# lh3/psmc

Measured on AMD Instinct MI355X. Metric: genome bins/sec through forward-backward (n=64), higher is better.
Workload: dtype f64; 1 GPU; configs[2]: whole-genome .psmcfa-like batch, 30000001 bins x 64 states in 90 segments per GPU, -p 4+25*2+4+6, one E-step (EM iteration) per step, parameters of a different EM round every step; mode=fast, bins_per_gpu=30000001, bins_total=30000001, n_states=64, segments=90, longest_segment=2490000, tiles=8127, speculative_overlap_bins=3072, structured_sweeps=True, tile_bins=3712

## Files before the change

psmc_amd/csrc/api.hip:

```cpp
#include "psmc_hip_ctx.h"

static void destroy_kids(psmc_hip_ctx *c);

static int make_streams(psmc_hip_ctx *c)
{
	hipStream_t *st[5] = {&c->stream, &c->stream2, &c->stream3, &c->stream4, &c->stream5};
	for (hipStream_t *s : st) if (*s) { (void)hipStreamSynchronize(*s); (void)hipStreamDestroy(*s); *s = nullptr; }
	if (c->cu_count <= 0) {
		for (hipStream_t *s : st) if (hipStreamCreateWithFlags(s, hipStreamNonBlocking) != hipSuccess) return PSMC_HIP_EDEVICE;
		return 0;
	}
	int cus = 0;
	if (hipDeviceGetAttribute(&cus, hipDeviceAttributeMultiprocessorCount, c->device) != hipSuccess || cus <= 0) return PSMC_HIP_EDEVICE;
	if (c->cu_first < 0 || c->cu_first + c->cu_count > cus) return PSMC_HIP_EINVAL;
	std::vector<uint32_t> mask((size_t)(cus + 31) / 32, 0u);
	for (int i = c->cu_first; i < c->cu_first + c->cu_count; ++i) mask[(size_t)i >> 5] |= 1u << (i & 31);
	for (hipStream_t *s : st) if (hipExtStreamCreateWithCUMask(s, (uint32_t)mask.size(), mask.data()) != hipSuccess) return PSMC_HIP_EDEVICE;
	return 0;
}

extern "C" int psmc_hip_device_cus(int device)
{
	int cus = 0;
	if (hipDeviceGetAttribute(&cus, hipDeviceAttributeMultiprocessorCount, device) != hipSuccess) { (void)hipGetLastError(); return 0; }
// ... 93 lines not shown
			}
		}
	}
	*out = c;
	return PSMC_HIP_OK;
}

static void destroy_kids(psmc_hip_ctx *c)
{
	if (c->x_twin) { psmc_hip_destroy(c->x_twin); c->x_twin = nullptr; }
	for (psmc_hip_ctx *k : c->kids) psmc_hip_destroy(k);
	c->kids.clear();
	c->share_T = 0;
}

extern "C" void psmc_hip_destroy(psmc_hip_ctx *c)
{
	if (!c) return;
	(void)hipSetDevice(c->device);
	destroy_kids(c);
	if (c->parent) {
		void *mine[] = {c->d_seg_off, c->d_seg_len, c->d_work, c->d_chunks, c->d_entry, c->d_bexit, c->d_Cpart, c->d_Epart, c->d_LLpart,
		                c->d_stage, c->d_stats, c->d_warm, c->d_bentry, c->d_dirty, c->d_cnt, c->d_gate, c->d_queue, c->d_touch, c->d_items, c->d_ftiles, c->d_Kcol,
		                c->d_segA, c->d_segE, c->d_segA0, c->d_chk};
		for (void *p : mine) if (p) (void)hipFree(p);
		if (c->h_cnt) (void)hipHostFree(c->h_cnt);
		if (c->h_ritems) (void)hipHostFree(c->h_ritems);
		if (c->h_mlen) (void)hipHostFree(c->h_mlen);
		if (c->h_chunks) (void)hipHostFree(c->h_chunks);
		if (c->h_mis) (void)hipHostFree(c->h_mis);
		if (c->d_prevx) (void)hipFree(c->d_prevx);
		if (c->d_finv) (void)hipFree(c->d_finv);
		delete c;
		return;
	}
	if (c->stream) (void)hipStreamSynchronize(c->stream);
	free_wide_fast(c);
	if (c->stream2) (void)hipStreamSynchronize(c->stream2);
	if (c->stream3) (void)hipStreamSynchronize(c->stream3);
	if (c->stream4) (void)hipStreamSynchronize(c->stream4);
	if (c->stream5) (void)hipStreamSynchronize(c->stream5);
	if (!c->obs_borrowed && c->d_obs) (void)hipFree(c->d_obs);
	void *ptrs[] = {c->d_seg_off, c->d_seg_len, c->d_work, c->d_par, c->d_f, c->d_b, c->d_s, c->d_segA, c->d_segE,
	                c->d_segA0, c->d_chk, c->d_chunks, c->d_entry, c->d_bexit, c->d_Cpart, c->d_Epart, c->d_LLpart,
	                c->d_stage, c->d_stats, c->d_warm, c->d_bentry, c->d_dirty, c->d_cnt, c->d_gate, c->d_queue, c->d_touch, c->d_sb, c->d_items, c->d_ftiles, c->d_Kcol,
	                c->d_bw_seg, c->d_bw_par, c->d_bw_tab, c->d_bpar, c->d_s_all, c->d_cu_mask, c->d_lkp, c->d_lkoff, c->d_b2};
	for (void *p : ptrs) if (p) (void)hipFree(p);
	if (c->h_par) (void)hipHostFree(c->h_par);
	if (c->h_cnt) (void)hipHostFree(c->h_cnt);
	if (c->h_ritems) (void)hipHostFree(c->h_ritems);
	if (c->h_mlen) (void)hipHostFree(c->h_mlen);
	if (c->h_chunks) (void)hipHostFree(c->h_chunks);
	if (c->h_mis) (void)hipHostFree(c->h_mis);
	if (c->d_prevx) (void)hipFree(c->d_prevx);
	if (c->d_finv) (void)hipFree(c->d_finv);
	for (int i = 0; i < 10; ++i) if (c->ev[i]) (void)hipEventDestroy(c->ev[i]);
	for (int i = 0; i < 14; ++i) if (c->evx[i]) (void)hipEventDestroy(c->evx[i]);
	if (c->stream4) (void)hipStreamDestroy(c->stream4);
	if (c->stream5) (void)hipStreamDestroy(c->stream5);
	if (c->stream2) (void)hipStreamDestroy(c->stream2);
	if (c->stream3) (void)hipStreamDestroy(c->stream3);
	if (c->stream) (void)hipStreamDestroy(c->stream);
	delete c;
}

extern "C" int psmc_hip_set_option(psmc_hip_ctx *c, const char *key, double v)
{
	if (!c || !key) return PSMC_HIP_EINVAL;
	std::string k(key);
	if (k == "batch_first") { if (v < 0 || v > 1e6) return PSMC_HIP_EINVAL; c->batch_first = (int)v; return PSMC_HIP_OK; }
	destroy_kids(c);
	if (k == "chunk") { if (v < 0) return PSMC_HIP_EINVAL; c->chunk = (int)v; c->plan_dirty = true; }
	else if (k == "warmup") { if (v < 0) return PSMC_HIP_EINVAL; c->warmup = (int)v; c->warmup_set = true; c->plan_dirty = true; }
	else if (k == "max_rounds") c->max_rounds = (int)v;
	else if (k == "structured") { c->struct_opt = v != 0 ? 1 : 0; }
	else if (k == "learn") { c->learn = v != 0 ? 1 : 0; }
	else if (k == "merge") { c->merge = v != 0 ? 1 : 0; c->plan_dirty = true; c->chunk_cap = 0; }
	else if (k == "adapt") { c->adapt = v != 0 ? 1 : 0; c->plan_dirty = true; c->chunk_cap = 0; }
	else if (k == "prev_start") { c->prev_start = v != 0 ? 1 : 0; c->prev_ok = false; c->plan_dirty = true; c->chunk_cap = 0; }
	else if (k == "warm_shift") { if (v < 0 || v > 4) return PSMC_HIP_EINVAL; c->warm_shift = (int)v; c->warm_shift_set = true; c->plan_dirty = true; }
	else if (k == "merge1") { if (v < -1 || v > 1) return PSMC_HIP_EINVAL; c->merge1 = (int)v; c->plan_dirty = true; }
	else if (k == "phase1") { if (v < -1 || v > 1) return PSMC_HIP_EINVAL; c->phase1 = (int)v; }
	else if (k == "phase1_waves") { if (v < 1 || v > 4) return PSMC_HIP_EINVAL; c->phase1_waves = (int)v; }
	else if (k == "lanes8") { if (v < -1 || v > 1) return PSMC_HIP_EINVAL; c->lanes8 = (int)v; }
	else if (k == "gap_tiles") { c->gap_tiles = v != 0 ? 1 : 0; c->plan_dirty = true; c->items_dirty = true; }
	else if (k == "coarse") { if (v < -1 || v > 16) return PSMC_HIP_EINVAL; c->coarse = (int)v; c->plan_dirty = true; c->items_dirty = true; }
	else if (k == "kc_sub") { if (v < 1 || v > 16) return PSMC_HIP_EINVAL; c->kc_sub = (int)v; c->kc_sub_set = true; c->plan_dirty = true; c->items_dirty = true; }
	else if (k == "two_phase") { if (v != -1 && v != 0 && v != 2) return PSMC_HIP_EINVAL; c->two_phase = (int)v; c->plan_dirty = true; c->items_dirty = true; }
	else if (k == "kc_min") { if (v < -1) return PSMC_HIP_EINVAL; c->kc_min = (int)v; c->items_dirty = true; }
	else if (k == "ckpt") { c->ckpt = v != 0 ? 1 : 0; }
	else if (k == "fuse") { c->fuse = v != 0 ? 1 : 0; c->plan_dirty = true; }
	else if (k == "fuse128") { if (v != 0 && v != 2) return PSMC_HIP_EINVAL; c->fuse128 = (int)v; c->plan_dirty = true; c->items_dirty = true; }
	else if (k == "group_cap") { if (v < 0) return PSMC_HIP_EINVAL; c->group_cap = (int)v; c->items_dirty = true; }
	else if (k == "share_learn") { c->share_learn = v != 0 ? 1 : 0; }
	else if (k == "exact_refwd") { if (v < -1 || v > 2) return PSMC_HIP_EINVAL; c->exact_refwd = (int)v; c->reserved_refwd = -1; c->reserved_cap = 0; if (c->d_b2) { (void)hipFree(c->d_b2); c->d_b2 = nullptr; c->b2_bins = c->b2_alloc = 0; } }
	else if (k == "batch_sort") { c->batch_sort = v != 0 ? 1 : 0; }
	else if (k == "batch_tailfill") c->batch_tailfill = v != 0;
	else if (k == "batch_major") c->batch_major = v != 0;
	else if (k == "batch_bins") { if (v < 0) return PSMC_HIP_EINVAL; c->batch_bins = (int64_t)v; }
	else if (k == "overlap") c->overlap = v != 0 ? 1 : 0;
	else if (k == "warm_tol") c->warm_tol = v;
	else if (k == "wide_fast") { if (v != 0 && v != 1) return PSMC_HIP_EINVAL; c->wide_fast = (int)v; }
	else if (k == "wide_decode") { if (v != 0 && v != 1) return PSMC_HIP_EINVAL; c->wide_decode = (int)v; }
	else if (k == "rep_impl") c->rep_impl = v < 0 ? -1 : (v != 0 ? 1 : 0);
	else return PSMC_HIP_EINVAL;
	return PSMC_HIP_OK;
}

int set_segments_common(psmc_hip_ctx *c, int n_seg, const int32_t *L)
{
	destroy_kids(c);
	c->reserved_refwd = -1; c->reserved_cap = 0;
	if (c->d_b2) { (void)hipFree(c->d_b2); c->d_b2 = nullptr; c->b2_bins = c->b2_alloc = 0; }
	c->n_seg = n_seg;
	c->L.assign(L, L + n_seg);
	int rc;
	if ((rc = dev_alloc(c, &c->d_seg_off, (size_t)n_seg))) return rc;
	if ((rc = dev_alloc(c, &c->d_seg_len, (size_t)n_seg))) return rc;
	HIPCHK(c, hipMemcpy(c->d_seg_off, c->off.data(), sizeof(int64_t) * n_seg, hipMemcpyHostToDevice));
	HIPCHK(c, hipMemcpy(c->d_seg_len, c->L.data(), sizeof(int32_t) * n_seg, hipMemcpyHostToDevice));
	std::vector<int32_t> all(n_seg);
	for (int i = 0; i < n_seg; ++i) all[i] = i;
	return psmc_hip_select(c, n_seg, all.data());
}

extern "C" int psmc_hip_load_segments(psmc_hip_ctx *c, int n_seg, const uint8_t *const *seq, const int32_t *L)
{
	if (!c || n_seg < 1 || !seq || !L) return fail(c, PSMC_HIP_EINVAL, "load_segments: bad argument");
	HIPCHK(c, hipSetDevice(c->device));
	c->off.resize(n_seg);
	int64_t tot = 0;
	for (int i = 0; i < n_seg; ++i) {
		if (L[i] < 1 || !seq[i]) return fail(c, PSMC_HIP_EINVAL, "load_segments: empty segment");
		c->off[i] = tot;
		tot += ((int64_t)L[i] + 63) & ~(int64_t)63;
	}
	c->total = tot;
	std::vector<uint8_t> host((size_t)tot + 256, 2);
	for (int i = 0; i < n_seg; ++i) {
		for (int32_t j = 0; j < L[i]; ++j)
			if (seq[i][j] > 2) return fail(c, PSMC_HIP_EINVAL, "load_segments: symbol outside {0,1,2}");
		memcpy(host.data() + c->off[i], seq[i], (size_t)L[i]);
	}
	if (!c->obs_borrowed && c->d_obs) { (void)hipFree(c->d_obs); }
	c->d_obs = nullptr; c->obs_borrowed = false;
	int rc;
	if ((rc = dev_alloc(c, &c->d_obs, host.size()))) return rc;
	HIPCHK(c, hipMemcpy(c->d_obs, host.data(), host.size(), hipMemcpyHostToDevice));
	return set_segments_common(c, n_seg, L);
}

extern "C" int psmc_hip_load_segments_device(psmc_hip_ctx *c, int n_seg, const void *d_obs, const int64_t *off,
                                             const int32_t *L)
{
	if (!c || n_seg < 1 || !d_obs || !off || !L) return fail(c, PSMC_HIP_EINVAL, "load_segments_device: bad argument");
	HIPCHK(c, hipSetDevice(c->device));
	int64_t end = 0;
	for (int i = 0; i < n_seg; ++i) {
		if (L[i] < 1 || (off[i] & 63) || off[i] < end) return fail(c, PSMC_HIP_EINVAL, "load_segments_device: bad layout");
		end = off[i] + (((int64_t)L[i] + 63) & ~(int64_t)63);
	}
	if (!c->obs_borrowed && c->d_obs) (void)hipFree(c->d_obs);
	c->d_obs = (uint8_t *)d_obs; c->obs_borrowed = true;
	c->off.assign(off, off + n_seg);
	c->total = end;
	return set_segments_common(c, n_seg, L);
// ... 374 lines not shown
```

psmc_amd/csrc/api_batch.hip:

```cpp
#include "psmc_hip_ctx.h"

namespace {
struct RepSel { std::vector<int32_t> work, sel2work; int64_t bins = 0; };
}

static int batch_selections(psmc_hip_ctx *c, int n_rep, const int32_t *sel_off, const int32_t *sel_idx, std::vector<RepSel> &reps)
{
	std::vector<int32_t> pos(c->n_seg);
	reps.assign(n_rep, RepSel());
	for (int r = 0; r < n_rep; ++r) {
		const int n_sel = sel_off[r + 1] - sel_off[r];
		if (n_sel < 1) return fail(c, PSMC_HIP_EINVAL, "estep_batch: empty selection");
		std::fill(pos.begin(), pos.end(), -1);
		RepSel &R = reps[r];
		R.sel2work.resize(n_sel);
		for (int i = 0; i < n_sel; ++i) {
			const int32_t sg = sel_idx[sel_off[r] + i];
			if (sg < 0 || sg >= c->n_seg) return fail(c, PSMC_HIP_EINVAL, "estep_batch: index out of range");
			if (pos[sg] < 0) { pos[sg] = (int32_t)R.work.size(); R.work.push_back(sg); R.bins += ((int64_t)c->L[sg] + 63) & ~(int64_t)63; }
			R.sel2work[i] = pos[sg];
		}
	}
	return 0;
}
// ... 299 lines not shown
				}
		}
	};
	std::vector<int32_t> finished;
	for (int g = 0; g < n_launches; ++g) {
		const double t_a = now();
		const int e0 = l_first[g], nw = l_first[g + 1] - e0;
		int64_t run = 0; int32_t longest = 0;
		for (int i = e0; i < e0 + nw; ++i) if (wseg[i] >= 0) { run = std::max(run, wtab[i] + padded_len(wseg[i])); longest = std::max(longest, c->L[wseg[i]]); }
		EstepLaunch p;
		fill_common(c, p, c->stream, c->d_bpar);
		p.d_work = c->d_bw_seg + e0; p.n_work = nw; p.d_work_par = c->d_bw_par + e0; p.d_work_tab = c->d_bw_tab + e0; p.par_stride = (int64_t)PL; p.work_align = align;
		p.exact_refwd = refwd ? (c->exact_refwd == 1 ? 1 : 2) : 0;
		p.d_cu_mask = c->d_cu_mask;
		if (fwd_all) { p.exact_only = 2; p.d_work_tab_s = c->d_bw_tab + n_all + e0; p.d_s = c->d_s_all; }
		p.d_segA = c->d_segA; p.d_segE = c->d_segE; p.d_segA0 = c->d_segA0; p.d_chk = c->d_chk;
		const double t_b = now();
		if (launch_exact(p) != 0) return fail(c, PSMC_HIP_EDEVICE, "launch_exact (batch)", hipGetLastError());
		if (dbg_t) (void)hipStreamSynchronize(c->stream);
		const double t_c = now();
		std::vector<int64_t> lkoff((size_t)nw);
		int64_t lk_tot = 0;
		for (int i = 0; i < nw; ++i) { lkoff[i] = lk_tot; lk_tot += wseg[e0 + i] >= 0 ? c->L[wseg[e0 + i]] / LKP_DIV + LKP_MIN : 1; }
		HIPCHK(c, hipMemcpyAsync(c->d_lkoff, lkoff.data(), sizeof(int64_t) * nw, hipMemcpyHostToDevice, c->stream));
		if (launch_lk_products(c->stream, p, fwd_all ? c->d_s_all : c->d_s, c->d_lkoff, c->d_lkp) != 0) return fail(c, PSMC_HIP_EDEVICE, "launch_lk_products", hipGetLastError());
		c->h_lkp.resize((size_t)lk_tot);
		HIPCHK(c, hipMemcpyAsync(c->h_segA.data() + (size_t)e0 * S * S, c->d_segA, sizeof(double) * nw * S * S, hipMemcpyDeviceToHost, c->stream));
		HIPCHK(c, hipMemcpyAsync(c->h_segE.data() + (size_t)e0 * 3 * S, c->d_segE, sizeof(double) * nw * 3 * S, hipMemcpyDeviceToHost, c->stream));
		HIPCHK(c, hipMemcpyAsync(c->h_lkp.data(), c->d_lkp, sizeof(double) * (size_t)lk_tot, hipMemcpyDeviceToHost, c->stream));
		HIPCHK(c, hipStreamSynchronize(c->stream));
		const double t_d = now();
		collect_timing(c);
		int n_over = 0;
		for (int i = 0; i < nw; ++i) {
			if (wseg[e0 + i] < 0) continue;
			const int32_t sg = wseg[e0 + i];
			const double *q = &c->h_lkp[(size_t)lkoff[i]];
			const int cnt = (int)q[0], cap_i = c->L[sg] / LKP_DIV + LKP_MIN;
			if (cnt >= 1 && cnt < cap_i) {
				double sum = 0.0;
				for (int j = 1; j <= cnt; ++j) sum += log(q[j]);
				lk_all[(size_t)e0 + i] = sum;
			} else {
				++n_over;
				c->h_s.resize((size_t)c->L[sg]);
				HIPCHK(c, hipMemcpyAsync(c->h_s.data(), (fwd_all ? c->d_s_all + wtab_s[e0 + i] : c->d_s + wtab[e0 + i]), sizeof(double) * (size_t)c->L[sg], hipMemcpyDeviceToHost, c->stream));
				HIPCHK(c, hipStreamSynchronize(c->stream));
				lk_all[(size_t)e0 + i] = host_lk(c->h_s.data(), c->L[sg]);
			}
		}
		if (dbg_t && n_over) fprintf(stderr, "[psmc_hip] batch launch %d: %d entries logged more products than their buffer holds (host hmm_lk)\n", g, n_over);
		if (dbg_t) fprintf(stderr, "[psmc_hip] batch launch %d: %d entries (longest %d bins), %.1f M table bins | prepare %.3f s, kernels %.3f (fwd %.0f bwd %.0f expect %.0f ms%s), read-back %.3f, hmm_lk %.3f\n",
		                   g, nw, (int)longest, run / 1e6, t_b - t_a, t_c - t_b, c->last_ms[1], c->last_ms[2], c->last_ms[3],
		                   fwd_all ? (g == 0 ? (std::string("; forward pass of all entries ") + std::to_string(fwd_all_s) + " s").c_str() : "; fwd: see launch 0") : "", t_d - t_c, now() - t_d);
		++c->last_batch_groups;
		const double t_f = now();
		finished.clear();
		for (int r = 0; r < n_rep; ++r) if (last_launch[r] == g) { finalize(r); finished.push_back(r); }
		t_sums += now() - t_f;
		if (done && !finished.empty()) done(user, (int)finished.size(), finished.data());
	}
	if (dbg_t) {
		std::string per;
		for (int g = 0; g < n_launches; ++g) per += (g ? " " : "") + std::to_string(std::count(last_launch.begin(), last_launch.end(), g));
		fprintf(stderr, "[psmc_hip] batch: %d replicates, %d entries in %d launches (replicates complete after launch 0..: %s), host sums %.3f s\n", n_rep, n_all, n_launches, per.c_str(), t_sums);
	}
	return PSMC_HIP_OK;
}

static psmc_hip_ctx *batch_child(psmc_hip_ctx *c, int r)
{
	while ((int)c->kids.size() <= r) {
		psmc_hip_ctx *k = new (std::nothrow) psmc_hip_ctx();
		if (!k) return nullptr;
		k->n = c->n; k->ns = c->ns; k->device = c->device; k->mode = c->mode; k->parent = c;
		k->chunk = c->chunk > 0 ? c->chunk : c->share_T;
		k->warmup = c->warmup; k->max_rounds = c->max_rounds; k->rep_impl = c->rep_impl;
		k->n_sub = c->n_sub; k->target_waves = c->target_waves; k->overlap = c->overlap; k->warm_tol = c->warm_tol; k->struct_opt = c->struct_opt;
		k->struct_tiles_set = c->struct_tiles_set; k->struct_tiles = c->struct_tiles;
		k->two_phase = c->two_phase; k->kc_div = c->kc_div; k->kc_min = c->kc_min; k->ckpt = c->ckpt; k->fuse = c->fuse;
		k->learn = c->learn; k->group_cap = c->group_cap; k->warm_shift = c->warm_shift; k->kc_sub = c->kc_sub; k->kcol_prio = c->kcol_prio;
		k->fuse128 = c->fuse128; k->coarse = c->coarse; k->gate = c->gate; k->lanes8 = c->lanes8; k->gap_tiles = c->gap_tiles; k->exact_refwd = c->exact_refwd;
		k->merge = c->merge; k->adapt = c->adapt; k->prev_start = c->prev_start;
		k->merge1 = c->merge1; k->merge_order = c->merge_order; k->runs_late = c->runs_late; k->warm_shift_set = c->warm_shift_set; k->kc_sub_set = c->kc_sub_set;
		k->stream = c->stream; k->stream2 = c->stream2; k->stream3 = c->stream3; k->stream4 = c->stream4; k->stream5 = c->stream5;
		for (int i = 0; i < 14; ++i) k->evx[i] = c->evx[i];
		for (int i = 0; i < 10; ++i) k->ev[i] = c->ev[i];
		k->h_par = c->h_par; k->d_par = c->d_par; k->par_len = c->par_len;
		k->d_obs = c->d_obs; k->obs_borrowed = true; k->off = c->off; k->total = c->total;
		if (set_segments_common(k, c->n_seg, c->L.data()) != 0) { c->err = k->err; psmc_hip_destroy(k); return nullptr; }
		c->kids.push_back(k);
	}
	return c->kids[r];
}

static int batch_exact_once(psmc_hip_ctx *c, int r, const int32_t *idx, int n_sel, const double *a, const double *e, const double *a0,
                            double *A, double *sums, double *E, double *LL, const char *why)
{
	const int n = c->n;
	fprintf(stderr, "[psmc_hip] replicate %d: fast E-step did not converge (%s); repeating this E-step with the exact kernels\n", c->batch_first + r, why);
	int rc = 0;
	if (!c->x_twin) {
		if ((rc = psmc_hip_create(&c->x_twin, n, c->device, PSMC_HIP_MODE_EXACT))) return fail(c, rc, "estep_batch: cannot create the exact twin context");
		if ((rc = psmc_hip_load_segments_device(c->x_twin, c->n_seg, c->d_obs, c->off.data(), c->L.data()))) {
			c->err = "exact twin: " + c->x_twin->err; psmc_hip_destroy(c->x_twin); c->x_twin = nullptr; return rc;
		}
	}
	std::vector<double> Af;
	double *Ao = A;
	if (!Ao) { Af.resize((size_t)n * n); Ao = Af.data(); }
	if ((rc = psmc_hip_select(c->x_twin, n_sel, idx)) || (rc = psmc_hip_estep(c->x_twin, a, e, a0, Ao, E, nullptr, LL, nullptr))) { c->err = "exact twin: " + c->x_twin->err; return rc; }
	if (sums) {
		memset(sums, 0, sizeof(double) * 5 * (size_t)n);
		for (int k = 0; k < n; ++k)
			for (int l = 0; l < n; ++l) {
				const double v = Ao[(size_t)k * n + l];
				if (l < k) { sums[k] += v; sums[3 * n + l] += v; } else if (l > k) { sums[n + k] += v; sums[4 * n + l] += v; } else sums[2 * n + k] = v;
			}
	}
	++c->n_exact_fallbacks;
	return PSMC_HIP_OK;
}

static int batch_fast(psmc_hip_ctx *c, int n_rep, const double *a, const double *e, const double *a0, const int32_t *sel_off,
                      const int32_t *sel_idx, double *A, double *sums, double *E, double *LL, psmc_hip_batch_done_fn done, void *user)
{
	const int n = c->n;
	if (c->share_T == 0 && c->share_learn) {
		int T = c->chunk;
		if (T <= 0) {
			std::vector<RepSel> reps;
			int rc0 = batch_selections(c, n_rep, sel_off, sel_idx, reps);
			if (rc0) return rc0;
			int64_t most = 0; size_t nw = 1;
			for (const RepSel &R : reps) {
				int64_t bins = 0;
				for (int32_t sg : R.work) bins += c->L[sg];
				if (bins > most) { most = bins; nw = R.work.size(); }
			}
			T = auto_tile_len(c, most, nw, true);
		}
		c->share_T = T;
		c->sh_glue_f.assign(c->n_seg, {}); c->sh_glue_b.assign(c->n_seg, {}); c->sh_wf.assign(c->n_seg, {}); c->sh_wb.assign(c->n_seg, {});
		for (int sg = 0; sg < c->n_seg; ++sg) {
			const size_t nt = ((size_t)c->L[sg] + T - 1) / T;
			c->sh_glue_f[sg].assign(nt, 0); c->sh_glue_b[sg].assign(nt, 0); c->sh_wf[sg].assign(nt, c->warmup); c->sh_wb[sg].assign(nt, c->warmup);
		}
	}
	static const bool dbg_t = getenv("PSMC_HIP_DEBUG_TIMES") != nullptr;
	const double t_call = dbg_now();
	double t_est = 0.0;
	for (int r = 0; r < n_rep; ++r) {
		const double t_k = dbg_now();
		psmc_hip_ctx *k = batch_child(c, c->batch_first + r);
		c->dbg_acc[0] += dbg_now() - t_k;
		if (!k) return fail(c, PSMC_HIP_ENOMEM, "estep_batch: cannot create the replicate context");
		const int n_sel = sel_off[r + 1] - sel_off[r];
		if (n_sel < 1) return fail(c, PSMC_HIP_EINVAL, "estep_batch: empty selection");
		const int32_t *idx = sel_idx + sel_off[r];
		int rc = 0;
		{
			const double t_s = dbg_now();
			if ((int)k->sel.size() != n_sel || memcmp(k->sel.data(), idx, sizeof(int32_t) * n_sel) != 0) rc = psmc_hip_select(k, n_sel, idx);
			c->dbg_acc[1] += dbg_now() - t_s;
		}
		const double t_e = dbg_now();
// ... 48 lines not shown
```

psmc_amd/csrc/api_fast.hip:

```cpp
#include "psmc_hip_ctx.h"

int ensure_fast_buffers(psmc_hip_ctx *c)
{
	if (c->d_stage && c->d_stats && c->d_warm && c->d_cnt && c->h_cnt && c->d_gate) return 0;
	int rc;
	const size_t sl = (size_t)c->ns * c->ns + 3 * (size_t)c->ns + 1;
	if ((rc = dev_alloc(c, &c->d_stage, (size_t)RED_ROWS * sl))) return rc;
	if ((rc = dev_alloc(c, &c->d_stats, sl))) return rc;
	if ((rc = dev_alloc(c, &c->d_warm, (size_t)2))) return rc;
	if ((rc = dev_alloc(c, &c->d_cnt, (size_t)4))) return rc;
	if ((rc = dev_alloc(c, &c->d_gate, (size_t)4))) return rc;
	if (!c->h_cnt && (hipHostMalloc((void **)&c->h_cnt, 4 * sizeof(int), hipHostMallocMapped) != hipSuccess ||
	                  hipHostGetDevicePointer((void **)&c->m_cnt, c->h_cnt, 0) != hipSuccess)) {
		c->h_cnt = nullptr;
		return fail(c, PSMC_HIP_ENOMEM, "hipHostMalloc (mapped)");
	}
	return 0;
}

int auto_tile_len(const psmc_hip_ctx *c, int64_t bins, size_t n_work, bool st)
{
	const int64_t ROUND1 = 4096;
	int64_t want = st ? c->struct_tiles : c->target_waves;
	if (st && !c->struct_tiles_set && bins < 2 * ROUND1 * (int64_t)std::max(c->warmup, 1))
		want = std::max<int64_t>(ROUND1 - (int64_t)n_work, ROUND1 / 2);
	const int T = (int)((bins + want - 1) / want);
	return std::max(256, (T + 63) & ~63);
}

static int plan_fast(psmc_hip_ctx *c)
{
	int64_t bins = 0;
	for (int32_t s : c->work) bins += c->L[s];
	int T = c->chunk;
	const bool st = c->use_struct;
	const int64_t ROUND1 = 4096;
	bool one_round = false;
	if (T <= 0) T = auto_tile_len(c, bins, c->work.size(), st);
	c->chunks.clear(); c->chunk_seg.clear(); c->chunk_idx.clear();
	for (size_t w = 0; w < c->work.size(); ++w) {
		const int32_t s = c->work[w];
		for (int32_t lo = 1; lo <= c->L[s]; lo += T) {
			c->chunk_seg.push_back(s); c->chunk_idx.push_back((lo - 1) / T);
			Chunk ch;
			ch.off = c->off[s]; ch.L = c->L[s]; ch.lo = lo; ch.hi = std::min(c->L[s], lo + T - 1); ch.mult = c->mult[w];
			ch.flags = 0; ch.wf = ch.wb = c->warmup;
			if (ch.lo - c->warmup <= 1) ch.flags |= CHUNK_ANCHOR_F;
			if ((int64_t)ch.hi + c->warmup + 1 >= ch.L) ch.flags |= CHUNK_ANCHOR_B;
			if (ch.hi == ch.L) ch.flags |= CHUNK_LAST;
			c->chunks.push_back(ch);
		}
	}
	const int nc = (int)c->chunks.size();
	c->chunk_used = T;
	c->planned_struct = st;
	one_round = st && nc <= ROUND1;
	c->two_phase_used = c->two_phase >= 0 ? c->two_phase : (one_round ? 0 : 2);
	c->merge1_used = c->merge1 >= 0 ? c->merge1 : (one_round ? 1 : 0);
	c->warm_shift_used = c->warm_shift_set ? c->warm_shift : (one_round ? 0 : 1);
	c->coarse_used = c->coarse >= 0 ? std::max(c->coarse, 1) : (one_round && nc > 2048 && T < c->warmup ? 2 : 1);
	c->kc_sub_used = c->kc_sub_set ? c->kc_sub : std::max(1, std::min(4, (int)((8 * (int64_t)T + T + c->warmup - 1) / std::max(T + c->warmup, 1))));
	c->n_sub_used = st ? (fused_counts(c) ? 1 : std::max(1, std::min(c->n_sub, (9216 + nc - 1) / std::max(nc, 1)))) : c->n_sub;
	c->glue_f.assign(nc, 0); c->glue_b.assign(nc, 0);
	if (c->parent && c->parent->share_T == T && st) {
		const psmc_hip_ctx *P = c->parent;
		for (int b = 0; b < nc; ++b) {
			const int sg = c->chunk_seg[b], ix = c->chunk_idx[b];
			if (sg >= (int)P->sh_glue_f.size() || ix >= (int)P->sh_glue_f[sg].size()) continue;
			c->glue_f[b] = P->sh_glue_f[sg][ix]; c->glue_b[b] = P->sh_glue_b[sg][ix];
			c->chunks[b].wf = std::max(c->chunks[b].wf, P->sh_wf[sg][ix]); c->chunks[b].wb = std::max(c->chunks[b].wb, P->sh_wb[sg][ix]);
		}
	}
	c->items_dirty = true;
	int rc;
	c->gap.assign(nc, 0);
	if (nc > c->chunk_cap) {
		if ((rc = dev_alloc(c, &c->d_chunks, (size_t)nc))) return rc;
		if ((rc = dev_alloc(c, &c->d_entry, (size_t)nc * c->ns))) return rc;
		if ((rc = dev_alloc(c, &c->d_bexit, (size_t)(nc + 1) * c->ns))) return rc;
		if ((rc = dev_alloc(c, &c->d_bentry, (size_t)nc * c->ns))) return rc;
		if ((rc = dev_alloc(c, &c->d_dirty, (size_t)2 * nc))) return rc;
		if ((rc = dev_alloc(c, &c->d_touch, (size_t)3 * nc))) return rc;
		if ((rc = dev_alloc(c, &c->d_finv, (size_t)nc))) return rc;
		if (c->h_mlen) { (void)hipHostFree(c->h_mlen); c->h_mlen = nullptr; c->m_mlen = nullptr; }
		if (c->h_mis) { (void)hipHostFree(c->h_mis); c->h_mis = nullptr; c->m_mis = nullptr; }
		if (c->prev_start && (rc = dev_alloc(c, &c->d_prevx, (size_t)nc * c->ns))) return rc;
		if ((c->merge || c->adapt) &&
		    (hipHostMalloc((void **)&c->h_mlen, (size_t)nc * sizeof(int), hipHostMallocMapped) != hipSuccess ||
		     hipHostGetDevicePointer((void **)&c->m_mlen, c->h_mlen, 0) != hipSuccess ||
		     hipHostMalloc((void **)&c->h_mis, (size_t)2 * nc * sizeof(double), hipHostMallocMapped) != hipSuccess ||
		     hipHostGetDevicePointer((void **)&c->m_mis, c->h_mis, 0) != hipSuccess))
			return fail(c, PSMC_HIP_ENOMEM, "hipHostMalloc (mapped)");
		if ((rc = dev_alloc(c, &c->d_LLpart, (size_t)nc))) return rc;
		if ((rc = dev_alloc(c, &c->d_items, (size_t)32 * nc + 64))) return rc;
		if ((rc = dev_alloc(c, &c->d_ftiles, (size_t)2 * (nc + 16)))) return rc;
		if (c->h_ritems) { (void)hipHostFree(c->h_ritems); c->h_ritems = nullptr; }
		if (hipHostMalloc((void **)&c->h_ritems, (size_t)4 * nc * sizeof(int), hipHostMallocMapped) != hipSuccess ||
		    hipHostGetDevicePointer((void **)&c->m_ritems, c->h_ritems, 0) != hipSuccess)
			return fail(c, PSMC_HIP_ENOMEM, "hipHostMalloc (mapped)");
		c->chunk_cap = nc;
	}
	if ((rc = dev_alloc(c, &c->d_Epart, (size_t)nc * c->n_sub_used * 3 * c->ns))) return rc;
	if ((rc = ensure_fast_buffers(c))) return rc;
	HIPCHK(c, hipMemcpy(c->d_chunks, c->chunks.data(), sizeof(Chunk) * nc, hipMemcpyHostToDevice));
	if (st && c->gap_tiles) {
		std::vector<int> fl(nc, 0);
		if (launch_tile_allmiss(c->stream, c->d_obs, c->d_chunks, nc, c->d_dirty) != 0) return fail(c, PSMC_HIP_EDEVICE, "k_tile_allmiss", hipGetLastError());
		HIPCHK(c, hipMemcpyAsync(fl.data(), c->d_dirty, sizeof(int) * nc, hipMemcpyDeviceToHost, c->stream));
		HIPCHK(c, hipMemsetAsync(c->d_dirty, 0, sizeof(int) * nc, c->stream));
		HIPCHK(c, hipStreamSynchronize(c->stream));
		for (int b = 0; b < nc; ++b) {
			const Chunk &ch = c->chunks[b];
			c->gap[b] = fl[b] && ch.lo > 1 && ch.hi < ch.L && ch.hi - ch.lo + 1 == T;
		}
		auto same = [&](int x, int y) { return x >= 0 && y < nc && c->chunks[x].off == c->chunks[y].off; };
		for (int b = 0; b < nc; ++b) {
			if (c->gap[b]) { if (same(b - 1, b)) c->glue_f[b] = 1; if (same(b, b + 1)) c->glue_b[b] = 1; }
			if (b > 0 && c->gap[b - 1] && same(b - 1, b)) c->glue_f[b] = 1;
			if (b + 1 < nc && c->gap[b + 1] && same(b, b + 1)) c->glue_b[b] = 1;
		}
	}
	c->plan_dirty = false; c->chunks_dirty = false; c->prev_ok = false;
	return 0;
}

static int build_items(psmc_hip_ctx *c, bool two_phase_bwd, int coarse)
{
	const int nc = (int)c->chunks.size(), W = c->warmup;
	const int cf = std::max(1, coarse), cb = two_phase_bwd ? 1 : cf;
	std::vector<int> odd(nc, 0), idx(nc, 0);
	for (int b = 1; b < nc; ++b) if (c->chunks[b].off == c->chunks[b - 1].off) { odd[b] = !odd[b - 1]; idx[b] = idx[b - 1] + 1; }
	std::vector<std::pair<long long, std::pair<int, int>>> kf, kb;
	auto key = [](int steps, bool run, bool phase_b) { return (run ? -(1ll << 40) : (phase_b ? (1ll << 40) : 0ll)) - steps; };
	std::vector<char> from_above(nc, 0), in_run(nc, 0), in_run_f(nc, 0), in_run_b(nc, 0);
	std::vector<std::pair<int, int>> gf, gb;
	auto same_seg = [&](int x, int y) { return c->chunks[x].off == c->chunks[y].off; };
	const bool gaps = c->gap_tiles && (int)c->gap.size() == nc;
	std::vector<int64_t> eff(nc + 1, 0);
	for (int b = 0; b < nc; ++b) eff[b + 1] = eff[b] + ((gaps && c->gap[b]) ? 0 : c->chunks[b].hi - c->chunks[b].lo + 1);
	auto span_ok = [&](int b, int e) { return eff[e + 1] - eff[b] <= (int64_t)c->group_cap; };
	for (int b = 0; b < nc;) {
		int e = b + 1;
		while (e < nc && c->glue_f[e] && same_seg(e, b) && span_ok(b, e)) ++e;
		if (e - b > 1) for (int t = b; t < e; ++t) in_run[t] = in_run_f[t] = 1;
		else
			while (e < nc && e - b < cf && same_seg(e, b) && idx[e] % cf != 0 && !c->glue_f[e] && !(e + 1 < nc && c->glue_f[e + 1] && same_seg(e + 1, e))) ++e;
		gf.push_back({b, e - b});
		b = e;
	}
	for (int b = 0; b < nc;) {
		int e = b + 1;
		while (e < nc && c->glue_b[e - 1] && same_seg(e, b) && span_ok(b, e) &&
		       c->chunks[e].lo < c->chunks[e].L)
			++e;
		if (e - b > 1) for (int t = b; t < e; ++t) in_run[t] = in_run_b[t] = 1;
		else
			while (e < nc && e - b < cb && same_seg(e, b) && idx[e] % cb != 0 && !c->glue_b[e - 1] && !(e + 1 < nc && c->glue_b[e] && same_seg(e + 1, e)) &&
			       c->chunks[e].lo < c->chunks[e].L)
				++e;
		gb.push_back({b, e - b});
		b = e;
	}
	int n_run = 0;
	for (int b = 0; b < nc; ++b) n_run += in_run[b];
	const int cap_b = (nc + 7) / 8 * 4;
	c->runs_in_b = two_phase_bwd && c->runs_late && n_run > 0 && n_run <= cap_b / 2;
	int above_budget = c->runs_in_b ? cap_b - n_run : nc;
	for (const auto &gr : gb) {
		const int b = gr.first, e = b + gr.second;
		const Chunk &lo = c->chunks[b], &top = c->chunks[e - 1];
		bool pb = two_phase_bwd && e - b == 1 && odd[b] && b + 1 < nc && c->chunks[b + 1].off == lo.off && c->chunks[b + 1].lo < c->chunks[b + 1].L;
		if (pb && c->runs_in_b && (in_run[b] || in_run[b + 1] || above_budget <= 0)) pb = false;
		if (pb) { from_above[b] = 1; --above_budget; }
		kb.push_back({key(std::min(top.hi + chunk_warm_b(top, W) + 1, top.L) - lo.lo, in_run_b[b] != 0, pb), {b, e - b}});
	}
	std::vector<int> la, lb;
	{
		std::vector<int> freet;
		for (int b = 0; b < nc; ++b) {
			if (from_above[b]) lb.push_back(b | (1 << 30));
			else if (b > 0 && from_above[b - 1]) la.push_back(b);
			else if (c->runs_in_b && in_run[b]) lb.push_back(b);
			else freet.push_back(b);
		}
		const bool single = lb.empty() && nc <= 4096;
		for (int b : freet) { if (single || la.size() <= lb.size()) la.push_back(b); else lb.push_back(b); }
	}
	for (const auto &gr : gf) {
		const int b = gr.first, e = b + gr.second;
		const Chunk &h = c->chunks[b], &l = c->chunks[e - 1];
		kf.push_back({key(l.hi - std::max(1, h.lo - chunk_warm_f(h, W)) + 1, in_run_f[b] != 0, false), {b, e - b}});
	}
	std::sort(kf.begin(), kf.end()); std::sort(kb.begin(), kb.end());
	std::vector<int> h((size_t)4 * nc, 0), mem((size_t)4 * nc, 0);
	c->n_mem_f = c->n_mem_b = 0;
	for (size_t i = 0; i < kf.size(); ++i) {
		h[2 * i] = kf[i].second.first; h[2 * i + 1] = kf[i].second.second;
		if (in_run_f[kf[i].second.first])
			for (int t = 0; t < kf[i].second.second; ++t) { mem[2 * (size_t)c->n_mem_f] = kf[i].second.first + t; mem[2 * (size_t)c->n_mem_f + 1] = 1; ++c->n_mem_f; }
	}
	for (size_t i = 0; i < kb.size(); ++i) {
		h[(size_t)2 * nc + 2 * i] = kb[i].second.first; h[(size_t)2 * nc + 2 * i + 1] = kb[i].second.second;
		if (in_run_b[kb[i].second.first])
			for (int t = 0; t < kb[i].second.second; ++t) {
				mem[(size_t)2 * nc + 2 * (size_t)c->n_mem_b] = kb[i].second.first + t; mem[(size_t)2 * nc + 2 * (size_t)c->n_mem_b + 1] = 1; ++c->n_mem_b;
			}
	}
	c->n_items_f = (int)kf.size(); c->n_items_b = (int)kb.size();
	c->order_f.clear();
	for (const auto &it : kf) if (!in_run_f[it.second.first]) c->order_f.push_back(it.second.first);
	c->n_long_f = c->n_long_b = 0;
	while (c->n_long_f < c->n_items_f && in_run_f[kf[c->n_long_f].second.first]) ++c->n_long_f;
	while (c->n_long_b < c->n_items_b && in_run_b[kb[c->n_long_b].second.first]) ++c->n_long_b;
	c->n_B_b = 0;
	for (int b = 0; b < nc; ++b) c->n_B_b += from_above[b];
	{
		c->n_list_a = (int)la.size(); c->n_list_b = (int)lb.size();
		c->count_group = c->ns == 128 && c->fuse128 == 2 ? 16 : 4;
		while (la.size() % c->count_group) la.push_back(-1);
		while (lb.size() % c->count_group) lb.push_back(-1);
		la.insert(la.end(), lb.begin(), lb.end());
		if (!la.empty()) HIPCHK(c, hipMemcpy(c->d_ftiles, la.data(), sizeof(int) * la.size(), hipMemcpyHostToDevice));
	}
	c->items_two_phase = two_phase_bwd ? 2 : 0; c->items_coarse = coarse;
	HIPCHK(c, hipMemcpy(c->d_items, h.data(), sizeof(int) * h.size(), hipMemcpyHostToDevice));
	{
		std::vector<int> sg;
		for (size_t i = (size_t)c->n_long_b; i < kb.size(); ++i)
			for (int t = kb[i].second.second - 1; t >= 0; --t) { sg.push_back(kb[i].second.first + t); sg.push_back(1); }
		c->n_singles_b = (int)sg.size() / 2;
		if (!sg.empty()) HIPCHK(c, hipMemcpy(c->d_items + (size_t)24 * nc, sg.data(), sizeof(int) * sg.size(), hipMemcpyHostToDevice));
	}
	HIPCHK(c, hipMemcpy(c->d_items + (size_t)8 * nc, mem.data(), sizeof(int) * mem.size(), hipMemcpyHostToDevice));
	{
		std::vector<int> fx;
		for (int b = 0; b < nc; ++b)
			if (!in_run_f[b] && !(b > 0 && in_run_f[b - 1] && same_seg(b - 1, b))) { fx.push_back(b); fx.push_back(1); }
		c->n_fix_f = (int)fx.size() / 2;
		if (!fx.empty()) HIPCHK(c, hipMemcpy(c->d_items + (size_t)30 * nc, fx.data(), sizeof(int) * fx.size(), hipMemcpyHostToDevice));
	}
	{
		const int n4f = c->n_items_f - c->n_long_f, n4b = c->n_items_b - c->n_long_b - c->n_B_b;
		std::vector<std::pair<long long, int>> qk;
		for (int k = 0; 4 * k < n4f; ++k) {
			long long st = 0;
			for (int i = c->n_long_f + 4 * k; i < std::min(c->n_long_f + 4 * k + 4, c->n_items_f); ++i) {
				const Chunk &h = c->chunks[kf[i].second.first], &l = c->chunks[kf[i].second.first + kf[i].second.second - 1];
				st = std::max(st, (long long)(l.hi - std::max(1, h.lo - chunk_warm_f(h, W)) + 1));
			}
			qk.push_back({-st * 504, 2 * k});
		}
		for (int k = 0; 4 * k < n4b; ++k) {
			long long st = 0;
			for (int i = c->n_long_b + 4 * k; i < std::min(c->n_long_b + 4 * k + 4, c->n_long_b + n4b); ++i) {
				const Chunk &lo = c->chunks[kb[i].second.first], &top = c->chunks[kb[i].second.first + kb[i].second.second - 1];
				const int q = std::min(top.hi + chunk_warm_b(top, W) + 1, top.L);
				st = std::max(st, (long long)(q - (coarse > 1 ? std::min(lo.hi, lo.L - 1) : std::min(top.hi, top.L - 1))));
			}
			qk.push_back({-st * 534, 2 * k + 1});
		}
		std::stable_sort(qk.begin(), qk.end(), [](const std::pair<long long, int> &x, const std::pair<long long, int> &y) { return x.first < y.first; });
		std::vector<int> qv(qk.size());
		for (size_t i = 0; i < qk.size(); ++i) qv[i] = qk[i].second;
		if (c->queue_cap < qv.size()) { int rc; if ((rc = dev_alloc(c, &c->d_queue, qv.size()))) return rc; c->queue_cap = qv.size(); }
		c->n_queue = (int)qv.size();
		if (!qv.empty()) HIPCHK(c, hipMemcpy(c->d_queue, qv.data(), sizeof(int) * qv.size(), hipMemcpyHostToDevice));
	}
	std::vector<int> wl((size_t)4 * nc, 0), kc, runs_f, runs_b, kslot, kuniq;
	int gap_slot[2] = {-1, -1};
	auto push_kc = [&](int t, int dir) {
		const int j = (int)kc.size() / 2;
		kc.push_back(t); kc.push_back(dir);
		if (gaps && c->gap[t] && c->chunk_used % 4 == 0) {
			if (gap_slot[dir] < 0) { gap_slot[dir] = (int)kuniq.size(); kuniq.push_back(j); }
			kslot.push_back(gap_slot[dir]);
		} else { kslot.push_back((int)kuniq.size()); kuniq.push_back(j); }
	};
	c->n_wl_f = c->n_wl_b = 0;
	const int kc_min = c->kc_min >= 0 ? c->kc_min : (c->ns == 128 ? (nc > 4096 ? 12 : 8) : (nc > 4096 ? 5 : 4));
	const bool chains = kc_min >= 2;
	const int head_count = c->ns == 64 ? 0 : 1;
	auto add_runs = [&](const std::vector<std::pair<long long, std::pair<int, int>>> &k, int n_long, bool bwd) {
		int &nw = bwd ? c->n_wl_b : c->n_wl_f;
		std::vector<int> &rv = bwd ? runs_b : runs_f;
		int *w = wl.data() + (bwd ? (size_t)2 * nc : 0);
		int budget = std::max(64, nc / c->kc_div);
		for (int i = 0; i < n_long; ++i) {
			int first = k[i].second.first, count = k[i].second.second;
			int cost = 0;
			for (int tt = first; tt < first + count; ++tt) cost += (gaps && c->gap[tt] && c->chunk_used % 4 == 0) ? 0 : 1;
			cost = std::max(cost - 1, 1);
			const bool chain = chains && count >= kc_min && cost <= budget;
			if (chain) budget -= cost;
			if (chain && !bwd && c->chunks[first].lo == 1) {
				w[2 * nw] = first; w[2 * nw + 1] = (head_count == 0 && count - 1 >= 2) ? -1 : 2; ++nw;
				first += 1; count -= 1;
				if (count >= 2) {
					rv.push_back(first); rv.push_back(count); rv.push_back((int)(kc.size() / 2)); rv.push_back(0);
					for (int t = first; t < first + count - 1; ++t) push_kc(t, 0);
				}
			} else if (chain) {
				w[2 * nw] = bwd ? first + count - 1 : first; w[2 * nw + 1] = head_count; ++nw;
				rv.push_back(first); rv.push_back(count); rv.push_back((int)(kc.size() / 2)); rv.push_back(0);
				if (!bwd) for (int t = first; t < first + count - 1; ++t) push_kc(t, 0);
				else for (int t = first + count - 1; t > first; --t) push_kc(t, 1);
// ... 83 lines not shown
	if (changed) {
		c->chunks_dirty = true;
		int64_t total = 0, waste = 0;
		for (size_t i = 0; i + 3 < c->order_f.size(); i += 4) {
			int64_t s4 = 0, mx = 0;
			for (int r = 0; r < 4; ++r) { const Chunk &ch = c->chunks[c->order_f[i + r]]; const int64_t st = (int64_t)ch.hi - std::max(1, ch.lo - ch.wf) + 1; s4 += st; mx = std::max(mx, st); }
			total += 4 * mx; waste += 4 * mx - s4;
		}
		if (total > 0 && waste * 100 > total * 3) c->items_dirty = true;
	}
}

int enqueue_fast(psmc_hip_ctx *c, const double *a, const double *e, const double *a0, double *d_out,
                        hipStream_t st)
{
	HIPCHK(c, hipSetDevice(c->device));
	if (c->n_seg < 1) return fail(c, PSMC_HIP_ESTATE, "estep: no segments loaded");
	int rc;
	c->dec_kind = DEC_NONE;
	const unsigned long long serial0 = dbg_root(c)->tab_serial;
	if ((rc = ensure_tables(c, false))) return rc;
	c->tables_batch = false;
	if ((rc = stage_params(c, a, e, a0, st))) return rc;
	if (!c->want_factored && !(c->use_struct && fused_counts(c)) && (rc = ensure_tables(c, true))) return rc;
	if (c->ns == 128 && !c->use_struct)
		return fail(c, PSMC_HIP_ENOTSUP, "fast mode beyond 64 states needs a transition matrix of the PSMC form (structured sweeps)");
	if (c->want_factored && !c->use_struct)
		return fail(c, PSMC_HIP_ENOTSUP, "factored statistics need a transition matrix of the PSMC form");
	{
		const double t0 = dbg_now();
		if ((c->plan_dirty || c->planned_struct != c->use_struct) && (rc = plan_fast(c))) return rc;
		dbg_root(c)->dbg_acc[2] += dbg_now() - t0;
	}
	EstepLaunch p;
	fill_common(c, p, st);
	p.d_chunks = c->d_chunks; p.n_chunks = (int)c->chunks.size(); p.warmup = c->warmup; p.n_sub = c->n_sub_used;
	const bool two_phase_bwd = c->two_phase_used >= 1 && p.fused == 1;
	p.merge1 = c->merge1_used; p.merge_order = c->merge_order >= 0 ? c->merge_order : (c->chunk_used < c->warmup ? 1 : 0);
	if (c->chunks_dirty) {
		psmc_hip_ctx *R = dbg_root(c);
		if (R->h_chunks_cap < c->chunks.size()) {
			if (R->h_chunks) { (void)hipHostFree(R->h_chunks); R->h_chunks = nullptr; }
			if (hipHostMalloc((void **)&R->h_chunks, sizeof(Chunk) * c->chunks.size(), hipHostMallocDefault) != hipSuccess) return fail(c, PSMC_HIP_ENOMEM, "hipHostMalloc");
			R->h_chunks_cap = c->chunks.size();
		}
		HIPCHK(c, hipStreamSynchronize(st));
		memcpy(R->h_chunks, c->chunks.data(), sizeof(Chunk) * c->chunks.size());
		HIPCHK(c, hipMemcpyAsync(c->d_chunks, R->h_chunks, sizeof(Chunk) * c->chunks.size(), hipMemcpyHostToDevice, st));
		c->chunks_dirty = false;
	}
	const int coarse = (c->use_struct && p.fused != 0) ? c->coarse_used : 1;
	{
		const double t0 = dbg_now();
		if (c->use_struct && (c->items_dirty || c->items_two_phase != (two_phase_bwd ? 2 : 0) || c->items_coarse != coarse) && (rc = build_items(c, two_phase_bwd, coarse))) return rc;
		dbg_root(c)->dbg_acc[3] += dbg_now() - t0;
	}
	p.lanes8 = (c->lanes8 >= 0 ? c->lanes8 != 0 && p.fused != 0 : p.fused == 2 && p.n_chunks > 4096) && c->ns == 64 ? 1 : 0;
	{
		const size_t nc_ = c->chunks.size(), S_ = (size_t)c->ns;
		const size_t need = p.fused == 2 ? nc_ * 7 * S_ + 64 : (p.fused == 1 ? (nc_ / 4 + 8) * S_ * S_ : nc_ * (size_t)c->n_sub_used * S_ * S_);
		if (c->cpart_cap < need) { if ((rc = dev_alloc(c, &c->d_Cpart, need))) return rc; c->cpart_cap = need; }
	}
	{
		c->merge_used = c->merge != 0 && c->h_mlen && c->use_struct && p.fused == 1 && c->ns == 64 && c->chunk_used % 16 == 0;
		p.merge = c->merge_used ? 1 : 0;
		p.d_fmerge = c->d_touch + 2 * (size_t)p.n_chunks; p.d_finv = c->d_finv; p.m_mlen = c->m_mlen; p.h_mlen = c->h_mlen; p.m_mis = c->m_mis;
		p.d_fix_f = c->d_items + 30 * (size_t)p.n_chunks; p.n_fix_f = c->n_fix_f;
		if (c->h_mlen) memset(c->h_mlen, 0, sizeof(int) * p.n_chunks);
		if (c->h_mis) for (int b = 0; b < p.n_chunks; ++b) c->h_mis[b] = -1.0;
		const bool prev = c->prev_start && c->d_prevx && c->prev_ok && c->use_struct && c->prev_serial == serial0 && c->prev_f == c->d_f && c->prev_ckpt == p.ckpt;
		p.d_prevx = prev ? c->d_prevx : nullptr;
		c->prev_ok = false;
	}
	p.d_gate = (c->gate >= 0 ? c->gate != 0 : coarse > 1) ? c->d_gate : nullptr;
	if (c->phase1 != 0 && c->use_struct && p.fused == 1 && c->ns == 64 && !p.lanes8 && !p.merge1 && c->overlap && c->n_queue > 0) {
		int cus = c->cu_count;
		if (cus <= 0 && (hipDeviceGetAttribute(&cus, hipDeviceAttributeMultiprocessorCount, c->device) != hipSuccess || cus <= 0)) return fail(c, PSMC_HIP_EDEVICE, "hipDeviceGetAttribute");
		p.d_queue = c->d_queue; p.n_queue = c->n_queue; p.d_qhead = c->d_gate + 2;
		p.q_grid = std::min(c->n_queue, 4 * cus * c->phase1_waves);
	}
	p.coarse = coarse; p.d_singles_b = c->d_items + 24 * (size_t)p.n_chunks; p.n_singles_b = c->n_singles_b;
	p.n_B_b = c->n_B_b; p.runs_in_b = c->runs_in_b ? 1 : 0; p.n_list_a = c->n_list_a; p.n_list_b = c->n_list_b; p.d_ftiles = c->d_ftiles; p.count_group = c->count_group;
	c->timing_two_launches = p.fused == 1 && p.n_list_b > 0;
	p.d_items_f = c->d_items; p.d_items_b = c->d_items + 2 * p.n_chunks;
	p.d_ritems_f = c->d_items + 4 * p.n_chunks; p.d_ritems_b = c->d_items + 6 * p.n_chunks;
	p.n_items_f = c->n_items_f; p.n_items_b = c->n_items_b; p.tile_len = c->chunk_used; p.h_ritems = c->h_ritems; p.m_ritems = c->m_ritems; p.m_cnt = c->m_cnt;
	c->flagged_f.clear(); c->flagged_b.clear();
	p.flagged_f = &c->flagged_f; p.flagged_b = &c->flagged_b;
	p.d_entry = c->d_entry; p.d_bentry = c->d_bentry; p.d_bexit = c->d_bexit; p.d_Cpart = c->d_Cpart; p.d_Epart = c->d_Epart;
	p.d_dirty = c->d_dirty; p.d_cnt = c->d_cnt; p.h_cnt = c->h_cnt; p.tol = c->warm_tol; p.max_rounds = c->max_rounds;
	p.d_touch_f = c->d_touch; p.d_touch_b = c->d_touch + p.n_chunks; p.d_dirty_b = c->d_dirty + p.n_chunks;
	p.stream2 = c->stream2; p.stream3 = c->stream3; p.stream4 = c->stream4; p.overlap = c->overlap;
	p.n_long_f = c->n_long_f; p.n_long_b = c->n_long_b; p.n_mem_f = c->n_mem_f; p.n_mem_b = c->n_mem_b;
	p.d_members_f = c->d_items + 8 * p.n_chunks; p.d_members_b = c->d_items + 10 * p.n_chunks;
	p.d_wl_f = c->d_items + 12 * (size_t)p.n_chunks; p.d_wl_b = c->d_items + 14 * (size_t)p.n_chunks; p.n_wl_f = c->n_wl_f; p.n_wl_b = c->n_wl_b;
	p.d_kc = c->d_items + 16 * (size_t)p.n_chunks; p.d_kruns = c->d_items + 20 * (size_t)p.n_chunks;
	p.n_kc = c->n_kc; p.n_chain_f = c->n_chain_f; p.n_chain_b = c->n_chain_b;
	p.d_kslot = c->d_items + 26 * (size_t)p.n_chunks; p.d_kuniq = c->d_items + 28 * (size_t)p.n_chunks; p.n_kuniq = c->n_kuniq;
	p.kcol_prio = c->kcol_prio;
	p.d_Kcol = c->d_Kcol; p.kc_sub = kcol2_on(c) ? c->kc_sub_used : 1;
	p.d_Kexp = c->d_Kcol ? c->d_Kcol + (size_t)c->n_kuniq * p.kc_sub * c->ns * c->ns : nullptr; p.stream5 = c->stream5;
	for (int i = 0; i < 14; ++i) p.evx[i] = c->evx[i];
	p.d_LLpart = c->d_LLpart; p.d_stage = c->d_stage; p.d_stats = d_out; p.d_warm = c->d_warm;
	p.tiny_total = (double)c->sel.size() * HMM_TINY_H;
	if (p.d_prevx) launch_gather_prev(p, st, c->n_long_f, c->n_items_f - c->n_long_f, c->d_prevx);
	{
		const double t0 = dbg_now();
		if (launch_fast(p, &c->report) != 0) return fail(c, PSMC_HIP_EDEVICE, "launch_fast", hipGetLastError());
		psmc_hip_ctx *R = dbg_root(c);
		R->dbg_acc[4] += dbg_now() - t0;
		R->dbg_acc[6] += c->report.fwd_rounds + c->report.bwd_rounds; R->dbg_acc[7] += c->report.fwd_tiles + c->report.bwd_tiles;
	}
	if (getenv("PSMC_HIP_DEBUG_FLAGGED")) {
		auto dump = [&](const char *dir, const std::vector<int> &fl, const std::vector<uint8_t> &glue, bool bwd) {
			std::vector<int> u(fl); std::sort(u.begin(), u.end()); u.erase(std::unique(u.begin(), u.end()), u.end());
			fprintf(stderr, "[psmc_hip] flagged %s: %zu tile repairs, %zu distinct tiles, rounds %d:", dir, fl.size(), u.size(), bwd ? c->report.bwd_rounds : c->report.fwd_rounds);
			for (size_t i = 0; i < u.size() && i < 400; ++i) {
				const int b = u[i]; const Chunk &ch = c->chunks[b];
				int seg = 0; while (seg + 1 < c->n_seg && c->off[seg + 1] <= ch.off) ++seg;
				fprintf(stderr, " [t%d seg%d %d..%d w%d g%d x%d m%.1e ml%d]", b, seg, ch.lo, ch.hi, bwd ? ch.wb : ch.wf, (int)glue[b], (int)std::count(fl.begin(), fl.end(), b),
				        c->h_mis ? c->h_mis[(bwd ? c->chunks.size() : 0) + b] : 0.0, (!bwd && c->h_mlen) ? c->h_mlen[b] : 0);
			}
			fprintf(stderr, "\n");
		};
		dump("fwd", c->flagged_f, c->glue_f, false); dump("bwd", c->flagged_b, c->glue_b, true);
	}
	if (!c->report.converged) return fail(c, PSMC_HIP_ECONVERGE, "fast mode: tile boundaries did not converge within max_rounds");
	if (c->merge_used && c->h_mlen)
		for (size_t b = 0; b < c->chunks.size(); ++b) {
			c->report.merged += c->h_mlen[b] > 0;
			if (c->h_mlen[b] < 0 || (c->h_mlen[b] > 0 && !c->adapt)) c->flagged_f.push_back((int)b);
		}
	if (c->use_struct && c->adapt && c->merge_used && c->h_mis) adapt_warmups(c);
	if (c->use_struct && c->learn) learn_groups(c);
	if (c->use_struct) { c->prev_ok = true; c->prev_serial = dbg_root(c)->tab_serial; c->prev_f = c->d_f; c->prev_ckpt = p.ckpt; }
	c->dec_kind = c->merge_used ? DEC_MERGED : (p.fused != 0 ? DEC_NO_BT : DEC_FAST);
	c->dec_serial = dbg_root(c)->tab_serial;
	return 0;
}

int read_warm(psmc_hip_ctx *c, hipStream_t st)
{
	unsigned long long w[2];
	HIPCHK(c, hipMemcpyAsync(w, c->d_warm, sizeof(w), hipMemcpyDeviceToHost, st));
	HIPCHK(c, hipStreamSynchronize(st));
	memcpy(&c->warm_err[0], &w[0], 8); memcpy(&c->warm_err[1], &w[1], 8);
	return 0;
}

extern "C" int psmc_hip_estep_device(psmc_hip_ctx *c, const double *a, const double *e, const double *a0,
                                     void *d_stats, void *stream)
{
	if (!c || !a || !e || !a0 || !d_stats) return fail(c, PSMC_HIP_EINVAL, "estep_device: bad argument");
	if (c->mode != PSMC_HIP_MODE_FAST) return fail(c, PSMC_HIP_ENOTSUP, "estep_device: fast mode only");
	c->timing_valid = false;
	return enqueue_fast(c, a, e, a0, (double *)d_stats, (hipStream_t)stream);
}

extern "C" int psmc_hip_fast_diag(psmc_hip_ctx *c, double *wf, double *wb, int *n_chunks, int *warmup_used)
{
	if (!c) return PSMC_HIP_EINVAL;
	if (c->mode != PSMC_HIP_MODE_FAST || !c->d_warm) return fail(c, PSMC_HIP_ESTATE, "fast_diag: no fast E-step yet");
	HIPCHK(c, hipSetDevice(c->device));
	unsigned long long w[2];
	HIPCHK(c, hipMemcpy(w, c->d_warm, sizeof(w), hipMemcpyDeviceToHost));
	memcpy(&c->warm_err[0], &w[0], 8); memcpy(&c->warm_err[1], &w[1], 8);
// ... 158 lines not shown
```

psmc_amd/csrc/estep_fast.hip:

```cpp
#include <hip/hip_runtime.h>
#include <cmath>
#include <algorithm>
#include "wave_prims.h"
#include "psmc_hip_internal.h"

namespace psmc {

typedef double d4_t __attribute__((ext_vector_type(4)));

__device__ __forceinline__ double pick_ef(int sym, double e0, double e1) {
	return sym == 0 ? e0 : (sym == 1 ? e1 : 1.0);
}

__device__ __forceinline__ double fast_rcp(double x) {
	double r = __builtin_amdgcn_rcp(x);
	double t = __builtin_fma(-x, r, 1.0);
	r = __builtin_fma(r, t, r);
	t = __builtin_fma(-x, r, 1.0);
	r = __builtin_fma(r, t, r);
	return r;
}

__device__ __forceinline__ double wave_max(double v) {
#pragma unroll
	for (int m = 32; m >= 1; m >>= 1) v = fmax(v, __shfl_xor(v, m, 64));
	return v;
}
__device__ __forceinline__ double wave_add(double v) {
#pragma unroll
	for (int m = 32; m >= 1; m >>= 1) v += __shfl_xor(v, m, 64);
	return v;
}
__device__ __forceinline__ double rel_mismatch(double x, double y) {
	const double num = wave_max(fabs(x - y)), den = wave_max(fabs(y));
	const bool bad = __any((x != x) || (y != y));
	return bad ? __builtin_inf() : num / den;
}

template <int REP, bool REPAIR>
__global__ __launch_bounds__(64) void k_fwd_fast(const double *__restrict__ a, const double *__restrict__ e,
                                                   const double *__restrict__ a0, const uint8_t *__restrict__ obs,
                                                   const Chunk *__restrict__ chunks, int W, double tol,
                                                   const int *__restrict__ dirty, double *__restrict__ f,
                                                   double *__restrict__ invd, double *__restrict__ entry,
                                                   int *__restrict__ touch_f)
{
	if (REPAIR && !dirty[blockIdx.x]) return;
	if (REPAIR) __builtin_amdgcn_s_setprio(3);
	const int lane = threadIdx.x;
	if (REPAIR && lane == 0) touch_f[blockIdx.x] = 1;
	const Chunk c = chunks[blockIdx.x];
	const uint8_t *o = obs + c.off;
	double *fo = f + c.off * 64, *io = invd + c.off;
	double A[64];
	load_nat_matrix(a, lane, A);
	const double e0 = e[lane], e1 = e[64 + lane];
	double x;
	int p;
	if (REPAIR) {
		x = fo[(int64_t)(c.lo - 2) * 64 + lane];
		p = c.lo;
	} else {
		const int ws = max(1, c.lo - W);
		if (ws == 1) {
			x = a0[lane] * pick_ef((int)o[0], e0, e1);
			if (c.lo == 1) fo[lane] = x;
			p = 2;
		} else {
			x = a0[lane];
			p = ws;
		}
	}
	int symn = o[(((p - 1) >> 6) << 6) + lane];
	bool done = false;
	while (p <= c.hi && !done) {
		const int blk = (p - 1) >> 6;
		const int symv = symn;
		symn = o[((blk + 1) << 6) + lane];
		const int pend = min(c.hi, (blk + 1) << 6);
		double oldv = 0.0;
		if (REPAIR) oldv = fo[(int64_t)(pend - 1) * 64 + lane];
		for (; p <= pend; ++p) {
			const int idx = p - 1;
			const int sym = __builtin_amdgcn_readlane(symv, idx & 63);
			if (p == c.lo) entry[(int64_t)blockIdx.x * 64 + lane] = x;
			double ev = pick_ef(sym, e0, e1);
			if ((p & (NORM_EVERY - 1)) == 0) {
				const double inv = fast_rcp(first_lane_f64(wave_sum_nat(x)));
				ev *= inv;
				if (p >= c.lo && lane == 0) io[idx] = inv;
			}
			x = matvec64_nat(x, A) * ev;
			if (p >= c.lo) fo[(int64_t)idx * 64 + lane] = x;
		}
		if (REPAIR && rel_mismatch(x, oldv) <= tol) done = true;
	}
}

template <int REP, bool REPAIR>
__global__ __launch_bounds__(64) void k_bwd_fast(const double *__restrict__ aT, const double *__restrict__ e,
                                                   const uint8_t *__restrict__ obs, const Chunk *__restrict__ chunks,
                                                   int W, double tol, const int *__restrict__ dirty,
                                                   double *__restrict__ bt, double *__restrict__ sb,
                                                   double *__restrict__ bentry, double *__restrict__ bexit,
                                                   int *__restrict__ touch_b)
{
	if (REPAIR && !dirty[blockIdx.x]) return;
	if (REPAIR) __builtin_amdgcn_s_setprio(3);
	const int lane = threadIdx.x;
	if (REPAIR && lane == 0) touch_b[blockIdx.x] = 1;
	const Chunk c = chunks[blockIdx.x];
	const int L = c.L, lo = c.lo, top = min(c.hi, L - 1);
	if (top < lo) return;
	const uint8_t *o = obs + c.off;
	double *bto = bt + c.off * 64, *sbo = sb + c.off;
	double A[64];
	load_nat_matrix(aT, lane, A);
	const double e0 = e[lane], e1 = e[64 + lane];
	double btn;
	int p;
	if (REPAIR) {
		btn = bexit[(int64_t)(blockIdx.x + 1) * 64 + lane];
		p = top;
	} else {
		const int q = min(c.hi + W + 1, L);
		btn = pick_ef((int)o[q - 1], e0, e1);
		p = q - 1;
	}
	int symn = o[(max((p - 1) >> 6, 0) << 6) + lane];
	bool done = false;
	while (p >= lo && !done) {
		const int blk = (p - 1) >> 6;
		const int symv = symn;
		symn = o[(max(blk - 1, 0) << 6) + lane];
		const int pbeg = max(lo, (blk << 6) + 1);
		const int pc = max(pbeg, lo + 1);
		double oldv = 0.0, chkv = 0.0;
		const bool can_check = REPAIR && pc <= min(p, top);
		if (can_check) oldv = bto[(int64_t)(pc - 1) * 64 + lane];
		for (; p >= pbeg; --p) {
			const int idx = p - 1;
			const int sym = __builtin_amdgcn_readlane(symv, idx & 63);
			double ev = pick_ef(sym, e0, e1);
			if ((p & (NORM_EVERY - 1)) == 0) {
				const double sc = fast_rcp(first_lane_f64(wave_sum_nat(btn)));
				ev *= sc;
				if (p <= top && lane == 0) sbo[idx] = sc;
			}
			if (p == top) {
				bto[(int64_t)top * 64 + lane] = btn;
				bentry[(int64_t)blockIdx.x * 64 + lane] = btn;
			}
			btn = matvec64_nat(btn, A) * ev;
			if (p <= top) {
				if (p > lo || lo == 1) bto[(int64_t)idx * 64 + lane] = btn;
				if (p == lo) bexit[(int64_t)blockIdx.x * 64 + lane] = btn;
				if (p == pc) chkv = btn;
			}
		}
		if (can_check && rel_mismatch(chkv, oldv) <= tol) done = true;
	}
}

template <int S> __device__ __forceinline__ double rel_mismatch_vec(const double *x, const double *y, int lane, bool with_scale = false) {
	double xv = x[lane], yv = y[lane], xw = 0.0, yw = 0.0;
	if (S == 128) { xw = x[64 + lane]; yw = y[64 + lane]; }
	const double sx = wave_add(xv + xw), sy = wave_add(yv + yw);
	const double ix = 1.0 / sx, iy = 1.0 / sy;
	double num = fabs(xv * ix - yv * iy), den = fabs(yv * iy);
	if (with_scale) num = fmax(num, fabs(sx - sy) * iy * den);
	bool bad = (xv != xv) || (yv != yv) || (ix != ix) || (iy != iy);
	if (S == 128) {
		num = fmax(num, fabs(xw * ix - yw * iy)); den = fmax(den, fabs(yw * iy));
		bad = bad || (xw != xw) || (yw != yw);
	}
	num = wave_max(num); den = wave_max(den);
	return __any(bad) ? __builtin_inf() : num / den;
}
template <bool BWD, int S>
__global__ __launch_bounds__(64) void k_verify(const Chunk *__restrict__ chunks, int n_chunks, double tol,
                                                 const double *__restrict__ f, const double *__restrict__ mine,
                                                 const double *__restrict__ bexit, int *__restrict__ dirty,
                                                 int *__restrict__ cnt, unsigned long long *__restrict__ warm, int with_scale,
                                                 double *__restrict__ mis)
{
	const int lane = threadIdx.x, b = blockIdx.x;
	const Chunk c = chunks[b];
	double m = 0.0;
	bool check;
	if (!BWD) {
		check = c.lo > 1 && !(c.flags & CHUNK_ANCHOR_F);
		if (check) m = rel_mismatch_vec<S>(mine + (int64_t)b * S, f + (c.off + c.lo - 2) * S, lane);
	} else {
		check = !(c.flags & (CHUNK_ANCHOR_B | CHUNK_LAST)) && min(c.hi, c.L - 1) >= c.lo && b + 1 < n_chunks;
		if (check) m = rel_mismatch_vec<S>(mine + (int64_t)b * S, bexit + (int64_t)(b + 1) * S, lane, with_scale != 0);
	}
	if (lane == 0) {
		const int bad = check && !(m <= tol);
		dirty[b] = bad;
		if (bad) atomicAdd(cnt, 1);
		if (mis) mis[b] = check ? m : -1.0;
		if (check) atomicMax(&warm[BWD ? 1 : 0], (unsigned long long)__double_as_longlong(m));
	}
}

__device__ __forceinline__ bool tile_touched(const Chunk *__restrict__ chunks, int b, const int *__restrict__ touch_f,
                                             const int *__restrict__ touch_b)
{
	bool t = touch_f[b] || touch_b[b];
	if (b > 0 && chunks[b - 1].off == chunks[b].off) t = t || touch_b[b - 1];
	return t;
}
template <int S>
__global__ __launch_bounds__(64, 2) void k_expect_mfma(const Chunk *__restrict__ chunks, int n_sub,
                                                         const uint8_t *__restrict__ obs, const double *__restrict__ f,
                                                         const double *__restrict__ bt, const double *__restrict__ sb,
                                                         const double *__restrict__ re, double *__restrict__ Cpart,
                                                         double *__restrict__ Spart, const int *__restrict__ touch_f,
                                                         const int *__restrict__ touch_b, int redo)
{
	constexpr int Q = S / 64, NB = S / 16;
	const int lane = threadIdx.x, t = lane >> 4, i = lane & 15;
	const int part = blockIdx.x / (Q * Q), quad = blockIdx.x % (Q * Q), qm = quad / Q, qn = quad % Q;
	const Chunk c = chunks[part / n_sub];
	if (redo && !tile_touched(chunks, part / n_sub, touch_f, touch_b)) return;
	const int sub = part % n_sub;
	const int top = min(c.hi, c.L - 1), n = top - c.lo + 1;
	const int per = n > 0 ? ((((n + n_sub - 1) / n_sub) + 3) & ~3) : 0;
	const int p0 = c.lo + sub * per, p1 = min(top, p0 + per - 1);
	const double *fo = f + c.off * S + i, *bo = bt + c.off * S + i, *sbo = sb + c.off;
	const uint8_t *o = obs + c.off;
	double re0[NB], re1[NB];
#pragma unroll
	for (int m = 0; m < NB; ++m) { re0[m] = re[16 * m + i]; re1[m] = re[S + 16 * m + i]; }
	d4_t acc[4][4];
	double Sacc[3][4];
#pragma unroll
	for (int m = 0; m < 4; ++m) {
#pragma unroll
		for (int nn = 0; nn < 4; ++nn) acc[m][nn] = (d4_t){0.0, 0.0, 0.0, 0.0};
		Sacc[0][m] = Sacc[1][m] = Sacc[2][m] = 0.0;
	}
	auto load = [&](int p, double (&FA)[NB], double (&BM)[4], double (&BP)[NB], double &sc, int &sym, bool &ok) {
		const int pp = p + t;
		ok = pp <= p1;
		const int64_t idx = (int64_t)(ok ? pp : p1) - 1;
		const double *fr = fo + idx * S, *br = bo + idx * S;
#pragma unroll
		for (int m = 0; m < NB; ++m) { FA[m] = fr[16 * m]; BP[m] = br[16 * m]; }
#pragma unroll
		for (int m = 0; m < 4; ++m) BM[m] = br[S + 64 * qn + 16 * m];
		sc = 1.0;
		if (((int)(idx + 1) & (NORM_EVERY - 1)) == 0) sc = sbo[idx];
		sym = o[idx];
	};
	if (p0 <= p1) {
		double FA[NB], BM[4], BP[NB], sc; int sym; bool ok;
		load(p0, FA, BM, BP, sc, sym, ok);
		for (int p = p0; p <= p1; p += 4) {
			double FN[NB], BN[4] = {0, 0, 0, 0}, BQ[NB], scn = 1.0; int symn = 2; bool okn = false;
#pragma unroll
			for (int m = 0; m < NB; ++m) { FN[m] = 0.0; BQ[m] = 0.0; }
			if (S == 64 && p + 4 <= p1) load(p + 4, FN, BN, BQ, scn, symn, okn);
			double g[NB], G = 0.0;
#pragma unroll
			for (int m = 0; m < NB; ++m) {
				const double r = sym == 0 ? re0[m] : (sym == 1 ? re1[m] : 1.0);
				g[m] = FA[m] * BP[m] * r;
				G += g[m];
			}
			G = G + dpp_mov<0xB1>(G);
			G = G + dpp_mov<0x4E>(G);
			G = G + dpp_mov<0x124>(G);
			G = G + dpp_mov<0x128>(G);
			const double iG = ok ? 1.0 / G : 0.0;
			const double w0 = sym == 0 ? iG : 0.0, w1 = sym == 1 ? iG : 0.0, w2 = sym == 2 ? iG : 0.0, wa = sc * iG;
			double FM[4];
#pragma unroll
			for (int m = 0; m < 4; ++m) {
				const double gm = g[4 * qm + m];
				Sacc[0][m] = __builtin_fma(gm, w0, Sacc[0][m]);
				Sacc[1][m] = __builtin_fma(gm, w1, Sacc[1][m]);
				Sacc[2][m] = __builtin_fma(gm, w2, Sacc[2][m]);
				FM[m] = FA[4 * qm + m] * wa;
			}
#pragma unroll
			for (int m = 0; m < 4; ++m)
#pragma unroll
				for (int nn = 0; nn < 4; ++nn)
					acc[m][nn] = __builtin_amdgcn_mfma_f64_16x16x4f64(FM[m], BM[nn], acc[m][nn], 0, 0, 0);
			if (S != 64 && p + 4 <= p1) load(p + 4, FA, BM, BP, sc, sym, ok);
			else if (S != 64) ok = false;
			if (S == 64) {
#pragma unroll
				for (int m = 0; m < NB; ++m) { FA[m] = FN[m]; BP[m] = BQ[m]; }
#pragma unroll
				for (int m = 0; m < 4; ++m) BM[m] = BN[m];
				sc = scn; sym = symn; ok = okn;
			}
		}
	}
	const double mult = (double)c.mult;
	double *out = Cpart + (int64_t)part * (S * S) + (int64_t)(64 * qm) * S + 64 * qn;
#pragma unroll
	for (int m = 0; m < 4; ++m)
#pragma unroll
		for (int nn = 0; nn < 4; ++nn)
#pragma unroll
			for (int r = 0; r < 4; ++r) out[(16 * m + t + 4 * r) * S + 16 * nn + i] = acc[m][nn][r] * mult;
	if (qn == 0) {
		double *os = Spart + (int64_t)part * (3 * S) + 64 * qm;
#pragma unroll
		for (int b = 0; b < 3; ++b)
#pragma unroll
			for (int m = 0; m < 4; ++m) {
				double v = Sacc[b][m];
				v += __shfl_xor(v, 16, 64);
				v += __shfl_xor(v, 32, 64);
				if (t == 0) os[b * S + 16 * m + i] = v * mult;
			}
	}
}

template <int S>
__global__ __launch_bounds__(64) void k_ll(const Chunk *__restrict__ chunks, const double *__restrict__ f,
                                             const double *__restrict__ invd, const double *__restrict__ entry,
                                             double *__restrict__ LLpart, const int *__restrict__ fmerge, const double *__restrict__ finv)
{
	const int lane = threadIdx.x;
	const Chunk c = chunks[blockIdx.x];
	const double *io = invd + c.off;
	double prod = 1.0, ll = 0.0;
	const int first = (max(c.lo, 2) + NORM_EVERY - 1) & ~(NORM_EVERY - 1);
	for (int p = first + NORM_EVERY * lane; p <= c.hi; p += NORM_EVERY * 64) {
		prod *= io[p - 1];
		if (prod > 1e280 || prod < 1e-280) { ll -= log(prod); prod = 1.0; }
	}
	ll -= log(prod);
	ll = wave_add(ll);
	if (c.lo > 1) {
		double u = f[(c.off + c.lo - 2) * S + lane], v = entry[(int64_t)blockIdx.x * S + lane];
		if (S == 128) { u += f[(c.off + c.lo - 2) * S + 64 + lane]; v += entry[(int64_t)blockIdx.x * S + 64 + lane]; }
		ll += log(wave_add(u)) - log(wave_add(v));
	}
	if (c.hi == c.L) {
		double v = f[(c.off + c.L - 1) * S + lane];
		if (S == 128) v += f[(c.off + c.L - 1) * S + 64 + lane];
		ll += log(wave_add(v));
	}
	if (fmerge && fmerge[blockIdx.x] > 0) ll -= log(finv[blockIdx.x]);
	if (lane == 0) LLpart[blockIdx.x] = ll * (double)c.mult;
}

template <int S>
__global__ __launch_bounds__(256) void k_reduce1(const double *__restrict__ Cpart, const double *__restrict__ Spart,
                                                   int nC, int nS, const double *__restrict__ LLpart, int nchunks,
                                                   double *__restrict__ stage)
{
	constexpr int SL = S * S + 3 * S + 1;
	const int y = blockIdx.y, tid = threadIdx.x;
	double *st = stage + (int64_t)y * SL;
	if ((int)blockIdx.x < S * S / 256) {
		const int i = blockIdx.x * 256 + tid;
		double s = 0.0;
		for (int j = y; j < nC; j += RED_ROWS) s += Cpart[(int64_t)j * (S * S) + i];
		st[i] = s;
	} else {
		for (int i = tid; i < 3 * S; i += 256) {
			double s = 0.0;
			for (int j = y; j < nS; j += RED_ROWS) s += Spart[(int64_t)j * (3 * S) + i];
			st[S * S + i] = s;
		}
		if (tid == 255) {
			double s = 0.0;
			for (int j = y; j < nchunks; j += RED_ROWS) s += LLpart[j];
			st[S * S + 3 * S] = s;
		}
	}
}
template <int S>
__global__ __launch_bounds__(256) void k_reduce2(const double *__restrict__ stage, const double *__restrict__ a,
                                                   const double *__restrict__ e, double tiny_total, int n,
                                                   double *__restrict__ out)
{
	constexpr int SL = S * S + 3 * S + 1;
	const int i = blockIdx.x * 256 + threadIdx.x;
	if (i >= SL) return;
	double s = 0.0;
	for (int y = 0; y < RED_ROWS; ++y) s += stage[(int64_t)y * SL + i];
	if (i < S * S) {
		const int k = i / S, l = i % S;
		if (k < n && l < n) out[k * n + l] = a[i] * s + tiny_total;
	} else if (i < S * S + 3 * S) {
		const int b = (i - S * S) / S, k = (i - S * S) % S;
		if (b < 2 && k < n) out[n * n + b * n + k] = s + tiny_total;
	} else {
		out[n * n + 2 * n] = s;
	}
}

template <bool REPAIR>
static void launch_fwd(const EstepLaunch &p, hipStream_t st)
{
	const dim3 g(p.n_chunks), b(64);
	if (p.rep_impl == 0)
		hipLaunchKernelGGL((k_fwd_fast<0, REPAIR>), g, b, 0, st, p.d_a, p.d_e, p.d_a0, p.d_obs, p.d_chunks, p.warmup,
		                   p.tol, p.d_dirty, p.d_f, p.d_s, p.d_entry, p.d_touch_f);
	else
		hipLaunchKernelGGL((k_fwd_fast<1, REPAIR>), g, b, 0, st, p.d_a, p.d_e, p.d_a0, p.d_obs, p.d_chunks, p.warmup,
		                   p.tol, p.d_dirty, p.d_f, p.d_s, p.d_entry, p.d_touch_f);
}
template <bool REPAIR>
static void launch_bwd(const EstepLaunch &p, hipStream_t st)
{
	const dim3 g(p.n_chunks), b(64);
	const double *aT = p.d_aeT + 2 * 4096;
	if (p.rep_impl == 0)
		hipLaunchKernelGGL((k_bwd_fast<0, REPAIR>), g, b, 0, st, aT, p.d_e, p.d_obs, p.d_chunks, p.warmup, p.tol,
		                   p.d_dirty_b, p.d_b, p.d_sb, p.d_bentry, p.d_bexit, p.d_touch_b);
	else
		hipLaunchKernelGGL((k_bwd_fast<1, REPAIR>), g, b, 0, st, aT, p.d_e, p.d_obs, p.d_chunks, p.warmup, p.tol,
		                   p.d_dirty_b, p.d_b, p.d_sb, p.d_bentry, p.d_bexit, p.d_touch_b);
}
static void launch_expect(const EstepLaunch &p, hipStream_t st, int redo)
{
	const int nC = p.n_chunks * p.n_sub;
	{
		if (p.ns == 128)
			hipLaunchKernelGGL(k_expect_mfma<128>, dim3(nC * 4), dim3(64), 0, st, p.d_chunks, p.n_sub, p.d_obs, p.d_f, p.d_b, p.d_sb,
			                   p.d_re, p.d_Cpart, p.d_Epart, p.d_touch_f, p.d_touch_b, redo);
		else
			hipLaunchKernelGGL(k_expect_mfma<64>, dim3(nC), dim3(64), 0, st, p.d_chunks, p.n_sub, p.d_obs, p.d_f, p.d_b, p.d_sb,
			                   p.d_re, p.d_Cpart, p.d_Epart, p.d_touch_f, p.d_touch_b, redo);
	}
}

int launch_fast(const EstepLaunch &p, FastReport *rep)
{
	if (p.n_chunks <= 0) return 0;
	(void)hipGetLastError();
	const dim3 g(p.n_chunks), b(64);
	const bool ov = p.overlap != 0;
	hipStream_t sm = p.stream, sa = ov ? p.stream2 : p.stream, sx = ov ? p.stream3 : p.stream;
	rep->fwd_rounds = rep->bwd_rounds = rep->fwd_tiles = rep->bwd_tiles = rep->merged = rep->recounted = 0;
	rep->converged = 1;
	(void)hipMemsetAsync(p.d_warm, 0, 2 * sizeof(unsigned long long), sm);
	(void)hipMemsetAsync(p.d_touch_f, 0, 3 * sizeof(int) * (size_t)p.n_chunks, sm);
	if (p.d_gate) (void)hipMemsetAsync(p.d_gate, 0, 2 * sizeof(int), sm);
	if (p.q_grid > 0) (void)hipMemsetAsync(p.d_qhead, 0, sizeof(int), sm);
	if (p.ev[0]) (void)hipEventRecord(p.ev[0], sm);
	(void)hipEventRecord(p.evx[0], sm);
	if (ov) (void)hipStreamWaitEvent(sa, p.evx[0], 0);
	const bool lw = p.structured && (p.n_long_f > 0 || p.n_long_b > 0) && (ov || p.fused);
	const bool lf = lw && p.n_long_f > 0, lb = lw && p.n_long_b > 0;
	const int ff0 = lf ? p.n_long_f : 0, fb0 = lb ? p.n_long_b : 0;
	const bool mg = p.merge1 && p.structured && p.fused && ov;
	hipStream_t sw = ov ? (mg ? sa : p.stream4) : sm, sk = ov ? p.stream5 : sm;
	if (lw) {
		if (ov && sw != sa) (void)hipStreamWaitEvent(sw, p.evx[0], 0);
		launch_walks(p, sw);
	}
	const bool gated = lw && ov && p.d_gate != nullptr && sw != sm;
	const int rw = p.lanes8 && p.ns == 64 && p.fused ? 8 : 4;
	if (gated) launch_gate(sm, p.d_gate, walk_blocks(p));
	if (mg) {
		launch_sweeps(p, sm, ff0, p.n_items_f - ff0, fb0, p.n_items_b - fb0 - p.n_B_b, true);
		if (p.merge) launch_fwd_struct(p, sm, 6, 0, p.n_fix_f);
		(void)hipEventRecord(p.evx[1], sm);
	}
	if (lw) {
		if (p.n_kc > 0) {
			if (ov) (void)hipStreamWaitEvent(sk, p.evx[0], 0);
			if (gated && sk != sm) launch_gate(sk, p.d_gate + 1, std::min(2048, mg ? (p.n_items_f - ff0 + rw - 1) / rw + (p.n_items_b - fb0 - p.n_B_b + rw - 1) / rw : (p.q_grid > 0 ? p.q_grid : (p.structured ? (p.n_items_f - ff0 + rw - 1) / rw : 0))));
			launch_kchain(p, sk, sw, p.evx[8]);
		}
		(void)hipEventRecord(p.evx[6], sw);
		if (lf) launch_fwd_struct(p, sw, 3, 0, p.n_mem_f);
		(void)hipEventRecord(p.evx[7], sw);
		if (ov) (void)hipStreamWaitEvent(sk, p.fused ? p.evx[7] : p.evx[6], 0);
		if (lb && !p.fused) launch_bwd_struct(p, sk, 3, 0, p.n_mem_b);
		if (p.fused != 2) (void)hipEventRecord(p.evx[9], sk);
	}
	const bool one = p.structured && !p.fused;
	if (mg) {
	} else if (one) {
		if (p.ev[7]) (void)hipEventRecord(p.ev[7], sm);
		launch_sweeps(p, sm, ff0, p.n_items_f - ff0, fb0, p.n_items_b - fb0, false);
		if (p.ev[6]) (void)hipEventRecord(p.ev[6], sm);
	} else if (p.q_grid > 0) launch_phase1_queue(p, sm, ff0, p.n_items_f - ff0, fb0, p.n_items_b - fb0 - p.n_B_b);
	else if (p.structured) launch_fwd_struct(p, sm, 0, ff0, p.n_items_f - ff0);
	else launch_fwd<false>(p, sm);
	if (!mg && p.merge) launch_fwd_struct(p, sm, 6, 0, p.n_fix_f);
	if (!mg) (void)hipEventRecord(p.evx[1], sm);
	if (p.merge && lf) {
		if (ov && sw != sm) (void)hipStreamWaitEvent(sw, p.evx[1], 0);
		launch_fwd_struct(p, sw, 7, 0, p.n_mem_f);
		(void)hipEventRecord(p.evx[7], sw);
	}
	if (p.ev[5]) (void)hipEventRecord(p.ev[5], sm);
	if (one && ov) (void)hipStreamWaitEvent(sa, p.evx[1], 0);
	if (!one && p.ev[7]) (void)hipEventRecord(p.ev[7], sa);
	if (p.fused) {
		if (!mg && p.q_grid <= 0) launch_bwd_struct(p, sa, 4, fb0, p.n_items_b - fb0 - p.n_B_b);
		if (p.fused == 2 && lw) {
			if (lb) { if (ov) (void)hipStreamWaitEvent(sk, p.evx[1], 0); launch_bwd_acc(p, sk, 3, 0, p.n_mem_b); }
			(void)hipEventRecord(p.evx[9], sk);
		}
		(void)hipStreamWaitEvent(sa, p.evx[1], 0);
		const bool late = p.fused == 1 && p.runs_in_b && p.n_list_b > 0;
		if (lw && ov && sw != sa && !late) (void)hipStreamWaitEvent(sa, p.evx[7], 0);
		if (p.ev[8]) (void)hipEventRecord(p.ev[8], sa);
		if (p.fused == 2) { if (p.coarse > 1) launch_bwd_acc(p, sa, 6, 0, p.n_singles_b); else launch_bwd_acc(p, sa, 0, fb0, p.n_items_b - fb0); }
		else {
			launch_bwd_count(p, sa, 0, false);
			if (p.n_list_b > 0) {
				if (lw && ov && sw != sa && late) (void)hipStreamWaitEvent(sa, p.evx[7], 0);
				(void)hipEventRecord(p.evx[11], sa);
				(void)hipEventRecord(p.evx[12], sa);
				launch_bwd_count(p, sa, 1, false);
			}
		}
		if (p.ev[9]) (void)hipEventRecord(p.ev[9], sa);
		if (p.ev[6]) (void)hipEventRecord(p.ev[6], sa);
	} else {
		if (!one) {
			if (p.structured) launch_bwd_struct(p, sa, 0, fb0, p.n_items_b - fb0);
			else launch_bwd<false>(p, sa);
			if (p.ev[6]) (void)hipEventRecord(p.ev[6], sa);
		}
		if (ov) {
			(void)hipEventRecord(p.evx[2], sa);
			(void)hipStreamWaitEvent(sx, p.evx[1], 0); (void)hipStreamWaitEvent(sx, p.evx[2], 0);
			if (lw) { (void)hipStreamWaitEvent(sx, p.evx[7], 0); (void)hipStreamWaitEvent(sx, p.evx[9], 0); }
			if (p.ev[8]) (void)hipEventRecord(p.ev[8], sx);
			launch_expect(p, sx, 0);
			if (p.ev[9]) (void)hipEventRecord(p.ev[9], sx);
			(void)hipEventRecord(p.evx[3], sx);
		}
	}
	struct Chain { hipStream_t st; hipEvent_t rb; int slot; bool bwd, done, pending; int round; };
	Chain ch[2] = {{sm, p.evx[4], 0, false, false, false, 0}, {sa, p.evx[5], 1, true, false, false, 0}};
	auto post_verify = [&](Chain &c) -> int {
		(void)hipMemsetAsync(p.d_cnt + c.slot, 0, sizeof(int), c.st);
		(void)hipMemsetAsync(p.d_warm + c.slot, 0, sizeof(unsigned long long), c.st);
#define PSMC_LV(BW, S, MINE, DIRTY, CNT) hipLaunchKernelGGL((k_verify<BW, S>), g, b, 0, c.st, p.d_chunks, p.n_chunks, p.tol, p.d_f, \
			MINE, p.d_bexit, DIRTY, CNT, p.d_warm, (BW && !p.fused) ? 1 : 0, \
			(p.m_mis && c.round == 0 && (BW || !p.merge)) ? p.m_mis + (BW ? p.n_chunks : 0) : nullptr)
		if (!c.bwd) { if (p.ns == 128) PSMC_LV(false, 128, p.d_entry, p.d_dirty, p.d_cnt); else PSMC_LV(false, 64, p.d_entry, p.d_dirty, p.d_cnt); }
		else { if (p.ns == 128) PSMC_LV(true, 128, p.d_bentry, p.d_dirty_b, p.d_cnt + 1); else PSMC_LV(true, 64, p.d_bentry, p.d_dirty_b, p.d_cnt + 1); }
#undef PSMC_LV
		launch_compact(p, c.st, c.bwd);
		if (hipEventRecord(c.rb, c.st) != hipSuccess) return -1;
		c.pending = true;
		return 0;
	};
	if (lw && ov) { if (sw != sm) (void)hipStreamWaitEvent(sm, p.evx[7], 0); (void)hipStreamWaitEvent(sa, p.evx[9], 0); }
	auto launch_ll = [&](hipStream_t st) {
		const int *fm = p.merge ? p.d_fmerge : nullptr;
		if (p.ns == 128) hipLaunchKernelGGL(k_ll<128>, g, b, 0, st, p.d_chunks, p.d_f, p.d_s, p.d_entry, p.d_LLpart, fm, p.d_finv);
		else hipLaunchKernelGGL(k_ll<64>, g, b, 0, st, p.d_chunks, p.d_f, p.d_s, p.d_entry, p.d_LLpart, fm, p.d_finv);
		PSMC_DBG("k_ll", p.n_chunks, 0, 0);
	};
	auto launch_reduce = [&](hipStream_t sm) {
		const int nS = p.n_chunks * p.n_sub, nC = p.fused == 1 ? (p.n_list_a + p.count_group - 1) / p.count_group + (p.n_list_b + p.count_group - 1) / p.count_group : nS;
		if (p.fused == 2) {
			launch_reduce_factored(p, sm);
		} else if (p.ns == 128) {
			hipLaunchKernelGGL(k_reduce1<128>, dim3(128 * 128 / 256 + 1, RED_ROWS), dim3(256), 0, sm, p.d_Cpart, p.d_Epart, nC, nS, p.d_LLpart,
			                   p.n_chunks, p.d_stage);
			hipLaunchKernelGGL(k_reduce2<128>, dim3((128 * 128 + 3 * 128 + 1 + 255) / 256), dim3(256), 0, sm, p.d_stage, p.d_a, p.d_e,
			                   p.tiny_total, p.n_states, p.d_stats);
		} else {
			hipLaunchKernelGGL(k_reduce1<64>, dim3(17, RED_ROWS), dim3(256), 0, sm, p.d_Cpart, p.d_Epart, nC, nS, p.d_LLpart,
			                   p.n_chunks, p.d_stage);
			hipLaunchKernelGGL(k_reduce2<64>, dim3((STATS_LEN + 255) / 256), dim3(256), 0, sm, p.d_stage, p.d_a, p.d_e,
			                   p.tiny_total, p.n_states, p.d_stats);
		}
		if (p.ev[4]) (void)hipEventRecord(p.ev[4], sm);
	};
	if (post_verify(ch[0]) || post_verify(ch[1])) return -1;
	static const bool recheck = getenv("PSMC_HIP_DEBUG_RECHECK") != nullptr;
	const bool optimistic = p.fused != 0 && ov && !recheck;
	if (optimistic) {
		(void)hipStreamWaitEvent(sx, p.evx[4], 0);
		launch_ll(sx);
		(void)hipEventRecord(p.evx[2], sa); (void)hipStreamWaitEvent(sx, p.evx[2], 0);
		if (p.ev[1]) (void)hipEventRecord(p.ev[1], sx);
		if (p.ev[2]) (void)hipEventRecord(p.ev[2], sx);
		if (p.ev[3]) (void)hipEventRecord(p.ev[3], sx);
		launch_reduce(sx);
		(void)hipEventRecord(p.evx[10], sx);
	}
	bool ll_stale = !optimistic;
	while (!(ch[0].done && ch[1].done)) {
		bool progressed = false;
		for (int d = 0; d < 2; ++d) {
			Chain &c = ch[d];
			if (c.done || !c.pending) continue;
			const hipError_t q = ov ? hipEventQuery(c.rb) : hipEventSynchronize(c.rb);
			if (q == hipErrorNotReady) continue;
			if (q != hipSuccess) return -1;
			c.pending = false; progressed = true;
			const int nd = p.h_cnt[c.slot];
			if (nd == 0) { c.done = true; continue; }
			if (c.round >= p.max_rounds) { rep->converged = 0; c.done = true; continue; }
			++c.round;
			if (p.structured) {
				std::vector<int> *fl = c.bwd ? p.flagged_b : p.flagged_f;
				if (fl) for (int i = 0; i < nd; ++i) fl->push_back(p.h_ritems[(size_t)c.slot * 2 * p.n_chunks + 2 * i]);
			}
			if (!c.bwd) {
				rep->fwd_rounds++; rep->fwd_tiles += nd; ll_stale = true;
				if (p.structured) launch_fwd_struct(p, c.st, 1, 0, nd); else launch_fwd<true>(p, c.st);
			} else {
				rep->bwd_rounds++; rep->bwd_tiles += nd;
				if (p.fused == 2) launch_bwd_acc(p, c.st, 1, 0, nd);
				else if (p.fused) launch_bwd_struct(p, c.st, 5, 0, nd);
				else if (p.structured) launch_bwd_struct(p, c.st, 1, 0, nd);
				else launch_bwd<true>(p, c.st);
			}
			if (post_verify(c)) return -1;
		}
		if (!progressed) __builtin_ia32_pause();
	}
	const bool repaired = rep->fwd_rounds + rep->bwd_rounds > 0;
	if (optimistic) (void)hipStreamWaitEvent(sm, p.evx[10], 0);
	if (optimistic && !repaired) return (int)hipGetLastError();
	if (hipStreamSynchronize(sm) != hipSuccess) return -1;
	if (p.ev[1]) (void)hipEventRecord(p.ev[1], sm);
	if (ll_stale) launch_ll(sm);
	if (p.fused) {
		if (ov) { (void)hipEventRecord(p.evx[2], sa); (void)hipStreamWaitEvent(sm, p.evx[2], 0); }
		if (p.ev[2]) (void)hipEventRecord(p.ev[2], sm);
		const bool recount = repaired;
		rep->recounted = recount ? 1 : 0;
		if (recount) {
			if (p.fused == 2) launch_bwd_acc(p, sm, 2, 0, p.n_chunks); else { launch_bwd_count(p, sm, 0, true); launch_bwd_count(p, sm, 1, true); }
		}
	} else if (ov) {
		(void)hipEventRecord(p.evx[2], sa); (void)hipStreamWaitEvent(sm, p.evx[2], 0);
		(void)hipStreamWaitEvent(sm, p.evx[3], 0);
		if (p.ev[2]) (void)hipEventRecord(p.ev[2], sm);
		if (repaired) launch_expect(p, sm, 1);
	} else {
		if (p.ev[2]) (void)hipEventRecord(p.ev[2], sm);
		if (p.ev[8]) (void)hipEventRecord(p.ev[8], sm);
		launch_expect(p, sm, 0);
		if (p.ev[9]) (void)hipEventRecord(p.ev[9], sm);
	}
	if (p.fused == 1 && recheck) {
		const int ga = (p.n_list_a + 3) / 4, gb = (p.n_list_b + 3) / 4, ng = ga + gb;
		const size_t gs = (size_t)p.ns * p.ns;
		std::vector<double> c0(gs * ng), c1(gs * ng);
		std::vector<int> tl(4 * (size_t)ng), tf(p.n_chunks), tb(p.n_chunks);
		std::vector<Chunk> ch(p.n_chunks);
		(void)hipDeviceSynchronize();
		(void)hipMemcpy(c0.data(), p.d_Cpart, sizeof(double) * c0.size(), hipMemcpyDeviceToHost);
		launch_bwd_count(p, sm, 0, false, true); launch_bwd_count(p, sm, 1, false, true);
		(void)hipDeviceSynchronize();
		(void)hipMemcpy(c1.data(), p.d_Cpart, sizeof(double) * c1.size(), hipMemcpyDeviceToHost);
		(void)hipMemcpy(tl.data(), p.d_ftiles, sizeof(int) * tl.size(), hipMemcpyDeviceToHost);
		(void)hipMemcpy(tf.data(), p.d_touch_f, sizeof(int) * tf.size(), hipMemcpyDeviceToHost);
		(void)hipMemcpy(tb.data(), p.d_touch_b, sizeof(int) * tb.size(), hipMemcpyDeviceToHost);
		(void)hipMemcpy(ch.data(), p.d_chunks, sizeof(Chunk) * ch.size(), hipMemcpyDeviceToHost);
		for (int g2 = 0; g2 < ng; ++g2) {
			double worst = 0.0, big = 0.0;
			for (size_t i = 0; i < gs; ++i) { big = std::max(big, std::fabs(c1[g2 * gs + i])); worst = std::max(worst, std::fabs(c0[g2 * gs + i] - c1[g2 * gs + i])); }
			if (worst > 1e-9 * big) {
				fprintf(stderr, "[psmc_hip] RECHECK group %d (list %c) differs by %.2e of %.2e; rounds %d/%d; tiles:", g2, g2 < ga ? 'A' : 'B', worst, big, rep->fwd_rounds, rep->bwd_rounds);
				for (int r = 0; r < 4; ++r) {
					const int en = tl[4 * (size_t)g2 + r];
					if (en < 0) { fprintf(stderr, " -"); continue; }
					const int t = en & ~(1 << 30);
// ... 14 lines not shown
```

psmc_amd/csrc/estep_fused.hip:

```cpp
#include <hip/hip_runtime.h>
#include "wave_prims.h"
#include "struct_prims.h"
#include <type_traits>
#include "psmc_hip_internal.h"

namespace psmc {

#ifdef PSMC_NO_SB
#define PSMC_SB
#else
#define PSMC_SB __builtin_amdgcn_sched_barrier(0);
#endif

typedef double d4f_t __attribute__((ext_vector_type(4)));
constexpr int NPLF = 4, SF = 64;

__device__ __forceinline__ int64_t readlane_i64f(int64_t v, int lane) {
	const unsigned lo = (unsigned)__builtin_amdgcn_readlane((int)(unsigned)v, lane);
	const unsigned hi = (unsigned)__builtin_amdgcn_readlane((int)(unsigned)((unsigned long long)v >> 32), lane);
	return (int64_t)(((unsigned long long)hi << 32) | lo);
}

template <bool NORM, bool MASKED>
__device__ __forceinline__ void count4f_step(const StructParN<NPLF> &sc, const double *lds_e, const double *lds_m, int k0, int sym,
                                             const double (&X)[NPLF], double (&x)[NPLF], bool active, double inv, double &rho,
                                             double (&FA)[NPLF], double (&FB)[NPLF], double (&S)[2][NPLF])
{
	double ev[NPLF], y[NPLF];
	ev_load<NPLF>(lds_e + sym * SF, k0, ev);
	const d2v_t mk = *reinterpret_cast<const d2v_t *>(lds_m + 2 * sym);
	double rho_next = rho;
	if (NORM) {
		const double tot = row_sum16((x[0] + x[1]) + (x[2] + x[3]));
		const double sb = rcp_newton(tot);
#pragma unroll
		for (int i = 0; i < NPLF; ++i) ev[i] *= sb;
		rho_next = rho * (inv * tot);
		if (MASKED) rho_next = active ? rho_next : rho;
	}
#pragma unroll
	for (int i = 0; i < NPLF; ++i) y[i] = x[i];
	struct_step<NPLF>(sc, y);
#pragma unroll
	for (int i = 0; i < NPLF; ++i) {
		FA[i] = rho * X[i];
		if (MASKED) FA[i] = active ? FA[i] : 0.0;
		const double gk = MASKED ? (active ? FA[i] * y[i] : 0.0) : FA[i] * y[i];
		S[0][i] = __builtin_fma(gk, mk.x, S[0][i]);
		S[1][i] = __builtin_fma(gk, mk.y, S[1][i]);
		FB[i] = MASKED ? (active ? x[i] : 0.0) : x[i];
		const double nb = y[i] * ev[i];
		x[i] = MASKED ? (active ? nb : x[i]) : nb;
	}
	rho = rho_next;
}
__device__ __forceinline__ void count4f_mfma(const double (&FA)[NPLF], const double (&FB)[NPLF], d4f_t (&acc)[4][4])
{
#pragma unroll
	for (int j = 0; j < 4; ++j)
#pragma unroll
		for (int j2 = 0; j2 < 4; ++j2) acc[j][j2] = __builtin_amdgcn_mfma_f64_16x16x4f64(FA[j], FB[j2], acc[j][j2], 0, 0, 0);
}
#ifdef PSMC_TRACE_SWEEP
__device__ unsigned long long g_trace_c[4 * 8192];
#endif
__global__ __launch_bounds__(64, 1) void k_bwd_count4f_struct(const double *__restrict__ sp, const double *__restrict__ e,
                                                                const double *__restrict__ invd, const uint8_t *__restrict__ obs,
                                                                const Chunk *__restrict__ chunks, const int *__restrict__ tiles,
                                                                int group0, int mode, const double *__restrict__ f,
                                                                double *__restrict__ bentry, double *__restrict__ bexit,
                                                                double *__restrict__ Cpart,
                                                                double *__restrict__ Epart, const int *__restrict__ touch_f,
                                                                const int *__restrict__ touch_b, const int *__restrict__ fmerge, const double *__restrict__ finv)
{
	__shared__ double lds_e[4 * SF], lds_m[8];
	const int lane = threadIdx.x, row = lane >> 4, m = lane & 15, k0 = NPLF * m;
	{ const int q = ev_slot<NPLF>(lane); lds_e[q] = e[lane]; lds_e[SF + q] = e[SF + lane]; lds_e[2 * SF + q] = 1.0; lds_e[3 * SF + q] = 1.0; }
	if (lane < 8) lds_m[lane] = (lane == 0 || lane == 3) ? 1.0 : 0.0;
	__syncthreads();
	const int group = group0 + blockIdx.x;
#ifdef PSMC_TRACE_SWEEP
	struct TraceC { int g; unsigned long long w0, c0; __device__ ~TraceC() { if (threadIdx.x == 0 && g < 8192) { g_trace_c[4 * g] = w0; g_trace_c[4 * g + 1] = __builtin_readcyclecounter() - c0; g_trace_c[4 * g + 2] = wall_clock64(); } } }
		trace_c{group, (unsigned long long)wall_clock64(), (unsigned long long)__builtin_readcyclecounter()};
#endif
	const int entry = tiles[4 * blockIdx.x + row];
	const bool valid = entry >= 0, from_above = valid && mode == 0 && (entry & (1 << 30)) != 0;
	const int tile = valid ? (entry & ~(1 << 30)) : 0;
	if (mode == 2 && !__any(valid && (touch_f[tile] | touch_b[tile]) != 0)) return;
	const Chunk c = chunks[tile];
	const int L = c.L, lo = c.lo, top = min(c.hi, L - 1);
	const bool work = valid && top >= lo;
	const double *fo = f + c.off * SF + k0;
	const double *io = invd + c.off;
	StructParN<NPLF> sc;
	loadN<NPLF>(sp + 3 * SF + k0, sc.mS); loadN<NPLF>(sp + SF + k0, sc.wS);
	loadN<NPLF>(sp + 2 * SF + k0, sc.mP); loadN<NPLF>(sp + k0, sc.wP); loadN<NPLF>(sp + 4 * SF + k0, sc.dd);
	double x[NPLF];
	loadN<NPLF>((from_above ? bexit + (int64_t)(tile + 1) * SF : bentry + (int64_t)tile * SF) + k0, x);
	if (from_above) storeN<NPLF>(bentry + (int64_t)tile * SF + k0, x);
	const int p_min = lo, p_max = max(top, lo);
	const int g_hi = work ? (top - 1) >> 2 : -1, g_lo = work ? (lo - 1) >> 2 : 0;
	const int ng = g_hi - g_lo + 1;
	const int64_t off0 = readlane_i64f(c.off, 0), off1 = readlane_i64f(c.off, 16), off2 = readlane_i64f(c.off, 32), off3 = readlane_i64f(c.off, 48);
	const int gh0 = __builtin_amdgcn_readlane(g_hi, 0), gh1 = __builtin_amdgcn_readlane(g_hi, 16), gh2 = __builtin_amdgcn_readlane(g_hi, 32), gh3 = __builtin_amdgcn_readlane(g_hi, 48);
	const int n0 = __builtin_amdgcn_readlane(ng, 0), n1 = __builtin_amdgcn_readlane(ng, 16), n2 = __builtin_amdgcn_readlane(ng, 32), n3 = __builtin_amdgcn_readlane(ng, 48);
	const int ng_max = max(max(n0, n1), max(n2, n3));
	int g_merge = -1;
	double rho_fix = 1.0;
	if (fmerge != nullptr && work) {
		const int bm = fmerge[tile];
		if (bm > 0 && lo + 16 * bm - 1 < p_max) { g_merge = (lo + 16 * bm - 2) >> 2; rho_fix = finv[tile]; }
	}
	double rho;
	{
		double y[NPLF], Xt[NPLF];
		loadN<NPLF>(fo + (int64_t)(p_max - 1) * SF, Xt);
#pragma unroll
		for (int i = 0; i < NPLF; ++i) y[i] = x[i];
		struct_step<NPLF>(sc, y);
		const double I = row_sum16((Xt[0] * y[0] + Xt[1] * y[1]) + (Xt[2] * y[2] + Xt[3] * y[3]));
		rho = work ? (double)c.mult * rcp_newton(I) : 0.0;
	}
	d4f_t acc[4][4];
	double S[2][NPLF];
#pragma unroll
	for (int j = 0; j < 4; ++j) {
#pragma unroll
		for (int j2 = 0; j2 < 4; ++j2) acc[j][j2] = (d4f_t){0.0, 0.0, 0.0, 0.0};
		S[0][j] = S[1][j] = 0.0;
	}
	auto load_row = [&](int g, int j, double (&Xq)[NPLF]) {
		const int p = min(max(4 * g + j + 1, p_min), p_max);
		loadN<NPLF>(fo + (int64_t)(p - 1) * SF, Xq);
	};
	auto load_inv = [&](int g) {
		return io[min(max(4 * g + 4, p_min), p_max) - 1];
	};
	double Xg[4][NPLF];
#pragma unroll
	for (int j = 0; j < 4; ++j) load_row(max(g_hi, 0), j, Xg[j]);
	double inv_cur = load_inv(max(g_hi, 0));
	int gi = 0;
	struct Words { unsigned w0, w1, w2, w3; };
	auto load_words = [&](int gi_) {
		Words q;
		const uint8_t *p0 = obs + off0 + 4 * (int64_t)max(gh0 - min(gi_, max(n0 - 1, 0)), 0);
		const uint8_t *p1 = obs + off1 + 4 * (int64_t)max(gh1 - min(gi_, max(n1 - 1, 0)), 0);
		const uint8_t *p2 = obs + off2 + 4 * (int64_t)max(gh2 - min(gi_, max(n2 - 1, 0)), 0);
		const uint8_t *p3 = obs + off3 + 4 * (int64_t)max(gh3 - min(gi_, max(n3 - 1, 0)), 0);
		asm volatile("s_load_dword %0, %4, 0x0\n\ts_load_dword %1, %5, 0x0\n\ts_load_dword %2, %6, 0x0\n\ts_load_dword %3, %7, 0x0"
		             : "=&s"(q.w0), "=&s"(q.w1), "=&s"(q.w2), "=&s"(q.w3) : "s"(p0), "s"(p1), "s"(p2), "s"(p3) : "memory");
		return q;
	};
	auto select_word = [&](Words q) {
		asm volatile("s_waitcnt lgkmcnt(0)" : "+s"(q.w0), "+s"(q.w1), "+s"(q.w2), "+s"(q.w3));
		return row == 0 ? q.w0 : (row == 1 ? q.w1 : (row == 2 ? q.w2 : q.w3));
	};
	unsigned w_cur = select_word(load_words(0));
	auto all_full = [&](int gi_) {
		const int g = max(g_hi - gi_, g_lo);
		return __all(gi_ < ng && 4 * g + 1 >= lo && 4 * g + 4 <= top) != 0;
	};
	auto do_group = [&](auto masked_tag) {
		constexpr bool MASKED = decltype(masked_tag)::value;
		const unsigned w = w_cur;
		const Words wn = load_words(gi + 1);
		__builtin_amdgcn_sched_barrier(0);
		const int g = max(g_hi - gi, g_lo);
		const bool in_tile = gi < ng;
		const int s3 = (int)((w >> 24) & 3u), s2 = (int)((w >> 16) & 3u), s1 = (int)((w >> 8) & 3u), s0 = (int)(w & 3u);
		const int pb = 4 * g + 1;
		const double inv = inv_cur;
		rho = (in_tile && g == g_merge) ? rho * rho_fix : rho;
		double FAn[NPLF], FBn[NPLF];
#define PSMC_C4F(NORM, J, SYM)                                                                                                   \
		count4f_step<NORM, MASKED>(sc, lds_e, lds_m, k0, SYM, Xg[J], x, in_tile && pb + J <= top && pb + J >= lo, inv, rho, FAn, FBn, S); \
		count4f_mfma(FAn, FBn, acc);                                                                                        \
		load_row(g - 1, J, Xg[J]);                                                                                          \
		if (J == 3) inv_cur = load_inv(g - 1);                                                                              \
		__builtin_amdgcn_sched_barrier(0);
		PSMC_C4F(true, 3, s3) PSMC_C4F(false, 2, s2) PSMC_C4F(false, 1, s1) PSMC_C4F(false, 0, s0)
#undef PSMC_C4F
		if (in_tile && g == g_lo) storeN<NPLF>(bexit + (int64_t)tile * SF + k0, x);
		w_cur = select_word(wn);
	};
	for (; gi < ng_max && !all_full(gi); ++gi) do_group(std::true_type{});
	for (; gi < ng_max && all_full(gi); ++gi) do_group(std::false_type{});
	for (; gi < ng_max; ++gi) do_group(std::true_type{});
	asm volatile("s_nop 15\n\ts_nop 15\n\ts_nop 15"
	             : "+a"(acc[0][0]), "+a"(acc[0][1]), "+a"(acc[0][2]), "+a"(acc[0][3]), "+a"(acc[1][0]), "+a"(acc[1][1]), "+a"(acc[1][2]),
	               "+a"(acc[1][3]), "+a"(acc[2][0]), "+a"(acc[2][1]), "+a"(acc[2][2]), "+a"(acc[2][3]), "+a"(acc[3][0]), "+a"(acc[3][1]),
	               "+a"(acc[3][2]), "+a"(acc[3][3]));
	double *out = Cpart + (int64_t)group * (SF * SF);
#pragma unroll
	for (int j = 0; j < 4; ++j)
#pragma unroll
		for (int r = 0; r < 4; ++r) {
			const double v[NPLF] = {acc[j][0][r], acc[j][1][r], acc[j][2][r], acc[j][3][r]};
			storeN<NPLF>(out + (4 * (row + 4 * r) + j) * SF + k0, v);
		}
	if (valid) {
		double *os = Epart + (int64_t)tile * (3 * SF) + k0;
		const double zero[NPLF] = {0.0, 0.0, 0.0, 0.0};
		storeN<NPLF>(os, S[0]); storeN<NPLF>(os + SF, S[1]); storeN<NPLF>(os + 2 * SF, zero);
	}
}

constexpr int NPL8 = 8, S8 = 128;
constexpr int G8X = 16;
__device__ __forceinline__ void load8p(const d2v_t *v, int m, double (&out)[NPL8]) {
#pragma unroll
	for (int p = 0; p < 4; ++p) { const d2v_t t = v[16 * p + m]; out[2 * p] = t.x; out[2 * p + 1] = t.y; }
}
__device__ __forceinline__ void fill8p(d2v_t *v, int k, double val) { reinterpret_cast<double *>(v + 16 * ((k & 7) >> 1) + (k >> 3))[k & 1] = val; }
__device__ __forceinline__ void struct_step8_lds(const d2v_t *lds_sc, int m, double (&x)[NPL8])
{
	double cS[NPL8], cP[NPL8], su[NPL8], pv[NPL8];
	load8p(lds_sc, m, cS); load8p(lds_sc + 2 * 64, m, cP);
	su[NPL8 - 1] = x[NPL8 - 1] * cS[NPL8 - 1];
#pragma unroll
	for (int i = NPL8 - 2; i >= 0; --i) su[i] = __builtin_fma(x[i], cS[i], su[i + 1]);
	pv[0] = x[0] * cP[0];
#pragma unroll
	for (int i = 1; i < NPL8; ++i) pv[i] = __builtin_fma(x[i], cP[i], pv[i - 1]);
	const double ES = row_excl_suffix(su[0]), EP = row_excl_prefix(pv[NPL8 - 1]);
	double wS[NPL8], wP[NPL8], dd[NPL8];
	load8p(lds_sc + 64, m, wS); load8p(lds_sc + 3 * 64, m, wP); load8p(lds_sc + 4 * 64, m, dd);
#pragma unroll
	for (int i = 0; i < NPL8; ++i) {
		const double t = __builtin_fma(wS[i], su[i], __builtin_fma(wP[i], pv[i], dd[i] * x[i]));
		x[i] = __builtin_fma(wS[i], ES, __builtin_fma(wP[i], EP, t));
	}
}
template <bool NORM, bool MASKED>
__device__ __forceinline__ void count8x_step(const d2v_t *lds_sc, const d2v_t *lds_e, const double *lds_m, int m, int sym,
                                             const double (&X)[NPL8], double (&x)[NPL8], bool active, double inv, double &rho,
                                             double (&FA)[NPL8], double (&FB)[NPL8], double (&S)[2][NPL8])
{
	double ev[NPL8], y[NPL8];
	load8p(lds_e + sym * 64, m, ev);
	const d2v_t mk = *reinterpret_cast<const d2v_t *>(lds_m + 2 * sym);
	double rho_next = rho;
	if (NORM) {
		double t = 0.0;
#pragma unroll
		for (int i = 0; i < NPL8; ++i) t += x[i];
		const double tot = row_sum16(t);
		const double sb = rcp_newton(tot);
#pragma unroll
		for (int i = 0; i < NPL8; ++i) ev[i] *= sb;
		rho_next = rho * (inv * tot);
		if (MASKED) rho_next = active ? rho_next : rho;
	}
#pragma unroll
	for (int i = 0; i < NPL8; ++i) y[i] = x[i];
	struct_step8_lds(lds_sc, m, y);
#pragma unroll
	for (int i = 0; i < NPL8; ++i) {
		FA[i] = rho * X[i];
		if (MASKED) FA[i] = active ? FA[i] : 0.0;
		const double gk = MASKED ? (active ? FA[i] * y[i] : 0.0) : FA[i] * y[i];
		S[0][i] = __builtin_fma(gk, mk.x, S[0][i]);
		S[1][i] = __builtin_fma(gk, mk.y, S[1][i]);
		FB[i] = MASKED ? (active ? x[i] : 0.0) : x[i];
		const double nb = y[i] * ev[i];
		x[i] = MASKED ? (active ? nb : x[i]) : nb;
	}
	rho = rho_next;
}

__global__ __launch_bounds__(256, 1) void k_bwd_count8x_struct(const double *__restrict__ sp, const double *__restrict__ e,
                                                                 const double *__restrict__ invd, const uint8_t *__restrict__ obs,
                                                                 const Chunk *__restrict__ chunks, const int *__restrict__ tiles,
                                                                 int group0, int mode, const double *__restrict__ f,
                                                                 double *__restrict__ bentry, double *__restrict__ bexit,
                                                                 double *__restrict__ Cpart,
                                                                 double *__restrict__ Epart, const int *__restrict__ touch_f,
                                                                 const int *__restrict__ touch_b)
{
	__shared__ d2v_t lds_e[4 * 64];
	__shared__ double lds_m[8];
	__shared__ d2v_t xa[2][4][4][64], xb[2][4][4][64];
	__shared__ int lds_ng[4];
	__shared__ d2v_t lds_sc[5 * 64];
	const int tid = threadIdx.x, lane = tid & 63, row = lane >> 4, m = lane & 15, k0 = NPL8 * m;
	const int w = __builtin_amdgcn_readfirstlane(tid >> 6);
	if (tid < S8) {
		fill8p(lds_e, tid, e[tid]); fill8p(lds_e + 64, tid, e[S8 + tid]); fill8p(lds_e + 2 * 64, tid, 1.0); fill8p(lds_e + 3 * 64, tid, 1.0);
		fill8p(lds_sc, tid, sp[3 * S8 + tid]); fill8p(lds_sc + 64, tid, sp[S8 + tid]); fill8p(lds_sc + 2 * 64, tid, sp[2 * S8 + tid]);
		fill8p(lds_sc + 3 * 64, tid, sp[tid]); fill8p(lds_sc + 4 * 64, tid, sp[4 * S8 + tid]);
	}
	if (tid < 8) lds_m[tid] = (tid == 0 || tid == 3) ? 1.0 : 0.0;
	__syncthreads();
	const int group = group0 + blockIdx.x;
	const int entry = tiles[G8X * blockIdx.x + 4 * w + row];
	const bool valid = entry >= 0, from_above = valid && mode == 0 && (entry & (1 << 30)) != 0;
	const int tile = valid ? (entry & ~(1 << 30)) : 0;
	if (mode == 2 && !__syncthreads_or(valid && (touch_f[tile] | touch_b[tile]) != 0)) return;
	const Chunk c = chunks[tile];
	const int L = c.L, lo = c.lo, top = min(c.hi, L - 1);
	const bool work = valid && top >= lo;
	const double *fo = f + c.off * S8 + k0;
	const double *io = invd + c.off;
	double x[NPL8];
	loadN<NPL8>((from_above ? bexit + (int64_t)(tile + 1) * S8 : bentry + (int64_t)tile * S8) + k0, x);
	if (from_above) storeN<NPL8>(bentry + (int64_t)tile * S8 + k0, x);
	const int p_min = lo, p_max = max(top, lo);
	double rho;
	{
		double y[NPL8], Xt[NPL8];
		loadN<NPL8>(fo + (int64_t)(p_max - 1) * S8, Xt);
#pragma unroll
		for (int i = 0; i < NPL8; ++i) y[i] = x[i];
		struct_step8_lds(lds_sc, m, y);
		double t = 0.0;
#pragma unroll
		for (int i = 0; i < NPL8; ++i) t = __builtin_fma(Xt[i], y[i], t);
		rho = work ? (double)c.mult * rcp_newton(row_sum16(t)) : 0.0;
	}
	d4f_t acc[2][NPL8];
	double S[2][NPL8];
#pragma unroll
	for (int j2 = 0; j2 < NPL8; ++j2) {
		acc[0][j2] = (d4f_t){0.0, 0.0, 0.0, 0.0}; acc[1][j2] = (d4f_t){0.0, 0.0, 0.0, 0.0};
		S[0][j2] = S[1][j2] = 0.0;
	}
	const int g_hi = work ? (top - 1) >> 2 : -1, g_lo = work ? (lo - 1) >> 2 : 0;
	const int ng = g_hi - g_lo + 1;
	const int64_t off0 = readlane_i64f(c.off, 0), off1 = readlane_i64f(c.off, 16), off2 = readlane_i64f(c.off, 32), off3 = readlane_i64f(c.off, 48);
	const int gh0 = __builtin_amdgcn_readlane(g_hi, 0), gh1 = __builtin_amdgcn_readlane(g_hi, 16), gh2 = __builtin_amdgcn_readlane(g_hi, 32), gh3 = __builtin_amdgcn_readlane(g_hi, 48);
	const int n0 = __builtin_amdgcn_readlane(ng, 0), n1 = __builtin_amdgcn_readlane(ng, 16), n2 = __builtin_amdgcn_readlane(ng, 32), n3 = __builtin_amdgcn_readlane(ng, 48);
	if (lane == 0) lds_ng[w] = max(max(n0, n1), max(n2, n3));
	__syncthreads();
	const int ng_max = max(max(lds_ng[0], lds_ng[1]), max(lds_ng[2], lds_ng[3]));
	auto row_pos = [&](int g, int j) { return min(max(4 * g + j + 1, p_min), p_max); };
	auto load_inv = [&](int g) { return io[min(max(4 * g + 4, p_min), p_max) - 1]; };
	double Xa[NPL8], Xb[NPL8];
	loadN<NPL8>(fo + (int64_t)(row_pos(max(g_hi, 0), 3) - 1) * S8, Xa);
	double inv_cur = load_inv(max(g_hi, 0));
	auto all_full = [&](int gi_) {
		const int g = max(g_hi - gi_, g_lo);
		return __all(gi_ < ng && 4 * g + 1 >= lo && 4 * g + 4 <= top) != 0;
	};
	int gi = 0, par = 0;
	auto exchange = [&](const double (&FA)[NPL8], const double (&FB)[NPL8]) {
#pragma unroll
		for (int p = 0; p < 4; ++p) {
			d2v_t u, v; u.x = FA[2 * p]; u.y = FA[2 * p + 1]; v.x = FB[2 * p]; v.y = FB[2 * p + 1];
			xa[par][w][p][lane] = u; xb[par][w][p][lane] = v;
		}
		__syncthreads();
		d2v_t oa[2], ob[2][4];
		oa[0] = xa[par][0][w][lane];
#pragma unroll
		for (int p = 0; p < 4; ++p) ob[0][p] = xb[par][0][p][lane];
#pragma unroll
		for (int g = 0; g < 4; ++g) {
			if (g < 3) {
				oa[(g + 1) & 1] = xa[par][g + 1][w][lane];
#pragma unroll
				for (int p = 0; p < 4; ++p) ob[(g + 1) & 1][p] = xb[par][g + 1][p][lane];
			}
			__builtin_amdgcn_sched_barrier(0);
			const d2v_t a = oa[g & 1];
			const double B[NPL8] = {ob[g & 1][0].x, ob[g & 1][0].y, ob[g & 1][1].x, ob[g & 1][1].y, ob[g & 1][2].x, ob[g & 1][2].y, ob[g & 1][3].x, ob[g & 1][3].y};
#pragma unroll
			for (int j2 = 0; j2 < NPL8; ++j2) {
				acc[0][j2] = __builtin_amdgcn_mfma_f64_16x16x4f64(a.x, B[j2], acc[0][j2], 0, 0, 0);
				acc[1][j2] = __builtin_amdgcn_mfma_f64_16x16x4f64(a.y, B[j2], acc[1][j2], 0, 0, 0);
			}
			__builtin_amdgcn_sched_barrier(0);
		}
		par ^= 1;
	};
	auto do_group = [&](auto masked_tag) {
		constexpr bool MASKED = decltype(masked_tag)::value;
		const unsigned w0 = *reinterpret_cast<const unsigned *>(obs + off0 + 4 * (int64_t)max(gh0 - min(gi, max(n0 - 1, 0)), 0));
		const unsigned w1 = *reinterpret_cast<const unsigned *>(obs + off1 + 4 * (int64_t)max(gh1 - min(gi, max(n1 - 1, 0)), 0));
		const unsigned w2 = *reinterpret_cast<const unsigned *>(obs + off2 + 4 * (int64_t)max(gh2 - min(gi, max(n2 - 1, 0)), 0));
		const unsigned w3 = *reinterpret_cast<const unsigned *>(obs + off3 + 4 * (int64_t)max(gh3 - min(gi, max(n3 - 1, 0)), 0));
		const unsigned ww = row == 0 ? w0 : (row == 1 ? w1 : (row == 2 ? w2 : w3));
		const int g = max(g_hi - gi, g_lo);
		const bool in_tile = gi < ng;
		const int s3 = (int)((ww >> 24) & 3u), s2 = (int)((ww >> 16) & 3u), s1 = (int)((ww >> 8) & 3u), s0 = (int)(ww & 3u);
		const int pb = 4 * g + 1;
		const double inv = inv_cur;
		double FA[NPL8], FB[NPL8];
#define PSMC_C8X(NORM, J, SYM, XC, XN, GN, JN)                                                                                   \
		loadN<NPL8>(fo + (int64_t)(row_pos(GN, JN) - 1) * S8, XN);                                                          \
		count8x_step<NORM, MASKED>(lds_sc, lds_e, lds_m, m, SYM, XC, x, in_tile && pb + J <= top && pb + J >= lo, inv, rho, FA, FB, S); \
		if (J == 3) inv_cur = load_inv(g - 1);                                                                               \
		exchange(FA, FB);
		PSMC_C8X(true, 3, s3, Xa, Xb, g, 2) PSMC_C8X(false, 2, s2, Xb, Xa, g, 1) PSMC_C8X(false, 1, s1, Xa, Xb, g, 0) PSMC_C8X(false, 0, s0, Xb, Xa, g - 1, 3)
#undef PSMC_C8X
		if (in_tile && g == g_lo) storeN<NPL8>(bexit + (int64_t)tile * S8 + k0, x);
	};
	for (; gi < ng_max && !all_full(gi); ++gi) do_group(std::true_type{});
	for (; gi < ng_max && all_full(gi); ++gi) do_group(std::false_type{});
	for (; gi < ng_max; ++gi) do_group(std::true_type{});
	asm volatile("s_nop 15\n\ts_nop 15\n\ts_nop 15"
	             : "+a"(acc[0][0]), "+a"(acc[0][1]), "+a"(acc[0][2]), "+a"(acc[0][3]), "+a"(acc[0][4]), "+a"(acc[0][5]), "+a"(acc[0][6]),
	               "+a"(acc[0][7]), "+a"(acc[1][0]), "+a"(acc[1][1]), "+a"(acc[1][2]), "+a"(acc[1][3]), "+a"(acc[1][4]), "+a"(acc[1][5]),
	               "+a"(acc[1][6]), "+a"(acc[1][7]));
	double *out = Cpart + (int64_t)group * (S8 * S8);
#pragma unroll
	for (int jj = 0; jj < 2; ++jj)
#pragma unroll
		for (int r = 0; r < 4; ++r) {
			double v[NPL8];
#pragma unroll
			for (int j2 = 0; j2 < NPL8; ++j2) v[j2] = acc[jj][j2][r];
			storeN<NPL8>(out + (int64_t)(8 * (row + 4 * r) + 2 * w + jj) * S8 + k0, v);
		}
	if (valid) {
		double *os = Epart + (int64_t)tile * (3 * S8) + k0;
		const double zero[NPL8] = {0.0, 0.0, 0.0, 0.0, 0.0, 0.0, 0.0, 0.0};
		storeN<NPL8>(os, S[0]); storeN<NPL8>(os + S8, S[1]); storeN<NPL8>(os + 2 * S8, zero);
	}
}

void launch_bwd_count(const EstepLaunch &p, hipStream_t st, int list, bool redo, bool all_from_bentry)
{
	const int G = p.count_group;
	const int ga = (p.n_list_a + G - 1) / G, gb = (p.n_list_b + G - 1) / G;
	const int n_groups = list == 0 ? ga : gb;
	if (n_groups <= 0) return;
	const int *tl = p.d_ftiles + (list == 0 ? 0 : G * ga);
	const int g0 = list == 0 ? 0 : ga, md = all_from_bentry ? 3 : (redo ? 2 : 0);
	if (p.ns == 128) {
		hipLaunchKernelGGL(k_bwd_count8x_struct, dim3(n_groups), dim3(256), 0, st, p.d_sp, p.d_e, p.d_s, p.d_obs, p.d_chunks, tl, g0, md,
		                   p.d_f, p.d_bentry, p.d_bexit, p.d_Cpart, p.d_Epart, p.d_touch_f, p.d_touch_b);
		PSMC_DBG("launch_bwd_count (128 states)", list, redo, n_groups);
		return;
	}
	hipLaunchKernelGGL(k_bwd_count4f_struct, dim3(n_groups), dim3(64), 0, st, p.d_sp, p.d_e, p.d_s, p.d_obs, p.d_chunks, tl, g0, md,
	                   p.d_f, p.d_bentry, p.d_bexit, p.d_Cpart, p.d_Epart, p.d_touch_f, p.d_touch_b, p.merge ? p.d_fmerge : nullptr, p.d_finv);
	PSMC_DBG("launch_bwd_count", list, redo, n_groups);
}

}

#ifdef PSMC_TRACE_SWEEP
extern "C" int psmc_hip_debug_trace_counts(unsigned long long *out, int n)
{
	if (n > 8192) n = 8192;
	return (int)hipMemcpyFromSymbol(out, HIP_SYMBOL(psmc::g_trace_c), sizeof(unsigned long long) * 4 * n);
}
#endif
```

psmc_amd/csrc/estep_struct.hip:

```cpp
#include <hip/hip_runtime.h>
#include "wave_prims.h"
#include "struct_prims.h"
#include "psmc_hip_internal.h"

namespace psmc {

#ifdef PSMC_TRACE_SWEEP
__device__ unsigned long long g_trace_f[4 * 16384], g_trace_b[4 * 16384], g_trace_w[4 * 16384];
__device__ __forceinline__ void trace_put(unsigned long long *t, int block, int slot, unsigned long long v) {
	if ((threadIdx.x & 63) == 0 && block < 16384) t[4 * block + slot] = v;
}
__device__ __forceinline__ unsigned long long trace_hw() {
	const unsigned hw = __builtin_amdgcn_s_getreg((31 << 11) | (0 << 6) | 4), xcc = __builtin_amdgcn_s_getreg((31 << 11) | (0 << 6) | 20);
	return (unsigned long long)hw | ((unsigned long long)(xcc & 0xf) << 32);
}
#define PSMC_TRACE(t, block, slot, v) trace_put(t, block, slot, v)
#else
#define PSMC_TRACE(t, block, slot, v) ((void)0)
#endif

template <int J> __device__ __forceinline__ int sym_of(unsigned w) { return (int)((w >> (8 * J)) & 3u); }
__device__ __forceinline__ unsigned sym_word(const uint4 sv, int g) { return g == 0 ? sv.x : (g == 1 ? sv.y : (g == 2 ? sv.z : sv.w)); }
__device__ __forceinline__ int64_t readlane_i64(int64_t v, int lane) {
	const unsigned lo = (unsigned)__builtin_amdgcn_readlane((int)(unsigned)v, lane);
// ... 767 lines not shown
#pragma unroll
			for (int h = 0; h < PER; ++h) y[h] = __builtin_fma(v, m[i][h], y[h]);
		}
		double (*pp)[S] = part[j & 1];
#pragma unroll
		for (int h = 0; h < PER; ++h) pp[w][lane + 64 * h] = y[h];
		__syncthreads();
#pragma unroll
		for (int h = 0; h < PER; ++h) {
			double tsum = pp[0][lane + 64 * h];
#pragma unroll
			for (int v = 1; v < NW; ++v) tsum += pp[v][lane + 64 * h];
			y[h] = tsum;
		}
		double tot = y[0];
		if constexpr (PER == 2) tot += y[1];
		const double inv = rcp_newton(first_lane_f64(wave_sum_nat(tot)));
#pragma unroll
		for (int h = 0; h < PER; ++h) x[h] = y[h] * inv;
	};
	auto tile_done = [&]() {
		double y[PER];
#pragma unroll
		for (int h = 0; h < PER; ++h) y[h] = x[h];
		if (!fwd) {
			const Chunk c = chunks[t];
			const int top = min(c.hi, c.L - 1), ps = min((c.lo + 3) & ~3, top);
			const uint8_t *o = obs + c.off;
			for (int pq = ps; pq >= c.lo; --pq) {
				const int sym = (int)o[pq - 1] & 3;
				double ev[PER];
#pragma unroll
				for (int h = 0; h < PER; ++h) ev[h] = walk_ev(sym, e0[h], e1[h]);
				if ((pq & 3) == 0) {
					double tot = y[0];
					if constexpr (PER == 2) tot += y[1];
					const double inv = rcp_newton(first_lane_f64(wave_sum_nat(tot)));
#pragma unroll
					for (int h = 0; h < PER; ++h) ev[h] *= inv;
				}
				struct_step1n<PER>(s1, y, wm);
#pragma unroll
				for (int h = 0; h < PER; ++h) y[h] *= ev[h];
			}
		}
		t += fwd ? 1 : -1;
#pragma unroll
		for (int h = 0; h < PER; ++h) { if (w == 0) vec[(int64_t)t * S + lane + 64 * h] = y[h]; x[h] = y[h]; }
	};
	if (n_mats > 0) load(0, ma, ea);
	for (int j = 0; j < n_mats; j += 2) {
		if (j + 1 < n_mats) load(j + 1, mb, eb);
		product(j, ma, ea);
		if (j % sub == sub - 1) tile_done();
		if (j + 1 >= n_mats) break;
		if (j + 2 < n_mats) load(j + 2, ma, ea);
		product(j + 1, mb, eb);
		if ((j + 1) % sub == sub - 1) tile_done();
	}
}

template <int NPL, bool CK, int LPT = 16>
__global__ __launch_bounds__(64) void k_sweep_struct(const double *__restrict__ sp, const double *__restrict__ e,
                                                       const double *__restrict__ a0, const uint8_t *__restrict__ obs,
                                                       const Chunk *__restrict__ chunks, const SweepItem *__restrict__ items_f,
                                                       int n_f, const SweepItem *__restrict__ items_b, int n_b, int W, int T,
                                                       int flags_f, int flags_b, double *__restrict__ f, double *__restrict__ invd,
                                                       double *__restrict__ entry, double *__restrict__ bt,
                                                       double *__restrict__ sb, double *__restrict__ bentry,
                                                       double *__restrict__ bexit, int *__restrict__ started, const double *__restrict__ prevx)
{
	announce_start(started);
	constexpr int R = 64 / LPT;
	const int nbf = (n_f + R - 1) / R, nbb = (n_b + R - 1) / R, both = 2 * min(nbf, nbb), b = blockIdx.x;
	bool fwd; int blk;
	if (!(flags_b & SWEEP_ALTERNATE)) { fwd = b < nbf; blk = fwd ? b : b - nbf; }
	else if (b < both) { fwd = (b & 1) == 0; blk = b >> 1; }
	else { fwd = nbf > nbb; blk = b - both + min(nbf, nbb); }
	if (fwd) fwd_struct_body<false, NPL, CK, LPT>(blk, sp, e, a0, obs, chunks, items_f, n_f, W, T, flags_f, f, invd, entry, nullptr, FwdCtl{prevx, 0.0, nullptr, nullptr, nullptr, nullptr});
	else bwd_struct_body<false, NPL, LPT>(blk, sp, e, obs, chunks, items_b, n_b, W, T, flags_b, bt, sb, bentry, bexit, nullptr);
}

__global__ __launch_bounds__(64) void k_compact(const int *__restrict__ dirty, int n, SweepItem *__restrict__ out,
                                                  SweepItem *__restrict__ host_out, int *__restrict__ host_cnt)
{
	const int lane = threadIdx.x;
	int base = 0;
	for (int i0 = 0; i0 < n; i0 += 64) {
		const int i = i0 + lane;
		const bool d = i < n && dirty[i] != 0;
		const unsigned long long mask = __ballot(d);
		if (d) {
			SweepItem s; s.first = i; s.count = 1;
			const int at = base + __popcll(mask & ((1ull << lane) - 1ull));
			out[at] = s;
			if (host_out) host_out[at] = s;
		}
		base += __popcll(mask);
	}
	if (lane == 0) *host_cnt = base;
	__threadfence_system();
}

void launch_fwd_struct(const EstepLaunch &p, hipStream_t st, int which, int first, int n_items)
{
	if (n_items <= 0) return;
	const bool l8 = p.lanes8 && p.ns == 64 && which == 0;
	const dim3 g(l8 ? (n_items + 7) / 8 : (n_items + 3) / 4), b(64);
	const SweepItem *items = (const SweepItem *)(which == 1 ? p.d_ritems_f : (which == 3 || which == 7 ? p.d_members_f : (which == 6 ? p.d_fix_f : p.d_items_f))) + first;
	const bool fixp = which == 6 || which == 7;
	const int flags = (which == 3 ? (SWEEP_FROM_ENTRY | SWEEP_NO_TOUCH) : 0)
	                  | (p.ckpt ? SWEEP_CKPT : 0) | (which == 0 && p.coarse > 1 ? SWEEP_COARSE : 0) | (fixp ? SWEEP_MERGE : 0);
	const FwdCtl ctl = {which == 0 ? p.d_prevx : nullptr, p.tol, fixp ? p.m_mis : nullptr, fixp ? p.m_mlen : nullptr, p.d_fmerge, p.d_finv};
#define PSMC_LF(REP, NPL, CK) hipLaunchKernelGGL((k_fwd_struct<REP, NPL, CK>), g, b, 0, st, p.d_sp, p.d_e, p.d_a0, p.d_obs, p.d_chunks, \
		items, n_items, p.warmup, p.tile_len, flags, p.d_f, p.d_s, p.d_entry, p.d_touch_f, which == 0 && p.d_gate ? p.d_gate + 1 : nullptr, ctl)
	const bool rep = which != 0;
	if (l8) {
#define PSMC_LF8(CK) hipLaunchKernelGGL((k_fwd_struct<false, 8, CK, 8>), g, b, 0, st, p.d_sp, p.d_e, p.d_a0, p.d_obs, p.d_chunks, \
		items, n_items, p.warmup, p.tile_len, flags, p.d_f, p.d_s, p.d_entry, p.d_touch_f, p.d_gate ? p.d_gate + 1 : nullptr, ctl)
		if (p.ckpt) PSMC_LF8(true); else PSMC_LF8(false);
#undef PSMC_LF8
	} else if (p.ns == 128) { if (rep) PSMC_LF(true, 8, false); else PSMC_LF(false, 8, false); }
	else if (p.ckpt) { if (rep) PSMC_LF(true, 4, true); else PSMC_LF(false, 4, true); }
	else { if (rep) PSMC_LF(true, 4, false); else PSMC_LF(false, 4, false); }
	PSMC_DBG("launch_fwd_struct", which, first, n_items);
#undef PSMC_LF
}
void launch_bwd_struct(const EstepLaunch &p, hipStream_t st, int which, int first, int n_items)
{
	if (n_items <= 0) return;
	const bool l8 = p.lanes8 && p.ns == 64 && which == 4;
	const dim3 g(l8 ? (n_items + 7) / 8 : (n_items + 3) / 4), b(64);
	const SweepItem *items = (const SweepItem *)(which == 1 || which == 5 ? p.d_ritems_b : (which == 3 ? p.d_members_b : p.d_items_b)) + first;
	const int flags = which == 5 ? SWEEP_WALK : (which == 3 ? (SWEEP_FROM_ENTRY | SWEEP_NO_TOUCH) : (which == 4 ? (p.coarse > 1 ? (SWEEP_WALK | SWEEP_COARSE) : SWEEP_TOP_ONLY) : 0));
#define PSMC_LB(REP, NPL) hipLaunchKernelGGL((k_bwd_struct<REP, NPL>), g, b, 0, st, p.d_sp, p.d_e, p.d_obs, p.d_chunks, items, \
		n_items, p.warmup, p.tile_len, flags, p.d_b, p.d_sb, p.d_bentry, p.d_bexit, p.d_touch_b)
	const bool rep = !(which == 0 || which == 4);
	if (l8)
		hipLaunchKernelGGL((k_bwd_struct<false, 8, 8>), g, b, 0, st, p.d_sp, p.d_e, p.d_obs, p.d_chunks, items, n_items, p.warmup, p.tile_len, flags,
		                   p.d_b, p.d_sb, p.d_bentry, p.d_bexit, p.d_touch_b);
	else if (p.ns == 128) { if (rep) PSMC_LB(true, 8); else PSMC_LB(false, 8); }
	else { if (rep) PSMC_LB(true, 4); else PSMC_LB(false, 4); }
	PSMC_DBG("launch_bwd_struct", which, first, n_items);
#undef PSMC_LB
}
void launch_phase1_queue(const EstepLaunch &p, hipStream_t st, int ff, int nf, int fb, int nb)
{
	if (p.n_queue <= 0 || p.q_grid <= 0) return;
	const int flags_f = (p.ckpt ? SWEEP_CKPT : 0) | (p.coarse > 1 ? SWEEP_COARSE : 0);
	const int flags_b = p.coarse > 1 ? (SWEEP_WALK | SWEEP_COARSE) : SWEEP_TOP_ONLY;
	const FwdCtl ctl = {p.d_prevx, p.tol, nullptr, nullptr, p.d_fmerge, p.d_finv};
#define PSMC_LQ(CK) hipLaunchKernelGGL(k_phase1_queue<CK>, dim3(p.q_grid), dim3(64), 0, st, p.d_sp, p.d_e, p.d_a0, p.d_obs, p.d_chunks, \
		(const SweepItem *)p.d_items_f + ff, nf, (const SweepItem *)p.d_items_b + fb, nb, p.warmup, p.tile_len, flags_f, flags_b, p.d_f, p.d_s, \
		p.d_entry, p.d_b, p.d_sb, p.d_bentry, p.d_bexit, p.d_touch_f, p.d_touch_b, p.d_queue, p.n_queue, p.d_qhead, p.d_gate ? p.d_gate + 1 : nullptr, ctl)
	if (p.ckpt) PSMC_LQ(true); else PSMC_LQ(false);
#undef PSMC_LQ
	PSMC_DBG("launch_phase1_queue", nf, nb, p.q_grid);
}
void launch_compact(const EstepLaunch &p, hipStream_t st, bool bwd)
{
	hipLaunchKernelGGL(k_compact, dim3(1), dim3(64), 0, st, bwd ? p.d_dirty_b : p.d_dirty, p.n_chunks,
	                   (SweepItem *)(bwd ? p.d_ritems_b : p.d_ritems_f),
	                   (SweepItem *)(p.m_ritems ? p.m_ritems + (size_t)(bwd ? 1 : 0) * 2 * p.n_chunks : nullptr), p.m_cnt + (bwd ? 1 : 0));
	PSMC_DBG("verify + launch_compact", bwd, p.n_chunks, 0);
}
void launch_sweeps(const EstepLaunch &p, hipStream_t st, int ff, int nf, int fb, int nb, bool top_only)
{
	const bool l8 = p.lanes8 && p.ns == 64 && top_only;
	const int nblk = l8 ? (nf + 7) / 8 + (nb + 7) / 8 : (nf + 3) / 4 + (nb + 3) / 4;
	if (nblk <= 0) return;
	const int co = top_only && p.coarse > 1 ? SWEEP_COARSE : 0;
	const int flags_f = (p.ckpt ? SWEEP_CKPT : 0) | co,
	          flags_b = (top_only ? (co ? SWEEP_WALK | co : SWEEP_TOP_ONLY) : 0) | (top_only && p.merge_order ? SWEEP_MERGED : SWEEP_ALTERNATE);
#define PSMC_LS(NPL, CK) hipLaunchKernelGGL((k_sweep_struct<NPL, CK>), dim3(nblk), dim3(64), 0, st, p.d_sp, p.d_e, p.d_a0, p.d_obs, p.d_chunks, \
		(const SweepItem *)p.d_items_f + ff, nf, (const SweepItem *)p.d_items_b + fb, nb, p.warmup, p.tile_len, flags_f, flags_b, \
		p.d_f, p.d_s, p.d_entry, p.d_b, p.d_sb, p.d_bentry, p.d_bexit, p.d_gate ? p.d_gate + 1 : nullptr, p.d_prevx)
#define PSMC_LS8(CK) hipLaunchKernelGGL((k_sweep_struct<8, CK, 8>), dim3(nblk), dim3(64), 0, st, p.d_sp, p.d_e, p.d_a0, p.d_obs, p.d_chunks, \
		(const SweepItem *)p.d_items_f + ff, nf, (const SweepItem *)p.d_items_b + fb, nb, p.warmup, p.tile_len, flags_f, flags_b, \
		p.d_f, p.d_s, p.d_entry, p.d_b, p.d_sb, p.d_bentry, p.d_bexit, p.d_gate ? p.d_gate + 1 : nullptr, p.d_prevx)
	if (l8) { if (p.ckpt) PSMC_LS8(true); else PSMC_LS8(false); }
	else if (p.ns == 128) PSMC_LS(8, false); else if (p.ckpt) PSMC_LS(4, true); else PSMC_LS(4, false);
#undef PSMC_LS8
	PSMC_DBG("launch_sweeps", nf, nb, top_only);
#undef PSMC_LS
}
__global__ __launch_bounds__(64) void k_gather_prev(const Chunk *__restrict__ chunks, const SweepItem *__restrict__ items, int S, const double *__restrict__ f,
                                                      const double *__restrict__ a0, double *__restrict__ prevx, int ck)
{
	const SweepItem it = items[blockIdx.x];
	const Chunk c = chunks[it.first];
	const int ws = max(1, c.lo - c.wf);
	const bool have = ws > 1 && !(ck && ((ws - 1) & 7));
	for (int k = threadIdx.x; k < S; k += 64) {
		double v = a0[k];
		if (have) { const double t = f[(c.off + ws - 2) * S + k]; v = (t > 0.0 && t < 1e300) ? t : v; }
		prevx[(int64_t)it.first * S + k] = v;
	}
}
void launch_gather_prev(const EstepLaunch &p, hipStream_t st, int first, int n_items, double *prevx)
{
	if (n_items <= 0) return;
	hipLaunchKernelGGL(k_gather_prev, dim3(n_items), dim3(64), 0, st, p.d_chunks, (const SweepItem *)p.d_items_f + first, p.ns, p.d_f, p.d_a0, prevx, p.ckpt);
}

__global__ __launch_bounds__(64) void k_tile_allmiss(const uint8_t *__restrict__ obs, const Chunk *__restrict__ chunks, int *__restrict__ flags)
{
	const Chunk c = chunks[blockIdx.x];
	const uint8_t *o = obs + c.off;
	int bad = 0;
	for (int p = c.lo + (int)threadIdx.x; p <= c.hi; p += 64) bad |= ((int)o[p - 1] & 3) != 2;
	const int any_bad = __any(bad);
	if (threadIdx.x == 0) flags[blockIdx.x] = any_bad ? 0 : 1;
}
int launch_tile_allmiss(hipStream_t st, const uint8_t *d_obs, const Chunk *d_chunks, int n_chunks, int *d_flags)
{
	if (n_chunks <= 0) return 0;
	hipLaunchKernelGGL(k_tile_allmiss, dim3(n_chunks), dim3(64), 0, st, d_obs, d_chunks, d_flags);
	return (int)hipGetLastError();
}

void launch_kchain(const EstepLaunch &p, hipStream_t st_cols, hipStream_t st_chain, hipEvent_t ev_cols)
{
	if (p.n_kc <= 0) return;
	if (p.ns == 128)
		hipLaunchKernelGGL(k_kcol_struct<8>, dim3(p.n_kuniq * 32), dim3(64), 0, st_cols, p.d_sp, p.d_e, p.d_obs, p.d_chunks,
		                   (const KcTile *)p.d_kc, p.d_kuniq, p.d_Kcol, p.d_Kexp);
	else
		hipLaunchKernelGGL(k_kcol2_struct<2>, dim3(p.n_kuniq * p.kc_sub), dim3(128), 0, st_cols, p.d_kcc, p.d_obs, p.d_chunks, (const KcTile *)p.d_kc, p.d_kuniq,
		                   p.d_Kcol, p.d_Kexp, p.kc_sub, p.kcol_prio);
	if (st_cols != st_chain) { (void)hipEventRecord(ev_cols, st_cols); (void)hipStreamWaitEvent(st_chain, ev_cols, 0); }
	if (p.ns == 128)
		hipLaunchKernelGGL(k_kchain_struct<2>, dim3(p.n_chain_f + p.n_chain_b), dim3(512), 0, st_chain, (const KcRun *)p.d_kruns, p.n_chain_f, p.d_kslot,
		                   p.d_Kcol, p.d_Kexp, p.d_sp, p.d_e, p.d_obs, p.d_chunks, p.d_entry, p.d_bentry, p.kc_sub);
	else
		hipLaunchKernelGGL(k_kchain_struct<1>, dim3(p.n_chain_f + p.n_chain_b), dim3(128), 0, st_chain, (const KcRun *)p.d_kruns, p.n_chain_f, p.d_kslot,
		                   p.d_Kcol, p.d_Kexp, p.d_sp, p.d_e, p.d_obs, p.d_chunks, p.d_entry, p.d_bentry, p.kc_sub);
	PSMC_DBG("launch_kchain", p.n_kc, p.n_chain_f, p.n_chain_b);
}
int walk_blocks(const EstepLaunch &p) { return p.ns == 64 ? p.n_wl_f + p.n_wl_b : (p.n_wl_f + 3) / 4 + (p.n_wl_b + 3) / 4; }
void launch_walks(const EstepLaunch &p, hipStream_t st)
{
	if (p.n_wl_f + p.n_wl_b <= 0) return;
	if (p.ns == 64) {
		hipLaunchKernelGGL(k_walk1_struct, dim3(p.n_wl_f + p.n_wl_b), dim3(64), 0, st, p.d_sp, p.d_e, p.d_a0, p.d_obs, p.d_chunks,
		                   (const SweepItem *)p.d_wl_f, p.n_wl_f, (const SweepItem *)p.d_wl_b, p.n_wl_b, p.warmup,
		                   p.tile_len, p.d_entry, p.d_bentry, p.d_bexit, p.d_gate);
// ... 21 lines not shown
```

psmc_amd/csrc/psmc_hip_ctx.h:

```cpp
#pragma once
#include <hip/hip_runtime.h>
#include <math.h>
#include <stdio.h>
#include <stdlib.h>
#include <string.h>
#include <algorithm>
#include <atomic>
#include <chrono>
#include <string>
#include <thread>
#include <vector>
#include "psmc_hip.h"
#include "psmc_hip_internal.h"

using namespace psmc;

#define HMM_TINY_H 1e-25

constexpr int DEC_NONE = 0;
constexpr int DEC_FAST = 1;
constexpr int DEC_EXACT = 2;
constexpr int DEC_NO_BT = 3;
constexpr int DEC_MERGED = 4;
constexpr int DEC_WIDE = 5;
// ... 29 lines not shown
	size_t queue_cap = 0; int n_queue = 0;
	int coarse = -1;
	int coarse_used = 1, items_coarse = -1;
	bool warm_shift_set = false, kc_sub_set = false;
	int warm_shift_used = 1, kc_sub_used = 4;
	int kc_div = 16;
	int kc_min = -1;
	int n_wl_f = 0, n_wl_b = 0, n_kc = 0, n_chain_f = 0, n_chain_b = 0, n_singles_b = 0;
	double *d_Kcol = nullptr; size_t kcol_cap = 0;
	hipStream_t stream5 = nullptr;
	int ckpt = 1;
	int fuse = 1;
	int fuse128 = 2;
	int count_group = 4;
	int merge = 0;
	int adapt = 0;
	int prev_start = 0;
	int *h_mlen = nullptr, *m_mlen = nullptr;
	double *h_mis = nullptr, *m_mis = nullptr;
	double *d_prevx = nullptr, *d_finv = nullptr;
	std::vector<int> order_f;
	int n_fix_f = 0;
	bool merge_used = false;
	Chunk *h_chunks = nullptr; size_t h_chunks_cap = 0;
	bool prev_ok = false;
	unsigned long long prev_serial = 0, tab_serial = 0;
	const double *prev_f = nullptr; int prev_ckpt = 0;
	int learn = 1;
	int warm_shift = 1;
	bool chunks_dirty = false;
	int group_cap = 131072;
	int *d_items = nullptr;
	int *h_ritems = nullptr;
	int *m_ritems = nullptr, *m_cnt = nullptr;
	std::vector<uint8_t> glue_f, glue_b;
	std::vector<uint8_t> gap;
	int gap_tiles = 1;
	int n_kuniq = 0;
	std::vector<int> flagged_f, flagged_b;
	bool items_dirty = true;
	int n_items_f = 0, n_items_b = 0;
	int n_sub_used = 6;
	int n_seg = 0;
	std::vector<int32_t> L;
	std::vector<int64_t> off;
	int64_t total = 0;
	bool obs_borrowed = false;
	uint8_t *d_obs = nullptr;
	int64_t *d_seg_off = nullptr;
	int32_t *d_seg_len = nullptr;
	std::vector<int32_t> sel;
	std::vector<int32_t> work;
	std::vector<int32_t> sel2work;
	std::vector<int32_t> mult;
	int32_t *d_work = nullptr;
	bool plan_dirty = true;
	double *h_par = nullptr, *d_par = nullptr;
	size_t par_len = 0;
	static constexpr size_t PAR_LEN = 2 * 16384 + 3 * 128 + 128 + 3 * 128 + 5 * 128 + 2 * 11 * 128;
	static constexpr size_t RE128_OFF = 2 * 16384 + 3 * 128 + 128, SP128_OFF = RE128_OFF + 3 * 128, KCC128_OFF = SP128_OFF + 5 * 128;
	static constexpr size_t SP_OFF = 4 * 4096 + 192 + 64 + 192;
	static constexpr size_t KCC_OFF = SP_OFF + 5 * 64;
	double *d_f = nullptr, *d_b = nullptr, *d_s = nullptr, *d_sb = nullptr;
	int64_t tab_bins = 0; bool have_b = false;
	double *d_segA = nullptr, *d_segE = nullptr, *d_segA0 = nullptr, *d_chk = nullptr;
	int seg_cap = 0;
	std::vector<double> h_segA, h_segE, h_segA0, h_chk, h_s;
	std::vector<Chunk> chunks;
	Chunk *d_chunks = nullptr;
	int chunk_cap = 0, chunk_used = 0;
	double *d_entry = nullptr, *d_bentry = nullptr, *d_bexit = nullptr, *d_Cpart = nullptr, *d_Epart = nullptr,
	       *d_LLpart = nullptr;
	size_t cpart_cap = 0;
	int *d_dirty = nullptr, *d_cnt = nullptr, *h_cnt = nullptr, *d_touch = nullptr;
	hipStream_t stream2 = nullptr, stream3 = nullptr, stream4 = nullptr;
	hipEvent_t evx[14] = {nullptr, nullptr, nullptr, nullptr, nullptr, nullptr, nullptr, nullptr, nullptr, nullptr, nullptr, nullptr, nullptr, nullptr};
	bool timing_two_launches = false;
	int n_long_f = 0, n_long_b = 0, n_mem_f = 0, n_mem_b = 0;
	int n_B_b = 0, n_list_a = 0, n_list_b = 0;
	int items_two_phase = -1;
	int runs_late = 1;
	bool runs_in_b = false;
	int *d_ftiles = nullptr;
	FastReport report = {0, 0, 0, 0, 1, 0, 0};
	double *d_stage = nullptr, *d_stats = nullptr;
	unsigned long long *d_warm = nullptr;
	double warm_err[2] = {0, 0};
	hipStream_t stream = nullptr;
	hipEvent_t ev[10] = {nullptr, nullptr, nullptr, nullptr, nullptr, nullptr, nullptr, nullptr, nullptr, nullptr};
	double last_ms[7] = {0, 0, 0, 0, 0, 0, 0};
	bool timing_valid = false;
	int64_t batch_bins = 0;
	int exact_refwd = -1;
	int32_t *d_bw_seg = nullptr, *d_bw_par = nullptr; int64_t *d_bw_tab = nullptr; size_t bw_cap = 0;
	double *d_bpar = nullptr; size_t bpar_cap = 0;
	int *d_cu_mask = nullptr;
	double *d_lkp = nullptr; size_t lkp_cap = 0; std::vector<double> h_lkp;
	int64_t *d_lkoff = nullptr; size_t lkoff_cap = 0;
	double *d_s_all = nullptr; size_t s_all_cap = 0;
	int batch_sort = 1;
	int batch_tailfill = 1;
	int batch_major = 1;
	int batch_first = 0;
	double *d_b2 = nullptr; int64_t b2_bins = 0, b2_alloc = 0;
	int64_t reserved_cap = 0;
	int reserved_refwd = -1;
	int cu_first = 0, cu_count = 0;
	int last_batch_groups = 0;
	bool tables_batch = false;
	psmc_hip_ctx *x_twin = nullptr;
	int n_exact_fallbacks = 0;
	psmc_hip_ctx *parent = nullptr;
	std::vector<psmc_hip_ctx *> kids;
	int share_learn = 1;
	int share_T = 0;
	std::vector<std::vector<uint8_t>> sh_glue_f, sh_glue_b;
	std::vector<std::vector<int32_t>> sh_wf, sh_wb;
	std::vector<int32_t> chunk_seg, chunk_idx;
	double dbg_acc[8] = {0, 0, 0, 0, 0, 0, 0, 0};
	int wide_fast = 0;
	bool wf_ran = false;
	std::vector<Chunk> wf_chunks;
	Chunk *d_wf_chunks = nullptr;
	int wf_cap = 0, wf_T = 0, wf_W = 0;
	bool warmup_set = false;
	double *d_wf_X = nullptr, *d_wf_inv = nullptr; int64_t wf_bins = 0;
	double *d_wf_par = nullptr, *h_wf_par = nullptr;
	double *d_wf_entry = nullptr, *d_wf_bentry = nullptr, *d_wf_bexit = nullptr, *d_wf_part = nullptr, *d_wf_ll = nullptr;
	int *d_wf_dirty = nullptr, *d_wf_list = nullptr;
	int wide_decode = 0;
	int wd_kind = 0; unsigned long long wd_serial = 0, wd_sel = 0, sel_serial = 0;
};
inline double dbg_now() { return std::chrono::duration<double>(std::chrono::steady_clock::now().time_since_epoch()).count(); }
inline psmc_hip_ctx *dbg_root(psmc_hip_ctx *c) { return c->parent ? c->parent : c; }

inline int fail(psmc_hip_ctx *c, int code, const char *what, hipError_t e = hipSuccess)
{
	if (c) {
		c->err = what;
		if (e != hipSuccess) { c->err += ": "; c->err += hipGetErrorString(e); }
	}
	return code;
}
#define HIPCHK(c, call)                                                     \
	do {                                                                    \
		hipError_t e__ = (call);                                            \
		if (e__ != hipSuccess) return fail((c), PSMC_HIP_EDEVICE, #call, e__); \
	} while (0)

template <class T> inline int dev_alloc(psmc_hip_ctx *c, T **p, size_t n)
{
	if (*p) { (void)hipFree(*p); *p = nullptr; }
	if (n == 0) n = 1;
	hipError_t e = hipMalloc((void **)p, n * sizeof(T));
	if (e != hipSuccess) { *p = nullptr; return fail(c, PSMC_HIP_ENOMEM, "hipMalloc", e); }
	static const char *poison = getenv("PSMC_HIP_POISON");
	static int poison_count = 0;
	if (poison) {
		(void)hipMemset(*p, strcmp(poison, "vary") == 0 ? 0x3B + (poison_count++ % 8) : 0xFF, n * sizeof(T));
		(void)hipDeviceSynchronize();
	}
	return 0;
}

int  set_segments_common(psmc_hip_ctx *c, int n_seg, const int32_t *L);
bool fill_params(const psmc_hip_ctx *c, const double *a, const double *e, const double *a0, double *dst);
// ... 20 lines not shown
```

psmc_amd/csrc/psmc_hip_internal.h:

```cpp
#pragma once
#include <cstdio>
#include <cstdlib>
#include <hip/hip_runtime.h>
#include <stdint.h>
#include <vector>

namespace psmc {

constexpr int NS = 64;
constexpr int NORM_EVERY = 4;
constexpr int STATS_LEN = NS * NS + 3 * NS + 1;

struct Chunk {
	int64_t off;
	int32_t L;
	int32_t lo;
	int32_t hi;
	int32_t mult;
	int32_t flags;
	int32_t wf, wb;
};
__host__ __device__ inline int chunk_warm_f(const Chunk &c, int) { return c.wf; }
__host__ __device__ inline int chunk_warm_b(const Chunk &c, int) { return c.wb; }
constexpr int CHUNK_ANCHOR_F = 1;
constexpr int CHUNK_ANCHOR_B = 2;
constexpr int CHUNK_LAST = 4;

struct ExWork {
	const int32_t *seg;
	const int32_t *par;
	const int64_t *tab;
	const int64_t *tab_s;
	int n;
	int64_t par_stride;
};

struct FastReport { int fwd_rounds, bwd_rounds, fwd_tiles, bwd_tiles, converged, merged, recounted; };

struct EstepLaunch {
	hipStream_t stream, stream2, stream3;
	hipEvent_t evx[14];
	int overlap;
	int rep_impl, n_states;
	const int64_t *d_work_tab_s;
	int *d_cu_mask = nullptr;
	int exact_only;
	int exact_refwd;
	int ns;
	const double *d_a;
	const double *d_aeT;
	const double *d_e;
	const double *d_a0;
	const double *d_re;
	const double *d_sp;
	int structured;
	const double *d_kcc;
	int kc_sub;
	int kcol_prio;
	int fused;
	int ckpt;
	int merge_order;
	int merge1;
	const int *d_items_f, *d_items_b;
	int n_items_f, n_items_b, tile_len;
	int n_long_f, n_long_b;
	const int *d_members_f, *d_members_b;
	int n_mem_f, n_mem_b;
	int lanes8;
	int *d_gate;
	const int *d_queue; int n_queue;
	int q_grid; int *d_qhead;
	int coarse;
	const int *d_singles_b; int n_singles_b;
	int n_B_b;
	const int *d_ftiles; int n_list_a, n_list_b;
	int count_group;
	int runs_in_b;
	hipStream_t stream4, stream5;
	const int *d_wl_f, *d_wl_b; int n_wl_f, n_wl_b;
	const int *d_kc, *d_kruns; int n_kc, n_chain_f, n_chain_b;
	const int *d_kslot, *d_kuniq; int n_kuniq;
	double *d_Kcol, *d_Kexp;
	int *d_ritems_f, *d_ritems_b;
	int *h_ritems;
	int *m_ritems, *m_cnt;
	std::vector<int> *flagged_f, *flagged_b;
	const uint8_t *d_obs;
	const int64_t *d_seg_off;
	const int32_t *d_seg_len;
	const int32_t *d_work;
	int n_work;
	const int32_t *d_work_par; const int64_t *d_work_tab; int64_t par_stride; int work_align;
	double *d_f, *d_b, *d_s;
	double *d_segA, *d_segE, *d_segA0, *d_chk;
	const Chunk *d_chunks;
	int n_chunks, warmup, n_sub;
	double *d_entry, *d_bentry, *d_bexit;
	int *d_dirty, *d_dirty_b, *d_cnt, *h_cnt;
	int *d_touch_f, *d_touch_b;
	int merge;
	const int *d_fix_f; int n_fix_f;
	int *d_fmerge;
	double *d_finv;
	int *m_mlen, *h_mlen;
	double *m_mis;
	const double *d_prevx;
	double *d_sb;
	double tol; int max_rounds;
	double *d_Cpart;
	double *d_Epart;
	double *d_LLpart;
	double *d_stage;
	double *d_stats;
	unsigned long long *d_warm;
	double tiny_total;
	hipEvent_t ev[10];
};

inline bool dbg_sync_on() { static const bool on = getenv("PSMC_HIP_DEBUG_SYNC") != nullptr; return on; }
#define PSMC_DBG(NAME, A, B, C) do { if (psmc::dbg_sync_on()) { hipError_t e_ = hipDeviceSynchronize(); \
	fprintf(stderr, "[psmc_hip] %s(%d, %d, %d): %s\n", NAME, (int)(A), (int)(B), (int)(C), hipGetErrorString(e_)); fflush(stderr); } } while (0)

constexpr int RED_ROWS = 64;

int launch_exact(const EstepLaunch &p);
constexpr int LKP_DIV = 16, LKP_MIN = 64;
int launch_lk_products(hipStream_t st, const EstepLaunch &p, const double *d_s, const int64_t *d_lk_off, double *d_out);
int launch_exact_wide(const EstepLaunch &p);
int launch_post_decode_wide(hipStream_t st, const double *f, const double *b, const double *s, int64_t off, int L, int n, int S, int32_t *path, double *maxp);
int launch_post_full_wide(hipStream_t st, const double *a, const double *e, const uint8_t *obs, const double *f, const double *b, const double *s,
                          int64_t off, int L, int n, int S, double *post, double *recomb);
int launch_post_counts_wide(hipStream_t st, const double *f, const double *b, const double *s, int64_t off, int min_l, const int32_t *cnt1,
                            int n_cnt, int n, int S, double *cnt);
int launch_fast(const EstepLaunch &p, FastReport *rep);
void launch_fwd_struct(const EstepLaunch &p, hipStream_t st, int which, int first, int n_items);
void launch_bwd_struct(const EstepLaunch &p, hipStream_t st, int which, int first, int n_items);
void launch_compact(const EstepLaunch &p, hipStream_t st, bool bwd);
void launch_gather_prev(const EstepLaunch &p, hipStream_t st, int first, int n_items, double *prevx);
int launch_tile_allmiss(hipStream_t st, const uint8_t *d_obs, const Chunk *d_chunks, int n_chunks, int *d_flags);
void launch_walks(const EstepLaunch &p, hipStream_t st);
void launch_gate(hipStream_t st, const int *ctr, int want);
int walk_blocks(const EstepLaunch &p);
void launch_kchain(const EstepLaunch &p, hipStream_t st_cols, hipStream_t st_chain, hipEvent_t ev_cols);
void launch_sweeps(const EstepLaunch &p, hipStream_t st, int ff, int nf, int fb, int nb, bool top_only);
void launch_phase1_queue(const EstepLaunch &p, hipStream_t st, int ff, int nf, int fb, int nb);
void launch_bwd_count(const EstepLaunch &p, hipStream_t st, int list, bool redo, bool all_from_bentry = false);
void launch_bwd_acc(const EstepLaunch &p, hipStream_t st, int which, int first, int n);
void launch_reduce_factored(const EstepLaunch &p, hipStream_t st);
int launch_post_decode(hipStream_t st, const double *f, const double *b, const double *s, int64_t off, int L, int n,
                       int ns, int32_t *path, double *maxp);
int launch_post_full(hipStream_t st, const double *a, const double *e, const uint8_t *obs, const double *f, const double *b,
                     const double *s, int64_t off, int L, int n, int ns, double *post, double *recomb);
int launch_post_counts(hipStream_t st, const double *f, const double *b, const double *s, int64_t off, int min_l,
                       const int32_t *cnt1, int n_cnt, int n, int ns, double *cnt);
int launch_post_fast(hipStream_t st, const double *f, const double *b, const double *sb, const double *re, const double *a,
                     const uint8_t *obs, int64_t off, int L, int n, int ns, double *post, double *recomb, int32_t *path, double *maxp);
int launch_scales_fast(hipStream_t st, const double *f, const double *invd, const double *entry, const double *a0, const double *e,
                       const uint8_t *obs, int64_t off, int L, int T, int first, int ns, double *s);
int post_counts_fast_blocks(int min_l);
int launch_post_counts_fast(hipStream_t st, const double *f, const double *b, const double *re, const uint8_t *obs, int64_t off,
                            int L, int min_l, const int32_t *cnt1, int n_cnt, int n, int ns, double *part, double *cnt);
int run_selftest(hipStream_t stream, unsigned *d_flags);
int run_microbench(hipStream_t stream, double *d_out);
int run_pipe_probe(hipStream_t stream, double *d_out, int n_waves, unsigned mask, int rounds);
int run_pipe_probe2(hipStream_t stream, double *d_out, const int *kinds8, int rounds, const void *gsrc);
int run_place_probe(hipStream_t stream, double *d_out, int n_waves, int wpb, int steps);
int run_stream_probe(hipStream_t stream, const double *src, double *dst, size_t n);
int run_hbm_probe(hipStream_t stream, int which, double *a, double *b, size_t bytes);
int run_load_probe(hipStream_t stream, double *d_out, int n_waves, int steps);
int run_load_probe_st(hipStream_t stream, double *d_out, int n_waves, int steps, double *tbl, int store_steps, int mode);

}
```

Measured before the change: 2.500 billion bins/s.

## Fuse backward verify into count kernel tail and split reduction early

Adds a tail-verify step inside the fused backward count kernels, so that tiles whose speculative boundary can be checked there are verified in-kernel. A per-tile cover table lets the standalone verify kernel skip those tiles, and compact exits early when the dirty count is zero. The reduction is split so that list-A partials are summed as soon as list A finishes, overlapping with list B, and the row-sum loops are unrolled with several loads in flight. This adds complexity to the count kernels (register pressure, extra branches), which could slow the main sweep.

```diff
diff --git a/psmc_amd/csrc/api.hip b/psmc_amd/csrc/api.hip
--- a/psmc_amd/csrc/api.hip
+++ b/psmc_amd/csrc/api.hip
@@ -199,6 +199,7 @@
 	else if (k == "merge1") { if (v < -1 || v > 1) return PSMC_HIP_EINVAL; c->merge1 = (int)v; c->plan_dirty = true; }
 	else if (k == "phase1") { if (v < -1 || v > 1) return PSMC_HIP_EINVAL; c->phase1 = (int)v; }
 	else if (k == "phase1_waves") { if (v < 1 || v > 4) return PSMC_HIP_EINVAL; c->phase1_waves = (int)v; }
+	else if (k == "tail") { if (v != 0 && v != 1) return PSMC_HIP_EINVAL; c->tail = (int)v; }
 	else if (k == "lanes8") { if (v < -1 || v > 1) return PSMC_HIP_EINVAL; c->lanes8 = (int)v; }
 	else if (k == "gap_tiles") { c->gap_tiles = v != 0 ? 1 : 0; c->plan_dirty = true; c->items_dirty = true; }
 	else if (k == "coarse") { if (v < -1 || v > 16) return PSMC_HIP_EINVAL; c->coarse = (int)v; c->plan_dirty = true; c->items_dirty = true; }
diff --git a/psmc_amd/csrc/api_batch.hip b/psmc_amd/csrc/api_batch.hip
--- a/psmc_amd/csrc/api_batch.hip
+++ b/psmc_amd/csrc/api_batch.hip
@@ -405,6 +405,7 @@
 		k->learn = c->learn; k->group_cap = c->group_cap; k->warm_shift = c->warm_shift; k->kc_sub = c->kc_sub; k->kcol_prio = c->kcol_prio;
 		k->fuse128 = c->fuse128; k->coarse = c->coarse; k->gate = c->gate; k->lanes8 = c->lanes8; k->gap_tiles = c->gap_tiles; k->exact_refwd = c->exact_refwd;
 		k->merge = c->merge; k->adapt = c->adapt; k->prev_start = c->prev_start;
+		k->tail = 0;
 		k->merge1 = c->merge1; k->merge_order = c->merge_order; k->runs_late = c->runs_late; k->warm_shift_set = c->warm_shift_set; k->kc_sub_set = c->kc_sub_set;
 		k->stream = c->stream; k->stream2 = c->stream2; k->stream3 = c->stream3; k->stream4 = c->stream4; k->stream5 = c->stream5;
 		for (int i = 0; i < 14; ++i) k->evx[i] = c->evx[i];
diff --git a/psmc_amd/csrc/api_fast.hip b/psmc_amd/csrc/api_fast.hip
--- a/psmc_amd/csrc/api_fast.hip
+++ b/psmc_amd/csrc/api_fast.hip
@@ -93,7 +93,8 @@
 			return fail(c, PSMC_HIP_ENOMEM, "hipHostMalloc (mapped)");
 		if ((rc = dev_alloc(c, &c->d_LLpart, (size_t)nc))) return rc;
 		if ((rc = dev_alloc(c, &c->d_items, (size_t)32 * nc + 64))) return rc;
-		if ((rc = dev_alloc(c, &c->d_ftiles, (size_t)2 * (nc + 16)))) return rc;
+		if ((rc = dev_alloc(c, &c->d_ftiles, (size_t)3 * (nc + 16)))) return rc;
+		c->vcover_off = (size_t)2 * (nc + 16);
 		if (c->h_ritems) { (void)hipHostFree(c->h_ritems); c->h_ritems = nullptr; }
 		if (hipHostMalloc((void **)&c->h_ritems, (size_t)4 * nc * sizeof(int), hipHostMallocMapped) != hipSuccess ||
 		    hipHostGetDevicePointer((void **)&c->m_ritems, c->h_ritems, 0) != hipSuccess)
@@ -221,6 +222,16 @@
 		while (lb.size() % c->count_group) lb.push_back(-1);
 		la.insert(la.end(), lb.begin(), lb.end());
 		if (!la.empty()) HIPCHK(c, hipMemcpy(c->d_ftiles, la.data(), sizeof(int) * la.size(), hipMemcpyHostToDevice));
+	}
+	{
+		std::vector<int> cov(nc, 0);
+		for (int b = 0; b < nc; ++b) {
+			if (from_above[b]) { cov[b] = 2; continue; }
+			if (b + 1 >= nc || c->chunks[b + 1].off != c->chunks[b].off || in_run[b]) continue;
+			const Chunk &up = c->chunks[b + 1];
+			if (std::min(up.hi, up.L - 1) >= up.lo) cov[b] = 1;
+		}
+		HIPCHK(c, hipMemcpy(c->d_ftiles + c->vcover_off, cov.data(), sizeof(int) * cov.size(), hipMemcpyHostToDevice));
 	}
 	c->items_two_phase = two_phase_bwd ? 2 : 0; c->items_coarse = coarse;
 	HIPCHK(c, hipMemcpy(c->d_items, h.data(), sizeof(int) * h.size(), hipMemcpyHostToDevice));
@@ -470,6 +481,7 @@
 	p.coarse = coarse; p.d_singles_b = c->d_items + 24 * (size_t)p.n_chunks; p.n_singles_b = c->n_singles_b;
 	p.n_B_b = c->n_B_b; p.runs_in_b = c->runs_in_b ? 1 : 0; p.n_list_a = c->n_list_a; p.n_list_b = c->n_list_b; p.d_ftiles = c->d_ftiles; p.count_group = c->count_group;
 	c->timing_two_launches = p.fused == 1 && p.n_list_b > 0;
+	p.tail = c->tail != 0 && c->use_struct && p.fused == 1 && c->overlap ? 1 : 0; p.d_vcover = c->d_ftiles + c->vcover_off;
 	p.d_items_f = c->d_items; p.d_items_b = c->d_items + 2 * p.n_chunks;
 	p.d_ritems_f = c->d_items + 4 * p.n_chunks; p.d_ritems_b = c->d_items + 6 * p.n_chunks;
 	p.n_items_f = c->n_items_f; p.n_items_b = c->n_items_b; p.tile_len = c->chunk_used; p.h_ritems = c->h_ritems; p.m_ritems = c->m_ritems; p.m_cnt = c->m_cnt;
diff --git a/psmc_amd/csrc/estep_fast.hip b/psmc_amd/csrc/estep_fast.hip
--- a/psmc_amd/csrc/estep_fast.hip
+++ b/psmc_amd/csrc/estep_fast.hip
@@ -21,16 +21,6 @@
 	return r;
 }
 
-__device__ __forceinline__ double wave_max(double v) {
-#pragma unroll
-	for (int m = 32; m >= 1; m >>= 1) v = fmax(v, __shfl_xor(v, m, 64));
-	return v;
-}
-__device__ __forceinline__ double wave_add(double v) {
-#pragma unroll
-	for (int m = 32; m >= 1; m >>= 1) v += __shfl_xor(v, m, 64);
-	return v;
-}
 __device__ __forceinline__ double rel_mismatch(double x, double y) {
 	const double num = wave_max(fabs(x - y)), den = wave_max(fabs(y));
 	const bool bad = __any((x != x) || (y != y));
@@ -165,26 +155,17 @@
 template <int S> __device__ __forceinline__ double rel_mismatch_vec(const double *x, const double *y, int lane, bool with_scale = false) {
 	double xv = x[lane], yv = y[lane], xw = 0.0, yw = 0.0;
 	if (S == 128) { xw = x[64 + lane]; yw = y[64 + lane]; }
-	const double sx = wave_add(xv + xw), sy = wave_add(yv + yw);
-	const double ix = 1.0 / sx, iy = 1.0 / sy;
-	double num = fabs(xv * ix - yv * iy), den = fabs(yv * iy);
-	if (with_scale) num = fmax(num, fabs(sx - sy) * iy * den);
-	bool bad = (xv != xv) || (yv != yv) || (ix != ix) || (iy != iy);
-	if (S == 128) {
-		num = fmax(num, fabs(xw * ix - yw * iy)); den = fmax(den, fabs(yw * iy));
-		bad = bad || (xw != xw) || (yw != yw);
-	}
-	num = wave_max(num); den = wave_max(den);
-	return __any(bad) ? __builtin_inf() : num / den;
+	return rel_mismatch_vals<S>(xv, yv, xw, yw, with_scale);
 }
 template <bool BWD, int S>
 __global__ __launch_bounds__(64) void k_verify(const Chunk *__restrict__ chunks, int n_chunks, double tol,
                                                  const double *__restrict__ f, const double *__restrict__ mine,
                                                  const double *__restrict__ bexit, int *__restrict__ dirty,
                                                  int *__restrict__ cnt, unsigned long long *__restrict__ warm, int with_scale,
-                                                 double *__restrict__ mis)
+                                                 double *__restrict__ mis, const int *__restrict__ cover)
 {
 	const int lane = threadIdx.x, b = blockIdx.x;
+	if (cover != nullptr && cover[b] != 0) return;
 	const Chunk c = chunks[b];
 	double m = 0.0;
 	bool check;
@@ -192,16 +173,10 @@
 		check = c.lo > 1 && !(c.flags & CHUNK_ANCHOR_F);
 		if (check) m = rel_mismatch_vec<S>(mine + (int64_t)b * S, f + (c.off + c.lo - 2) * S, lane);
 	} else {
-		check = !(c.flags & (CHUNK_ANCHOR_B | CHUNK_LAST)) && min(c.hi, c.L - 1) >= c.lo && b + 1 < n_chunks;
+		check = verify_check_bwd(c, b, n_chunks);
 		if (check) m = rel_mismatch_vec<S>(mine + (int64_t)b * S, bexit + (int64_t)(b + 1) * S, lane, with_scale != 0);
 	}
-	if (lane == 0) {
-		const int bad = check && !(m <= tol);
-		dirty[b] = bad;
-		if (bad) atomicAdd(cnt, 1);
-		if (mis) mis[b] = check ? m : -1.0;
-		if (check) atomicMax(&warm[BWD ? 1 : 0], (unsigned long long)__double_as_longlong(m));
-	}
+	if (lane == 0) verify_commit(b, check, m, tol, dirty, cnt, &warm[BWD ? 1 : 0], mis);
 }
 
 __device__ __forceinline__ bool tile_touched(const Chunk *__restrict__ chunks, int b, const int *__restrict__ touch_f,
@@ -352,10 +327,28 @@
 	if (lane == 0) LLpart[blockIdx.x] = ll * (double)c.mult;
 }
 
+template <int NB>
+__device__ __forceinline__ double sum_ahead(const double *__restrict__ p, int64_t stride, int &j, int n, double s)
+{
+	for (; j + (NB - 1) * RED_ROWS < n; j += NB * RED_ROWS) {
+		double v[NB];
+#pragma unroll
+		for (int u = 0; u < NB; ++u) v[u] = p[(int64_t)(j + u * RED_ROWS) * stride];
+#pragma unroll
+		for (int u = 0; u < NB; ++u) s += v[u];
+	}
+	return s;
+}
+__device__ __forceinline__ double sum_rows(const double *__restrict__ p, int64_t stride, int j, int n, double s)
+{
+	s = sum_ahead<16>(p, stride, j, n, s);
+	s = sum_ahead<4>(p, stride, j, n, s);
+	return sum_ahead<1>(p, stride, j, n, s);
+}
 template <int S>
 __global__ __launch_bounds__(256) void k_reduce1(const double *__restrict__ Cpart, const double *__restrict__ Spart,
                                                    int nC, int nS, const double *__restrict__ LLpart, int nchunks,
-                                                   double *__restrict__ stage)
+                                                   double *__restrict__ stage, int c0)
 {
 	constexpr int SL = S * S + 3 * S + 1;
 	const int y = blockIdx.y, tid = threadIdx.x;
@@ -363,19 +356,12 @@
 	if ((int)blockIdx.x < S * S / 256) {
 		const int i = blockIdx.x * 256 + tid;
 		double s = 0.0;
-		for (int j = y; j < nC; j += RED_ROWS) s += Cpart[(int64_t)j * (S * S) + i];
-		st[i] = s;
+		int j = y;
+		if (c0 > 0) { s = st[i]; if (j < c0) j += (c0 - j + RED_ROWS - 1) / RED_ROWS * RED_ROWS; }
+		st[i] = sum_rows(Cpart + i, S * S, j, nC, s);
 	} else {
-		for (int i = tid; i < 3 * S; i += 256) {
-			double s = 0.0;
-			for (int j = y; j < nS; j += RED_ROWS) s += Spart[(int64_t)j * (3 * S) + i];
-			st[S * S + i] = s;
-		}
-		if (tid == 255) {
-			double s = 0.0;
-			for (int j = y; j < nchunks; j += RED_ROWS) s += LLpart[j];
-			st[S * S + 3 * S] = s;
-		}
+		for (int i = tid; i < 3 * S; i += 256) st[S * S + i] = sum_rows(Spart + i, 3 * S, y, nS, 0.0);
+		if (tid == 255) st[S * S + 3 * S] = sum_rows(LLpart, 1, y, nchunks, 0.0);
 	}
 }
 template <int S>
@@ -444,7 +430,11 @@
 	hipStream_t sm = p.stream, sa = ov ? p.stream2 : p.stream, sx = ov ? p.stream3 : p.stream;
 	rep->fwd_rounds = rep->bwd_rounds = rep->fwd_tiles = rep->bwd_tiles = rep->merged = rep->recounted = 0;
 	rep->converged = 1;
+	static const bool recheck = getenv("PSMC_HIP_DEBUG_RECHECK") != nullptr;
+	const bool optimistic = p.fused != 0 && ov && !recheck;
+	const bool tl = p.tail != 0 && p.fused == 1 && optimistic && p.d_vcover != nullptr;
 	(void)hipMemsetAsync(p.d_warm, 0, 2 * sizeof(unsigned long long), sm);
+	if (tl) (void)hipMemsetAsync(p.d_cnt + 1, 0, sizeof(int), sm);
 	(void)hipMemsetAsync(p.d_touch_f, 0, 3 * sizeof(int) * (size_t)p.n_chunks, sm);
 	if (p.d_gate) (void)hipMemsetAsync(p.d_gate, 0, 2 * sizeof(int), sm);
 	if (p.q_grid > 0) (void)hipMemsetAsync(p.d_qhead, 0, sizeof(int), sm);
@@ -512,13 +502,14 @@
 		if (p.ev[8]) (void)hipEventRecord(p.ev[8], sa);
 		if (p.fused == 2) { if (p.coarse > 1) launch_bwd_acc(p, sa, 6, 0, p.n_singles_b); else launch_bwd_acc(p, sa, 0, fb0, p.n_items_b - fb0); }
 		else {
-			launch_bwd_count(p, sa, 0, false);
+			launch_bwd_count(p, sa, 0, false, false, tl);
 			if (p.n_list_b > 0) {
 				if (lw && ov && sw != sa && late) (void)hipStreamWaitEvent(sa, p.evx[7], 0);
 				(void)hipEventRecord(p.evx[11], sa);
 				(void)hipEventRecord(p.evx[12], sa);
-				launch_bwd_count(p, sa, 1, false);
-			}
+				launch_bwd_count(p, sa, 1, false, false, tl);
+			}
+			if (tl) (void)hipEventRecord(p.evx[13], sa);
 		}
 		if (p.ev[9]) (void)hipEventRecord(p.ev[9], sa);
 		if (p.ev[6]) (void)hipEventRecord(p.ev[6], sa);
@@ -541,15 +532,19 @@
 	struct Chain { hipStream_t st; hipEvent_t rb; int slot; bool bwd, done, pending; int round; };
 	Chain ch[2] = {{sm, p.evx[4], 0, false, false, false, 0}, {sa, p.evx[5], 1, true, false, false, 0}};
 	auto post_verify = [&](Chain &c) -> int {
-		(void)hipMemsetAsync(p.d_cnt + c.slot, 0, sizeof(int), c.st);
-		(void)hipMemsetAsync(p.d_warm + c.slot, 0, sizeof(unsigned long long), c.st);
+		const bool tv = tl && c.bwd && c.round == 0;
+		if (!tv) {
+			(void)hipMemsetAsync(p.d_cnt + c.slot, 0, sizeof(int), c.st);
+			(void)hipMemsetAsync(p.d_warm + c.slot, 0, sizeof(unsigned long long), c.st);
+		}
 #define PSMC_LV(BW, S, MINE, DIRTY, CNT) hipLaunchKernelGGL((k_verify<BW, S>), g, b, 0, c.st, p.d_chunks, p.n_chunks, p.tol, p.d_f, \
 			MINE, p.d_bexit, DIRTY, CNT, p.d_warm, (BW && !p.fused) ? 1 : 0, \
-			(p.m_mis && c.round == 0 && (BW || !p.merge)) ? p.m_mis + (BW ? p.n_chunks : 0) : nullptr)
+			(p.m_mis && c.round == 0 && (BW || !p.merge)) ? p.m_mis + (BW ? p.n_chunks : 0) : nullptr,  \
+			(BW && tv) ? p.d_vcover : nullptr)
 		if (!c.bwd) { if (p.ns == 128) PSMC_LV(false, 128, p.d_entry, p.d_dirty, p.d_cnt); else PSMC_LV(false, 64, p.d_entry, p.d_dirty, p.d_cnt); }
 		else { if (p.ns == 128) PSMC_LV(true, 128, p.d_bentry, p.d_dirty_b, p.d_cnt + 1); else PSMC_LV(true, 64, p.d_bentry, p.d_dirty_b, p.d_cnt + 1); }
 #undef PSMC_LV
-		launch_compact(p, c.st, c.bwd);
+		launch_compact(p, c.st, c.bwd, tv);
 		if (hipEventRecord(c.rb, c.st) != hipSuccess) return -1;
 		c.pending = true;
 		return 0;
@@ -561,34 +556,38 @@
 		else hipLaunchKernelGGL(k_ll<64>, g, b, 0, st, p.d_chunks, p.d_f, p.d_s, p.d_entry, p.d_LLpart, fm, p.d_finv);
 		PSMC_DBG("k_ll", p.n_chunks, 0, 0);
 	};
-	auto launch_reduce = [&](hipStream_t sm) {
+	auto launch_reduce = [&](hipStream_t sm, int part = 0) {
+		const int ga = p.fused == 1 ? (p.n_list_a + p.count_group - 1) / p.count_group : 0, c0 = part == 2 ? ga : 0;
 		const int nS = p.n_chunks * p.n_sub, nC = p.fused == 1 ? (p.n_list_a + p.count_group - 1) / p.count_group + (p.n_list_b + p.count_group - 1) / p.count_group : nS;
 		if (p.fused == 2) {
 			launch_reduce_factored(p, sm);
 		} else if (p.ns == 128) {
-			hipLaunchKernelGGL(k_reduce1<128>, dim3(128 * 128 / 256 + 1, RED_ROWS), dim3(256), 0, sm, p.d_Cpart, p.d_Epart, nC, nS, p.d_LLpart,
-			                   p.n_chunks, p.d_stage);
+			hipLaunchKernelGGL(k_reduce1<128>, dim3(128 * 128 / 256 + (part == 1 ? 0 : 1), RED_ROWS), dim3(256), 0, sm, p.d_Cpart, p.d_Epart, part == 1 ? ga : nC, nS, p.d_LLpart,
+			                   p.n_chunks, p.d_stage, c0);
+			if (part == 1) return;
 			hipLaunchKernelGGL(k_reduce2<128>, dim3((128 * 128 + 3 * 128 + 1 + 255) / 256), dim3(256), 0, sm, p.d_stage, p.d_a, p.d_e,
 			                   p.tiny_total, p.n_states, p.d_stats);
 		} else {
-			hipLaunchKernelGGL(k_reduce1<64>, dim3(17, RED_ROWS), dim3(256), 0, sm, p.d_Cpart, p.d_Epart, nC, nS, p.d_LLpart,
-			                   p.n_chunks, p.d_stage);
+			hipLaunchKernelGGL(k_reduce1<64>, dim3(part == 1 ? 16 : 17, RED_ROWS), dim3(256), 0, sm, p.d_Cpart, p.d_Epart, part == 1 ? ga : nC, nS, p.d_LLpart,
+			                   p.n_chunks, p.d_stage, c0);
+			if (part == 1) return;
 			hipLaunchKernelGGL(k_reduce2<64>, dim3((STATS_LEN + 255) / 256), dim3(256), 0, sm, p.d_stage, p.d_a, p.d_e,
 			                   p.tiny_total, p.n_states, p.d_stats);
 		}
 		if (p.ev[4]) (void)hipEventRecord(p.ev[4], sm);
 	};
 	if (post_verify(ch[0]) || post_verify(ch[1])) return -1;
-	static const bool recheck = getenv("PSMC_HIP_DEBUG_RECHECK") != nullptr;
-	const bool optimistic = p.fused != 0 && ov && !recheck;
 	if (optimistic) {
 		(void)hipStreamWaitEvent(sx, p.evx[4], 0);
 		launch_ll(sx);
-		(void)hipEventRecord(p.evx[2], sa); (void)hipStreamWaitEvent(sx, p.evx[2], 0);
+		const bool early = tl && p.n_list_a > 0 && p.n_list_b > 0;
+		if (early) { (void)hipStreamWaitEvent(sx, p.evx[12], 0); launch_reduce(sx, 1); }
+		if (tl) (void)hipStreamWaitEvent(sx, p.evx[13], 0);
+		else { (void)hipEventRecord(p.evx[2], sa); (void)hipStreamWaitEvent(sx, p.evx[2], 0); }
 		if (p.ev[1]) (void)hipEventRecord(p.ev[1], sx);
 		if (p.ev[2]) (void)hipEventRecord(p.ev[2], sx);
 		if (p.ev[3]) (void)hipEventRecord(p.ev[3], sx);
-		launch_reduce(sx);
+		launch_reduce(sx, early ? 2 : 0);
 		(void)hipEventRecord(p.evx[10], sx);
 	}
 	bool ll_stale = !optimistic;
diff --git a/psmc_amd/csrc/estep_fused.hip b/psmc_amd/csrc/estep_fused.hip
--- a/psmc_amd/csrc/estep_fused.hip
+++ b/psmc_amd/csrc/estep_fused.hip
@@ -60,6 +60,49 @@
 	for (int j = 0; j < 4; ++j)
 #pragma unroll
 		for (int j2 = 0; j2 < 4; ++j2) acc[j][j2] = __builtin_amdgcn_mfma_f64_16x16x4f64(FA[j], FB[j2], acc[j][j2], 0, 0, 0);
+}
+template <int NPL, int S>
+__device__ __forceinline__ void tail_verify(const TailVerify &tv, const Chunk *__restrict__ chunks, int tile, bool valid, bool work, bool from_above,
+                                            const double (&x)[NPL], const double *__restrict__ bentry, const double *__restrict__ bexit, int lane)
+{
+#pragma unroll
+	for (int r = 0; r < 4; ++r) {
+		const int t = __builtin_amdgcn_readlane(tile, 16 * r);
+		const bool v_r = __builtin_amdgcn_readlane((int)valid, 16 * r) != 0, w_r = __builtin_amdgcn_readlane((int)work, 16 * r) != 0;
+		const bool fa_r = __builtin_amdgcn_readlane((int)from_above, 16 * r) != 0;
+		if (v_r && fa_r && tv.cover[t] == 2) {
+			const Chunk cb = chunks[t];
+			const bool check = verify_check_bwd(cb, t, tv.n_chunks);
+			double m = 0.0;
+			if (check) {
+				const double *y = bexit + (int64_t)(t + 1) * S;
+				const double yv = y[lane], yw = S == 128 ? y[64 + lane] : 0.0;
+				m = rel_mismatch_vals<S>(yv, yv, yw, yw, false);
+			}
+			if (lane == 0) verify_commit(t, check, m, tv.tol, tv.dirty, tv.cnt, tv.warm, tv.mis);
+		}
+		if (w_r && t > 0 && tv.cover[t - 1] == 1) {
+			const Chunk cb = chunks[t - 1];
+			const bool check = verify_check_bwd(cb, t - 1, tv.n_chunks);
+			double m = 0.0;
+			if (check) {
+				double yv = 0.0, yw = 0.0;
+#pragma unroll
+				for (int i = 0; i < NPL; ++i) {
+					const double lo_v = __shfl(x[i], 16 * r + lane / NPL, 64);
+					if (lane % NPL == i) yv = lo_v;
+					if (S == 128) {
+						const double hi_v = __shfl(x[i], 16 * r + (64 + lane) / NPL, 64);
+						if (lane % NPL == i) yw = hi_v;
+					}
+				}
+				const double *xm = bentry + (int64_t)(t - 1) * S;
+				const double xv = xm[lane], xw = S == 128 ? xm[64 + lane] : 0.0;
+				m = rel_mismatch_vals<S>(xv, yv, xw, yw, false);
+			}
+			if (lane == 0) verify_commit(t - 1, check, m, tv.tol, tv.dirty, tv.cnt, tv.warm, tv.mis);
+		}
+	}
 }
 #ifdef PSMC_TRACE_SWEEP
 __device__ unsigned long long g_trace_c[4 * 8192];
@@ -71,7 +114,7 @@
                                                                 double *__restrict__ bentry, double *__restrict__ bexit,
                                                                 double *__restrict__ Cpart,
                                                                 double *__restrict__ Epart, const int *__restrict__ touch_f,
-                                                                const int *__restrict__ touch_b, const int *__restrict__ fmerge, const double *__restrict__ finv)
+                                                                const int *__restrict__ touch_b, const int *__restrict__ fmerge, const double *__restrict__ finv, const TailVerify tv)
 {
 	__shared__ double lds_e[4 * SF], lds_m[8];
 	const int lane = threadIdx.x, row = lane >> 4, m = lane & 15, k0 = NPLF * m;
@@ -204,6 +247,7 @@
 		const double zero[NPLF] = {0.0, 0.0, 0.0, 0.0};
 		storeN<NPLF>(os, S[0]); storeN<NPLF>(os + SF, S[1]); storeN<NPLF>(os + 2 * SF, zero);
 	}
+	if (tv.dirty != nullptr) tail_verify<NPLF, SF>(tv, chunks, tile, valid, work, from_above, x, bentry, bexit, lane);
 }
 
 constexpr int NPL8 = 8, S8 = 128;
@@ -276,7 +320,7 @@
                                                                  double *__restrict__ bentry, double *__restrict__ bexit,
                                                                  double *__restrict__ Cpart,
                                                                  double *__restrict__ Epart, const int *__restrict__ touch_f,
-                                                                 const int *__restrict__ touch_b)
+                                                                 const int *__restrict__ touch_b, const TailVerify tv)
 {
 	__shared__ d2v_t lds_e[4 * 64];
 	__shared__ double lds_m[8];
@@ -417,9 +461,10 @@
 		const double zero[NPL8] = {0.0, 0.0, 0.0, 0.0, 0.0, 0.0, 0.0, 0.0};
 		storeN<NPL8>(os, S[0]); storeN<NPL8>(os + S8, S[1]); storeN<NPL8>(os + 2 * S8, zero);
 	}
-}
-
-void launch_bwd_count(const EstepLaunch &p, hipStream_t st, int list, bool redo, bool all_from_bentry)
+	if (tv.dirty != nullptr) tail_verify<NPL8, S8>(tv, chunks, tile, valid, work, from_above, x, bentry, bexit, lane);
+}
+
+void launch_bwd_count(const EstepLaunch &p, hipStream_t st, int list, bool redo, bool all_from_bentry, bool verify)
 {
 	const int G = p.count_group;
 	const int ga = (p.n_list_a + G - 1) / G, gb = (p.n_list_b + G - 1) / G;
@@ -427,14 +472,16 @@
 	if (n_groups <= 0) return;
 	const int *tl = p.d_ftiles + (list == 0 ? 0 : G * ga);
 	const int g0 = list == 0 ? 0 : ga, md = all_from_bentry ? 3 : (redo ? 2 : 0);
+	TailVerify tv = {nullptr, nullptr, nullptr, nullptr, nullptr, 0.0, 0};
+	if (verify && md == 0) tv = {p.d_vcover, p.d_dirty_b, p.d_cnt + 1, p.d_warm + 1, p.m_mis ? p.m_mis + p.n_chunks : nullptr, p.tol, p.n_chunks};
 	if (p.ns == 128) {
 		hipLaunchKernelGGL(k_bwd_count8x_struct, dim3(n_groups), dim3(256), 0, st, p.d_sp, p.d_e, p.d_s, p.d_obs, p.d_chunks, tl, g0, md,
-		                   p.d_f, p.d_bentry, p.d_bexit, p.d_Cpart, p.d_Epart, p.d_touch_f, p.d_touch_b);
+		                   p.d_f, p.d_bentry, p.d_bexit, p.d_Cpart, p.d_Epart, p.d_touch_f, p.d_touch_b, tv);
 		PSMC_DBG("launch_bwd_count (128 states)", list, redo, n_groups);
 		return;
 	}
 	hipLaunchKernelGGL(k_bwd_count4f_struct, dim3(n_groups), dim3(64), 0, st, p.d_sp, p.d_e, p.d_s, p.d_obs, p.d_chunks, tl, g0, md,
-	                   p.d_f, p.d_bentry, p.d_bexit, p.d_Cpart, p.d_Epart, p.d_touch_f, p.d_touch_b, p.merge ? p.d_fmerge : nullptr, p.d_finv);
+	                   p.d_f, p.d_bentry, p.d_bexit, p.d_Cpart, p.d_Epart, p.d_touch_f, p.d_touch_b, p.merge ? p.d_fmerge : nullptr, p.d_finv, tv);
 	PSMC_DBG("launch_bwd_count", list, redo, n_groups);
 }
 
diff --git a/psmc_amd/csrc/estep_struct.hip b/psmc_amd/csrc/estep_struct.hip
--- a/psmc_amd/csrc/estep_struct.hip
+++ b/psmc_amd/csrc/estep_struct.hip
@@ -873,9 +873,14 @@
 }
 
 __global__ __launch_bounds__(64) void k_compact(const int *__restrict__ dirty, int n, SweepItem *__restrict__ out,
-                                                  SweepItem *__restrict__ host_out, int *__restrict__ host_cnt)
+                                                  SweepItem *__restrict__ host_out, int *__restrict__ host_cnt, const int *__restrict__ counted)
 {
 	const int lane = threadIdx.x;
+	if (counted != nullptr && *counted == 0) {
+		if (lane == 0) *host_cnt = 0;
+		__threadfence_system();
+		return;
+	}
 	int base = 0;
 	for (int i0 = 0; i0 < n; i0 += 64) {
 		const int i = i0 + lane;
@@ -948,11 +953,11 @@
 #undef PSMC_LQ
 	PSMC_DBG("launch_phase1_queue", nf, nb, p.q_grid);
 }
-void launch_compact(const EstepLaunch &p, hipStream_t st, bool bwd)
+void launch_compact(const EstepLaunch &p, hipStream_t st, bool bwd, bool counted)
 {
 	hipLaunchKernelGGL(k_compact, dim3(1), dim3(64), 0, st, bwd ? p.d_dirty_b : p.d_dirty, p.n_chunks,
 	                   (SweepItem *)(bwd ? p.d_ritems_b : p.d_ritems_f),
-	                   (SweepItem *)(p.m_ritems ? p.m_ritems + (size_t)(bwd ? 1 : 0) * 2 * p.n_chunks : nullptr), p.m_cnt + (bwd ? 1 : 0));
+	                   (SweepItem *)(p.m_ritems ? p.m_ritems + (size_t)(bwd ? 1 : 0) * 2 * p.n_chunks : nullptr), p.m_cnt + (bwd ? 1 : 0), counted ? p.d_cnt + (bwd ? 1 : 0) : nullptr);
 	PSMC_DBG("verify + launch_compact", bwd, p.n_chunks, 0);
 }
 void launch_sweeps(const EstepLaunch &p, hipStream_t st, int ff, int nf, int fb, int nb, bool top_only)
diff --git a/psmc_amd/csrc/psmc_hip_ctx.h b/psmc_amd/csrc/psmc_hip_ctx.h
--- a/psmc_amd/csrc/psmc_hip_ctx.h
+++ b/psmc_amd/csrc/psmc_hip_ctx.h
@@ -135,6 +135,8 @@
 	int runs_late = 1;
 	bool runs_in_b = false;
 	int *d_ftiles = nullptr;
+	size_t vcover_off = 0;
+	int tail = 1;
 	FastReport report = {0, 0, 0, 0, 1, 0, 0};
 	double *d_stage = nullptr, *d_stats = nullptr;
 	unsigned long long *d_warm = nullptr;
diff --git a/psmc_amd/csrc/psmc_hip_internal.h b/psmc_amd/csrc/psmc_hip_internal.h
--- a/psmc_amd/csrc/psmc_hip_internal.h
+++ b/psmc_amd/csrc/psmc_hip_internal.h
@@ -25,6 +25,50 @@
 constexpr int CHUNK_ANCHOR_F = 1;
 constexpr int CHUNK_ANCHOR_B = 2;
 constexpr int CHUNK_LAST = 4;
+
+__device__ __forceinline__ double wave_max(double v) {
+#pragma unroll
+	for (int m = 32; m >= 1; m >>= 1) v = fmax(v, __shfl_xor(v, m, 64));
+	return v;
+}
+__device__ __forceinline__ double wave_add(double v) {
+#pragma unroll
+	for (int m = 32; m >= 1; m >>= 1) v += __shfl_xor(v, m, 64);
+	return v;
+}
+template <int S> __device__ __forceinline__ double rel_mismatch_vals(double xv, double yv, double xw, double yw, bool with_scale) {
+	if (S != 128) { xw = 0.0; yw = 0.0; }
+	const double sx = wave_add(xv + xw), sy = wave_add(yv + yw);
+	const double ix = 1.0 / sx, iy = 1.0 / sy;
+	double num = fabs(xv * ix - yv * iy), den = fabs(yv * iy);
+	if (with_scale) num = fmax(num, fabs(sx - sy) * iy * den);
+	bool bad = (xv != xv) || (yv != yv) || (ix != ix) || (iy != iy);
+	if (S == 128) {
+		num = fmax(num, fabs(xw * ix - yw * iy)); den = fmax(den, fabs(yw * iy));
+		bad = bad || (xw != xw) || (yw != yw);
+	}
+	num = wave_max(num); den = wave_max(den);
+	return __any(bad) ? __builtin_inf() : num / den;
+}
+__device__ __forceinline__ bool verify_check_bwd(const Chunk &c, int b, int n_chunks) {
+	return !(c.flags & (CHUNK_ANCHOR_B | CHUNK_LAST)) && min(c.hi, c.L - 1) >= c.lo && b + 1 < n_chunks;
+}
+__device__ __forceinline__ void verify_commit(int b, bool check, double m, double tol, int *__restrict__ dirty, int *__restrict__ cnt,
+                                              unsigned long long *__restrict__ warm, double *__restrict__ mis) {
+	const int bad = check && !(m <= tol);
+	dirty[b] = bad;
+	if (bad) atomicAdd(cnt, 1);
+	if (mis) mis[b] = check ? m : -1.0;
+	if (check) atomicMax(warm, (unsigned long long)__double_as_longlong(m));
+}
+struct TailVerify {
+	const int *cover;
+	int *dirty, *cnt;
+	unsigned long long *warm;
+	double *mis;
+	double tol;
+	int n_chunks;
+};
 
 struct ExWork {
 	const int32_t *seg;
@@ -76,6 +120,8 @@
 	const int *d_ftiles; int n_list_a, n_list_b;
 	int count_group;
 	int runs_in_b;
+	int tail;
+	const int *d_vcover;
 	hipStream_t stream4, stream5;
 	const int *d_wl_f, *d_wl_b; int n_wl_f, n_wl_b;
 	const int *d_kc, *d_kruns; int n_kc, n_chain_f, n_chain_b;
@@ -135,7 +181,7 @@
 int launch_fast(const EstepLaunch &p, FastReport *rep);
 void launch_fwd_struct(const EstepLaunch &p, hipStream_t st, int which, int first, int n_items);
 void launch_bwd_struct(const EstepLaunch &p, hipStream_t st, int which, int first, int n_items);
-void launch_compact(const EstepLaunch &p, hipStream_t st, bool bwd);
+void launch_compact(const EstepLaunch &p, hipStream_t st, bool bwd, bool counted = false);
 void launch_gather_prev(const EstepLaunch &p, hipStream_t st, int first, int n_items, double *prevx);
 int launch_tile_allmiss(hipStream_t st, const uint8_t *d_obs, const Chunk *d_chunks, int n_chunks, int *d_flags);
 void launch_walks(const EstepLaunch &p, hipStream_t st);
@@ -144,7 +190,7 @@
 void launch_kchain(const EstepLaunch &p, hipStream_t st_cols, hipStream_t st_chain, hipEvent_t ev_cols);
 void launch_sweeps(const EstepLaunch &p, hipStream_t st, int ff, int nf, int fb, int nb, bool top_only);
 void launch_phase1_queue(const EstepLaunch &p, hipStream_t st, int ff, int nf, int fb, int nb);
-void launch_bwd_count(const EstepLaunch &p, hipStream_t st, int list, bool redo, bool all_from_bentry = false);
+void launch_bwd_count(const EstepLaunch &p, hipStream_t st, int list, bool redo, bool all_from_bentry = false, bool verify = false);
 void launch_bwd_acc(const EstepLaunch &p, hipStream_t st, int which, int first, int n);
 void launch_reduce_factored(const EstepLaunch &p, hipStream_t st);
 int launch_post_decode(hipStream_t st, const double *f, const double *b, const double *s, int64_t off, int L, int n,
```

Result: faster. 2.540 billion bins/s (median of 6 runs) (+1.6%).
